# haberdashPI/SignalOperators.jl

Hardware: AMD Instinct MI355X
Metric: frames/sec sink() 44.1kHz 8ch Mix+Filt+Resample; achieved HBM GB/s (higher is better)
Workload: dtype f64

## Files before the change

include/sigops.h:

```cpp
#ifndef SIGOPS_H
#define SIGOPS_H

#include <stdint.h>

#ifdef __cplusplus
extern "C" {
#endif
#if defined(__GNUC__)
#pragma GCC visibility push(default)
#endif

#define SO_ABI_VERSION 1

typedef enum so_status {
    SO_OK = 0,
    SO_ERR_INVALID = -1,
    SO_ERR_LENGTH = -2,
    SO_ERR_UNSUPPORTED = -3,
    SO_ERR_RUNTIME = -4,
    SO_ERR_CHANNELS = -5,
    SO_ERR_NODEVICE = -6
} so_status_t;

typedef enum so_dtype {
// ... 39 lines not shown
    SO_RAMP_IDENTITY = 1,
    SO_RAMP_EXPR = 2
} so_rampfn_t;

typedef enum so_mapfn {
    SO_MAP_ADD = 0,
    SO_MAP_MUL = 1,
    SO_MAP_SUB = 2,
    SO_MAP_DIV = 3,
    SO_MAP_TUPLECAT = 4,
    SO_MAP_GETCHAN = 5,
    SO_MAP_AS1CHANNEL = 6,
    SO_MAP_ASNCHANNELS = 7,
    SO_MAP_TOELTYPE = 8,
    SO_MAP_REVERSECH = 9,
    SO_MAP_EXPR = 10
} so_mapfn_t;

typedef struct so_eop {
    int32_t code;
    int32_t arg;
} so_eop_t;

typedef enum so_eop_code {
    SO_EOP_ARG = 0,
    SO_EOP_CONST = 1,
    SO_EOP_UN = 2,
    SO_EOP_BIN = 3,
    SO_EOP_CMP = 4,
    SO_EOP_SELECT = 5,
    SO_EOP_ROUND32 = 6,
    SO_EOP_INTERP = 7
} so_eop_code_t;

typedef enum so_un {
    SO_UN_NEG = 0, SO_UN_ABS = 1, SO_UN_SQRT = 2, SO_UN_CBRT = 3, SO_UN_SQUARE = 4,
    SO_UN_RECIPROCAL = 5, SO_UN_EXP = 6, SO_UN_EXP2 = 7, SO_UN_EXPM1 = 8, SO_UN_LOG = 9,
    SO_UN_LOG2 = 10, SO_UN_LOG10 = 11, SO_UN_LOG1P = 12, SO_UN_SIN = 13, SO_UN_COS = 14,
    SO_UN_TAN = 15, SO_UN_ARCSIN = 16, SO_UN_ARCCOS = 17, SO_UN_ARCTAN = 18, SO_UN_SINH = 19,
    SO_UN_COSH = 20, SO_UN_TANH = 21, SO_UN_ARCSINH = 22, SO_UN_ARCCOSH = 23,
    SO_UN_ARCTANH = 24, SO_UN_FLOOR = 25, SO_UN_CEIL = 26, SO_UN_TRUNC = 27, SO_UN_RINT = 28,
    SO_UN_SIGN = 29,
    SO_UN_COUNT = 30
} so_un_t;

typedef enum so_bin {
    SO_BIN_ADD = 0, SO_BIN_SUB = 1, SO_BIN_MUL = 2, SO_BIN_DIV = 3, SO_BIN_POW = 4,
    SO_BIN_REMAINDER = 5, SO_BIN_FMOD = 6, SO_BIN_MINIMUM = 7, SO_BIN_MAXIMUM = 8,
    SO_BIN_FMIN = 9, SO_BIN_FMAX = 10, SO_BIN_ARCTAN2 = 11, SO_BIN_HYPOT = 12,
    SO_BIN_COPYSIGN = 13,
    SO_BIN_COUNT = 14
} so_bin_t;

typedef enum so_cmp {
    SO_CMP_LT = 0, SO_CMP_LE = 1, SO_CMP_GT = 2, SO_CMP_GE = 3, SO_CMP_EQ = 4, SO_CMP_NE = 5,
    SO_CMP_COUNT = 6
} so_cmp_t;

typedef enum so_padkind {
    SO_PAD_VALUE = 0,
    SO_PAD_VECTOR = 1,
    SO_PAD_ZERO = 2,
    SO_PAD_ONE = 3,
    SO_PAD_LASTFRAME = 4,
    SO_PAD_CYCLE = 5,
    SO_PAD_MIRROR = 6
} so_padkind_t;

typedef enum so_rskind {
    SO_RS_RATIONAL = 0,
    SO_RS_ARBITRARY = 1,
    SO_RS_FIR = 2
} so_rskind_t;

typedef struct so_node {
    int32_t kind;
    int32_t dtype;
    int32_t nch;
    int32_t n_children;
    const int32_t* children;
    int64_t nframes;
    double fs;
    int32_t i0, i1, i2, i3;
    int64_t l0, l1;
    double d0, d1, d2, d3;
    const void* p0;
    const void* p1;
    int64_t s0, s1;
} so_node_t;

typedef struct so_out_desc {
    int32_t dtype;
    int32_t nch;
    int64_t nframes;
    int64_t frame_stride;
    int64_t chan_stride;
    int32_t is_device;
    int32_t reserved;
} so_out_desc_t;

typedef struct so_stats {
    int32_t n_stages;
    int32_t n_launches;
    int64_t algorithmic_bytes;
    int64_t scratch_bytes;
    int64_t h2d_bytes;
    int64_t d2h_bytes;
    double last_exec_ms;
    double dominant_kernel_ms;
    int64_t dominant_kernel_bytes;
    char dominant_kernel[64];
} so_stats_t;

typedef struct so_plan so_plan_t;

int32_t so_abi_version(void);

const char* so_last_error(void);

int32_t so_device_count(void);

int32_t so_plan_create(const so_node_t* nodes, int32_t n_nodes, int32_t root,
                       const so_out_desc_t* out, int32_t device, so_plan_t** plan);

int64_t so_plan_nframes(const so_plan_t* plan);

int32_t so_plan_execute(so_plan_t* plan, void* out, void* hip_stream);

int32_t so_plan_check(so_plan_t* plan, void* hip_stream);

int32_t so_plan_set_array(so_plan_t* plan, int32_t node_index, const void* data);

int32_t so_plan_stats(const so_plan_t* plan, so_stats_t* stats);

typedef struct so_step_info {
    char name[64];
    int64_t algorithmic_bytes;
    double ms;
    int32_t launches;
    int32_t pad;
} so_step_info_t;
int32_t so_plan_step_info(const so_plan_t* plan, int32_t index, so_step_info_t* info);

typedef enum so_counter {
    SO_COUNTER_GRAPH_REPLAYS = 0,
    SO_COUNTER_GRAPH_CAPTURES = 1,
    SO_COUNTER_DIRECT_EXECUTES = 2,
    SO_COUNTER_FUSED_MFMAS_PER_BLOCK = 3,
    SO_COUNTER_WPROJ = 4,
    SO_COUNTER_RSOS_RANGE_PERIODS = 5,
    SO_COUNTER_RSOS_WARMUP_PERIODS = 6,
    SO_COUNTER_RSOS_PERIOD_INPUTS = 7,
    SO_COUNTER_WPROJ_FRAMES = 8,
    SO_COUNTER_WPROJ_FIRST = 9
} so_counter_t;
int64_t so_plan_counter(const so_plan_t* plan, int32_t which);

int32_t so_rtc_compile_check(const char* body, char* log, int32_t log_capacity);

int32_t so_rtc_wait_idle(void);
int32_t so_rtc_shutdown(void);

int32_t so_plan_set_profiling(so_plan_t* plan, int32_t enable);

void so_plan_destroy(so_plan_t* plan);

typedef struct so_comm so_comm_t;
typedef struct so_slab {
    int64_t rows, row_elems;
    int64_t dst_offset;
    int64_t dst_row_stride;
} so_slab_t;
int32_t so_comm_unique_id(void* id128);
int32_t so_comm_create(const void* id128, int32_t world, int32_t rank, int32_t device, so_comm_t** comm);
int32_t so_comm_allgather(so_comm_t* comm, const void* mine, int64_t src_row_stride, void* full,
                          const so_slab_t* slabs, int32_t dtype, void* stream);
int32_t so_comm_reduce_sum(so_comm_t* comm, void* buf, int64_t rows, int64_t row_elems, int64_t row_stride,
                           int32_t dtype, int32_t root, void* stream);
const char* so_comm_last_error(void);
void so_comm_destroy(so_comm_t* comm);

typedef enum so_filt_type {
    SO_FILT_LOWPASS = 0,
    SO_FILT_HIGHPASS = 1,
    SO_FILT_BANDPASS = 2,
    SO_FILT_BANDSTOP = 3
} so_filt_type_t;

typedef enum so_filt_method {
    SO_METHOD_BUTTERWORTH = 0,
    SO_METHOD_CHEBYSHEV1 = 1
} so_filt_method_t;

int32_t so_design_iir(int32_t type, double f1, double f2, double fs, int32_t method,
                      int32_t order, double ripple_db, double* sos, int32_t sos_capacity,
                      int32_t* nsections, double* gain);

int32_t so_design_iir_zpk(int32_t type, double f1, double f2, double fs, int32_t method, int32_t order,
                          double ripple_db, double* z, int32_t* nz, double* p, int32_t* np, int32_t capacity,
                          double* k);
int32_t so_zpk_to_sos(const double* z, int32_t nz, const double* p, int32_t np, double k, double* sos,
                      int32_t sos_capacity, int32_t* nsections, double* gain);

int32_t so_tf_to_sos(const double* b, int32_t nb, const double* a, int32_t na, double* sos, int32_t sos_capacity,
                     int32_t* nsections, double* gain, double* residual);
int32_t so_tf_zero_input(const double* b, int32_t nb, const double* a, int32_t na, const double* si, int32_t nsi,
                         double* out, int64_t capacity, int64_t* nframes);

int32_t so_design_resample_rational(int64_t num, int64_t den, double* h, int32_t capacity,
                                    int32_t* hlen);
int32_t so_design_resample_arbitrary(double rate, int32_t nphi, double* h, int32_t capacity,
                                     int32_t* hlen);

int32_t so_resample_positions(double fs_in, double fs_out, double rate, int32_t nphi, const double* h,
                              int32_t hlen, int64_t n_out, int64_t* j, int32_t* p, double* alpha,
                              int64_t* nfix, int64_t* nbaked);

int32_t so_rsos_wproj_matrix(const double* sos, int32_t nsec, double gain, const double* tab, const int32_t* jend,
                             int32_t ngroups, int32_t kw, int64_t m, int32_t wp, double* v, int32_t capacity,
                             int32_t* j0, int32_t* k);

#if defined(__GNUC__)
#pragma GCC visibility pop
#endif
#ifdef __cplusplus
}
#endif
#endif
```

signaloperators.jl_amd/_capi.py:

```python
import ctypes as C
import os

_HERE = os.path.dirname(os.path.abspath(__file__))
LIB_PATH = os.environ.get("SIGOPS_LIB") or os.path.join(_HERE, "csrc", "libsigops.so")

SO_F32, SO_F64, SO_I64 = 0, 1, 2
SO_LEN_INF, SO_LEN_MISSING, SO_LEN_UNCHECKED = -1, -2, -3
(NODE_ARRAY, NODE_CONST, NODE_FUNC, NODE_UNTIL, NODE_AFTER, NODE_PAD, NODE_APPEND, NODE_RAMP,
 NODE_MAP, NODE_FILT_SOS, NODE_RESAMPLE, NODE_NORMPOWER, NODE_SAMPLEAT, NODE_COMB, NODE_CUMSUM,
 NODE_MOVING, NODE_MOVSUM, NODE_RECUR) = range(18)
FN = {"sin": 0, "cos": 1, "identity": 2, "randn": 3}
SO_FN_RANDN = FN["randn"]
RAMPFN = {"sinramp": 0, "identity": 1, "expr": 2}
MAPFN = {"add": 0, "mul": 1, "sub": 2, "div": 3, "tuplecat": 4, "getchan": 5, "as1channel": 6,
         "asnchannels": 7, "toeltype": 8, "reversech": 9, "expr": 10}
EOP = {"arg": 0, "const": 1, "un": 2, "bin": 3, "cmp": 4, "select": 5, "round32": 6, "interp": 7}
INTERP_MAX_KNOTS = 1 << 20
UN = {name: i for i, name in enumerate((
    "neg", "abs", "sqrt", "cbrt", "square", "reciprocal", "exp", "exp2", "expm1", "log", "log2", "log10", "log1p",
    "sin", "cos", "tan", "arcsin", "arccos", "arctan", "sinh", "cosh", "tanh", "arcsinh", "arccosh", "arctanh",
    "floor", "ceil", "trunc", "rint", "sign"))}
BIN = {name: i for i, name in enumerate((
    "add", "sub", "mul", "div", "pow", "remainder", "fmod", "minimum", "maximum", "fmin", "fmax", "arctan2", "hypot",
    "copysign"))}
CMP = {"lt": 0, "le": 1, "gt": 2, "ge": 3, "eq": 4, "ne": 5}
PAD = {"value": 0, "vector": 1, "zero": 2, "one": 3, "lastframe": 4, "cycle": 5, "mirror": 6}
RS_RATIONAL, RS_ARBITRARY, RS_FIR = 0, 1, 2
FILT = {"lowpass": 0, "highpass": 1, "bandpass": 2, "bandstop": 3}
METHOD = {"butterworth": 0, "chebyshev1": 1}


class so_node_t(C.Structure):
    _fields_ = [("kind", C.c_int32), ("dtype", C.c_int32), ("nch", C.c_int32),
                ("n_children", C.c_int32), ("children", C.POINTER(C.c_int32)),
                ("nframes", C.c_int64), ("fs", C.c_double),
                ("i0", C.c_int32), ("i1", C.c_int32), ("i2", C.c_int32), ("i3", C.c_int32),
                ("l0", C.c_int64), ("l1", C.c_int64),
                ("d0", C.c_double), ("d1", C.c_double), ("d2", C.c_double), ("d3", C.c_double),
                ("p0", C.c_void_p), ("p1", C.c_void_p), ("s0", C.c_int64), ("s1", C.c_int64)]


class so_out_desc_t(C.Structure):
    _fields_ = [("dtype", C.c_int32), ("nch", C.c_int32), ("nframes", C.c_int64),
                ("frame_stride", C.c_int64), ("chan_stride", C.c_int64),
                ("is_device", C.c_int32), ("reserved", C.c_int32)]


class so_stats_t(C.Structure):
    _fields_ = [("n_stages", C.c_int32), ("n_launches", C.c_int32),
                ("algorithmic_bytes", C.c_int64), ("scratch_bytes", C.c_int64),
                ("h2d_bytes", C.c_int64), ("d2h_bytes", C.c_int64),
                ("last_exec_ms", C.c_double), ("dominant_kernel_ms", C.c_double),
                ("dominant_kernel_bytes", C.c_int64), ("dominant_kernel", C.c_char * 64)]


class so_slab_t(C.Structure):
    _fields_ = [("rows", C.c_int64), ("row_elems", C.c_int64), ("dst_offset", C.c_int64), ("dst_row_stride", C.c_int64)]


class so_step_info_t(C.Structure):
    _fields_ = [("name", C.c_char * 64), ("algorithmic_bytes", C.c_int64), ("ms", C.c_double),
                ("launches", C.c_int32), ("pad", C.c_int32)]


EXPORTS = ["so_abi_version", "so_last_error", "so_device_count", "so_plan_create",
           "so_plan_nframes", "so_plan_execute", "so_plan_check", "so_plan_set_array", "so_plan_stats",
           "so_plan_set_profiling", "so_plan_destroy", "so_design_iir",
           "so_design_resample_rational", "so_design_resample_arbitrary",
           "so_resample_positions", "so_plan_step_info", "so_design_iir_zpk", "so_zpk_to_sos", "so_tf_to_sos", "so_tf_zero_input", "so_plan_counter", "so_rsos_wproj_matrix",
           "so_rtc_compile_check", "so_rtc_wait_idle", "so_rtc_shutdown", "so_comm_unique_id", "so_comm_create", "so_comm_allgather", "so_comm_reduce_sum", "so_comm_last_error", "so_comm_destroy"]

_lib = None


class EngineMissing(RuntimeError):
    pass


def lib():
    global _lib
    if _lib is not None:
        return _lib
    if not os.path.exists(LIB_PATH):
        raise EngineMissing(
            f"{LIB_PATH} not built: run `python __graft_entry__.py build` "
            "(hipcc --offload-arch=gfx950). The HIP engine has no CPU fallback.")
    try:
        import importlib.util as _ilu

        if _ilu.find_spec("torch") is not None:
            import torch
    except Exception:
        pass
    L = C.CDLL(LIB_PATH)
    L.so_abi_version.restype = C.c_int32
    L.so_last_error.restype = C.c_char_p
    L.so_device_count.restype = C.c_int32
    L.so_plan_create.restype = C.c_int32
    L.so_plan_create.argtypes = [C.POINTER(so_node_t), C.c_int32, C.c_int32,
                                 C.POINTER(so_out_desc_t), C.c_int32, C.POINTER(C.c_void_p)]
    L.so_plan_nframes.restype = C.c_int64
    L.so_plan_nframes.argtypes = [C.c_void_p]
    L.so_plan_execute.restype = C.c_int32
    L.so_plan_execute.argtypes = [C.c_void_p, C.c_void_p, C.c_void_p]
    L.so_plan_check.restype = C.c_int32
    L.so_plan_check.argtypes = [C.c_void_p, C.c_void_p]
    L.so_plan_set_array.restype = C.c_int32
    L.so_plan_set_array.argtypes = [C.c_void_p, C.c_int32, C.c_void_p]
    L.so_plan_stats.restype = C.c_int32
    L.so_plan_stats.argtypes = [C.c_void_p, C.POINTER(so_stats_t)]
    L.so_plan_set_profiling.restype = C.c_int32
    L.so_plan_set_profiling.argtypes = [C.c_void_p, C.c_int32]
    L.so_plan_destroy.restype = None
    L.so_plan_destroy.argtypes = [C.c_void_p]
    L.so_design_iir.restype = C.c_int32
    L.so_design_iir.argtypes = [C.c_int32, C.c_double, C.c_double, C.c_double, C.c_int32,
                                C.c_int32, C.c_double, C.POINTER(C.c_double), C.c_int32,
                                C.POINTER(C.c_int32), C.POINTER(C.c_double)]
    L.so_design_resample_rational.restype = C.c_int32
    L.so_design_resample_rational.argtypes = [C.c_int64, C.c_int64, C.POINTER(C.c_double),
                                              C.c_int32, C.POINTER(C.c_int32)]
    L.so_design_resample_arbitrary.restype = C.c_int32
    L.so_design_resample_arbitrary.argtypes = [C.c_double, C.c_int32, C.POINTER(C.c_double),
                                               C.c_int32, C.POINTER(C.c_int32)]
    L.so_design_iir_zpk.restype = C.c_int32
    L.so_design_iir_zpk.argtypes = [C.c_int32, C.c_double, C.c_double, C.c_double, C.c_int32, C.c_int32, C.c_double,
                                    C.POINTER(C.c_double), C.POINTER(C.c_int32), C.POINTER(C.c_double),
                                    C.POINTER(C.c_int32), C.c_int32, C.POINTER(C.c_double)]
    L.so_zpk_to_sos.restype = C.c_int32
    L.so_zpk_to_sos.argtypes = [C.POINTER(C.c_double), C.c_int32, C.POINTER(C.c_double), C.c_int32, C.c_double,
                                C.POINTER(C.c_double), C.c_int32, C.POINTER(C.c_int32), C.POINTER(C.c_double)]
    L.so_tf_to_sos.restype = C.c_int32
    L.so_tf_to_sos.argtypes = [C.POINTER(C.c_double), C.c_int32, C.POINTER(C.c_double), C.c_int32, C.POINTER(C.c_double),
                               C.c_int32, C.POINTER(C.c_int32), C.POINTER(C.c_double), C.POINTER(C.c_double)]
    L.so_tf_zero_input.restype = C.c_int32
    L.so_tf_zero_input.argtypes = [C.POINTER(C.c_double), C.c_int32, C.POINTER(C.c_double), C.c_int32,
                                   C.POINTER(C.c_double), C.c_int32, C.POINTER(C.c_double), C.c_int64,
                                   C.POINTER(C.c_int64)]
    L.so_rtc_compile_check.restype = C.c_int32
    L.so_rtc_compile_check.argtypes = [C.c_char_p, C.c_char_p, C.c_int32]
    L.so_rtc_wait_idle.restype = C.c_int32
    L.so_rtc_wait_idle.argtypes = []
    L.so_rtc_shutdown.restype = C.c_int32
    L.so_rtc_shutdown.argtypes = []
    import atexit

    atexit.register(L.so_rtc_shutdown)
    L.so_comm_unique_id.restype = C.c_int32
    L.so_comm_unique_id.argtypes = [C.c_void_p]
    L.so_comm_create.restype = C.c_int32
    L.so_comm_create.argtypes = [C.c_void_p, C.c_int32, C.c_int32, C.c_int32, C.POINTER(C.c_void_p)]
    L.so_comm_allgather.restype = C.c_int32
    L.so_comm_allgather.argtypes = [C.c_void_p, C.c_void_p, C.c_int64, C.c_void_p, C.POINTER(so_slab_t), C.c_int32, C.c_void_p]
    L.so_comm_reduce_sum.restype = C.c_int32
    L.so_comm_reduce_sum.argtypes = [C.c_void_p, C.c_void_p, C.c_int64, C.c_int64, C.c_int64, C.c_int32, C.c_int32, C.c_void_p]
    L.so_comm_last_error.restype = C.c_char_p
    L.so_comm_destroy.restype = None
    L.so_comm_destroy.argtypes = [C.c_void_p]
    L.so_plan_counter.restype = C.c_int64
    L.so_plan_counter.argtypes = [C.c_void_p, C.c_int32]
    L.so_rsos_wproj_matrix.restype = C.c_int32
    L.so_rsos_wproj_matrix.argtypes = [C.POINTER(C.c_double), C.c_int32, C.c_double, C.POINTER(C.c_double), C.POINTER(C.c_int32),
                                       C.c_int32, C.c_int32, C.c_int64, C.c_int32, C.POINTER(C.c_double), C.c_int32,
                                       C.POINTER(C.c_int32), C.POINTER(C.c_int32)]
    L.so_plan_step_info.restype = C.c_int32
    L.so_plan_step_info.argtypes = [C.c_void_p, C.c_int32, C.POINTER(so_step_info_t)]
    L.so_resample_positions.restype = C.c_int32
    L.so_resample_positions.argtypes = [C.c_double, C.c_double, C.c_double, C.c_int32, C.POINTER(C.c_double),
                                        C.c_int32, C.c_int64, C.POINTER(C.c_int64), C.POINTER(C.c_int32),
                                        C.POINTER(C.c_double), C.POINTER(C.c_int64), C.POINTER(C.c_int64)]
    if L.so_abi_version() != 1:
        raise EngineMissing("libsigops ABI version mismatch")
    _lib = L
    return L


def last_error():
    return lib().so_last_error().decode("utf-8", "replace")
```

signaloperators.jl_amd/csrc/capi.cpp:

```cpp
#include <hip/hip_runtime_api.h>

#include <cstring>
#include <string>
#include <vector>

#include "../../include/sigops.h"
#include "plan.h"

namespace {
thread_local std::string g_err;
int set_err(int status, const std::string& msg) {
    g_err = msg;
    return status;
}
}

struct so_plan {
    so::Plan* p;
};

extern "C" {

int32_t so_abi_version(void) { return SO_ABI_VERSION; }

// ... 73 lines not shown
int32_t so_rtc_shutdown(void) {
    so::rtc_shutdown();
    return SO_OK;
}

int64_t so_plan_counter(const so_plan_t* plan, int32_t which) {
    if (!plan) return -1;
    return so::plan_counter(plan->p, which);
}

int32_t so_plan_step_info(const so_plan_t* plan, int32_t index, so_step_info_t* info) {
    if (!plan) return set_err(SO_ERR_INVALID, "so_plan_step_info: null plan");
    return so::plan_step_info(plan->p, index, info);
}

void so_plan_destroy(so_plan_t* plan) {
    if (!plan) return;
    so::plan_destroy(plan->p);
    delete plan;
}

int32_t so_design_iir(int32_t type, double f1, double f2, double fs, int32_t method,
                      int32_t order, double ripple_db, double* sos, int32_t sos_capacity,
                      int32_t* nsections, double* gain) {
    std::vector<double> s;
    double g = 1.0;
    std::string err;
    int st = so::design_iir(type, f1, f2, fs, method, order, ripple_db, s, g, err);
    if (st != SO_OK) return set_err(st, err);
    if (!sos || !nsections || !gain || (int)s.size() > sos_capacity)
        return set_err(SO_ERR_INVALID, "so_design_iir: output buffer too small");
    std::memcpy(sos, s.data(), s.size() * sizeof(double));
    *nsections = (int32_t)(s.size() / 6);
    *gain = g;
    return SO_OK;
}

int32_t so_design_iir_zpk(int32_t type, double f1, double f2, double fs, int32_t method, int32_t order,
                          double ripple_db, double* z, int32_t* nz, double* p, int32_t* np, int32_t capacity,
                          double* k) {
    std::vector<double> zz, pp;
    double kk = 1.0;
    std::string err;
    int st = so::design_iir_zpk(type, f1, f2, fs, method, order, ripple_db, zz, pp, kk, err);
    if (st != SO_OK) return set_err(st, err);
    if (!z || !p || !nz || !np || !k || (int)zz.size() > 2 * capacity || (int)pp.size() > 2 * capacity)
        return set_err(SO_ERR_INVALID, "so_design_iir_zpk: output buffer too small");
    std::memcpy(z, zz.data(), zz.size() * sizeof(double));
    std::memcpy(p, pp.data(), pp.size() * sizeof(double));
    *nz = (int32_t)(zz.size() / 2);
    *np = (int32_t)(pp.size() / 2);
    *k = kk;
    return SO_OK;
}

int32_t so_zpk_to_sos(const double* z, int32_t nz, const double* p, int32_t np, double k, double* sos,
                      int32_t sos_capacity, int32_t* nsections, double* gain) {
    std::vector<double> s;
    double g = 1.0;
    std::string err;
    if ((nz > 0 && !z) || (np > 0 && !p)) return set_err(SO_ERR_INVALID, "so_zpk_to_sos: null roots");
    int st = so::zpk_to_sos(z, nz, p, np, k, s, g, err);
    if (st != SO_OK) return set_err(st, err);
    if (!sos || !nsections || !gain || (int)s.size() > sos_capacity)
        return set_err(SO_ERR_INVALID, "so_zpk_to_sos: output buffer too small");
    std::memcpy(sos, s.data(), s.size() * sizeof(double));
    *nsections = (int32_t)(s.size() / 6);
    *gain = g;
    return SO_OK;
}

int32_t so_tf_to_sos(const double* b, int32_t nb, const double* a, int32_t na, double* sos, int32_t sos_capacity,
                     int32_t* nsections, double* gain, double* residual) {
    std::vector<double> s;
    double g = 1.0, r = 0.0;
    std::string err;
    int st = so::tf_to_sos(b, nb, a, na, s, g, r, err);
    if (st != SO_OK) return set_err(st, err);
    if (!sos || !nsections || !gain || (int)s.size() > sos_capacity)
        return set_err(SO_ERR_INVALID, "so_tf_to_sos: output buffer too small");
    std::memcpy(sos, s.data(), s.size() * sizeof(double));
    *nsections = (int32_t)(s.size() / 6);
    *gain = g;
    if (residual) *residual = r;
    return SO_OK;
}

int32_t so_tf_zero_input(const double* b, int32_t nb, const double* a, int32_t na, const double* si, int32_t nsi,
                         double* out, int64_t capacity, int64_t* nframes) {
    std::string err;
    int64_t used = 0;
    if (!out || !nframes || capacity < 0) return set_err(SO_ERR_INVALID, "so_tf_zero_input: null output");
    int st = so::tf_zero_input(b, nb, a, na, si, nsi, out, capacity, used, err);
    if (st != SO_OK) return set_err(st, err);
    *nframes = used;
    return SO_OK;
}

static int32_t copy_taps(const std::vector<double>& h, double* out, int32_t capacity, int32_t* hlen) {
    if (!hlen) return set_err(SO_ERR_INVALID, "null hlen");
    *hlen = (int32_t)h.size();
    if (!out) return SO_OK;
    if ((int)h.size() > capacity) return set_err(SO_ERR_INVALID, "tap buffer too small");
    std::memcpy(out, h.data(), h.size() * sizeof(double));
    return SO_OK;
}

int32_t so_design_resample_rational(int64_t num, int64_t den, double* h, int32_t capacity,
                                    int32_t* hlen) {
    std::vector<double> t;
    std::string err;
    int st = so::design_resample_rational(num, den, t, err);
    if (st != SO_OK) return set_err(st, err);
    return copy_taps(t, h, capacity, hlen);
}

int32_t so_design_resample_arbitrary(double rate, int32_t nphi, double* h, int32_t capacity,
                                     int32_t* hlen) {
    std::vector<double> t;
    std::string err;
    int st = so::design_resample_arbitrary(rate, nphi, t, err);
    if (st != SO_OK) return set_err(st, err);
    return copy_taps(t, h, capacity, hlen);
}

int32_t so_resample_positions(double fs_in, double fs_out, double rate, int32_t nphi, const double* h,
                              int32_t hlen, int64_t n_out, int64_t* j, int32_t* p, double* alpha,
                              int64_t* nfix, int64_t* nbaked) {
    if (!h || hlen < 1 || nphi < 1 || !(rate > 0) || n_out < 0 || !j || !p || !alpha)
        return set_err(SO_ERR_INVALID, "so_resample_positions: bad arguments");
    return so::resample_positions(fs_in, fs_out, rate, nphi, h, hlen, n_out, j, p, alpha, nfix, nbaked);
}

int32_t so_rsos_wproj_matrix(const double* sos, int32_t nsec, double gain, const double* tab, const int32_t* jend,
                             int32_t ngroups, int32_t kw, int64_t m, int32_t wp, double* v, int32_t capacity,
                             int32_t* j0, int32_t* k) {
    if (!sos || !tab || !jend || !v || !j0 || !k || nsec < 1 || nsec > 6 || ngroups < 1 || kw < 1 || m < 1 || wp < 1)
        return set_err(SO_ERR_INVALID, "so_rsos_wproj_matrix: bad arguments");
    if (ngroups > 256 || kw > 4096 || capacity < 0 || m > (1 << 20) || wp > (1 << 20) || (int64_t)wp * m + kw > (1 << 22))
        return set_err(SO_ERR_INVALID, "so_rsos_wproj_matrix: period, window or warm-up too long");
    for (int g = 0; g < ngroups; ++g)
        if (jend[g] < -(1 << 22) || jend[g] > (1 << 22)) return set_err(SO_ERR_INVALID, "so_rsos_wproj_matrix: window end out of range");
    std::vector<double> V;
    int jj = 0, K = 0;
    so::rsos_wproj_matrix_sos(sos, nsec, gain, tab, jend, ngroups, kw, m, wp, V, jj, K);
    *j0 = jj;
    *k = K;
    if (K > capacity) return set_err(SO_ERR_INVALID, "so_rsos_wproj_matrix: capacity too small");
    for (int d = 0; d < 12; ++d)
        for (int o = 0; o < K; ++o) v[(size_t)d * capacity + o] = V[(size_t)d * K + o];
    return SO_OK;
}

}
```

signaloperators.jl_amd/csrc/executor.cpp:

```cpp
#include "plan_impl.h"

namespace so {

static inline int carrier_vec_ok(const DCarrier& c, int64_t V) {
    if (!std::getenv("SIGOPS_STRICT_ALIGN")) return (uintptr_t)c.base % (c.dtype == SO_F64 ? 8 : 4) == 0;
    return ((uintptr_t)c.base % 16 == 0) && (c.cstride % V == 0);
}

static hipError_t h2d_small(void* dst, const void* src, size_t bytes) {
    constexpr size_t kPiece = 16 * 1024;
    if (bytes < 2 * kPiece || bytes > (1u << 20)) return hipMemcpy(dst, src, bytes, hipMemcpyHostToDevice);
    for (size_t off = 0; off < bytes; off += kPiece) {
        const hipError_t e = hipMemcpy((char*)dst + off, (const char*)src + off, std::min(kPiece, bytes - off), hipMemcpyHostToDevice);
        if (e != hipSuccess) return e;
    }
    return hipSuccess;
}

static void upload_tables(Plan* P) {
    std::vector<Buf>& bufs = P->bufs;
    auto up = [&](int buf, const auto& v, size_t at = 0) {
        HIPCHECK(h2d_small((char*)bufs[buf].d + at, v.data(), v.size() * sizeof(*v.data())));
    };
    auto alloc_up = [](auto*& d, const auto& v) {
// ... 723 lines not shown
    const int nl = launch_comb(a, st);
    if (nl < 0) fail(SO_ERR_UNSUPPORTED, "Comb: more than 65535 channels, or a delay AND a signal of 2^39 frames and more, are not lowered");
    return nl;
}

static int run_cumsum(Plan* P, const Step& s, void* outp, hipStream_t st) {
    const Stage& S = P->stages[s.idx];
    const Node& N = P->nodes[S.node];
    const int xdt = P->nodes[N.kids[0]].dtype;
    const View in = stage_in(P, S, N.nch, xdt), out = stage_out(P, s.idx, outp);
    CumsumArgs a{};
    a.x = in.d;
    a.xcs = in.pitch;
    a.xfs = S.x_fstride;
    a.x_f32 = xdt == SO_F32;
    a.y = (double*)out.d;
    a.ycs = out.pitch;
    a.n = S.need;
    a.nch = N.nch;
    a.tot_pitch = cumsum_totals(S.need);
    a.tot = S.aux_buf >= 0 ? (double*)P->bufs[S.aux_buf].d : nullptr;
    const int nl = launch_cumsum(a, st);
    if (nl < 0) fail(SO_ERR_UNSUPPORTED, "Cumsum: more than 65535 channels, or 2^31 chunks of 16384 frames and more, are not lowered");
    return nl;
}

static int run_recur(Plan* P, const Step& s, void* outp, hipStream_t st) {
    const Stage& S = P->stages[s.idx];
    const Node& N = P->nodes[S.node];
    const bool row = N.kids.size() == 2;
    const int bdt = P->nodes[N.kids[row ? 1 : 0]].dtype;
    const View in = stage_in(P, S, N.nch, bdt), out = stage_out(P, s.idx, outp);
    RecurArgs a{};
    a.b = in.d;
    a.bcs = in.pitch;
    a.bfs = S.x_fstride;
    a.b_f32 = bdt == SO_F32;
    if (!row) {
        a.ac = N.nd.d0;
    } else if (S.pos_array_node >= 0) {
        a.a = (const double*)array_base(P, S.pos_array_node) + S.pos_offset;
        a.acs = S.pos_pitch;
    } else {
        const Buf& b = P->bufs[S.pos_buf];
        a.a = (const double*)b.d;
        a.acs = S.pos_pitch == 0 ? 0 : b.pitch;
    }
    a.y = (double*)out.d;
    a.ycs = out.pitch;
    a.n = S.need;
    a.nch = N.nch;
    a.op = N.nd.i0;
    a.tot_pitch = cumsum_totals(S.need);
    a.tot = S.aux_buf >= 0 ? (double*)P->bufs[S.aux_buf].d : nullptr;
    const int nl = launch_recur(a, st);
    if (nl < 0) fail(SO_ERR_UNSUPPORTED, "Recur: more than 65535 channels, or 2^31 chunks of 16384 frames and more, are not lowered");
    return nl;
}

static int run_moving(Plan* P, const Step& s, void* outp, hipStream_t st) {
    const Stage& S = P->stages[s.idx];
    const Node& N = P->nodes[S.node];
    const View in = stage_in(P, S, N.nch, N.dtype), out = stage_out(P, s.idx, outp);
    MovingArgs a{};
    a.x = in.d;
    a.xcs = in.pitch;
    a.xfs = S.x_fstride;
    a.n_in = S.in_frames;
    a.y = out.d;
    a.ycs = out.pitch;
    a.n_out = S.need - S.base;
    a.off = S.base - S.in_base;
    a.back = N.nd.l0;
    a.ahead = N.nd.l1;
    a.tab = S.aux_buf >= 0 ? P->bufs[S.aux_buf].d : nullptr;
    a.nch = N.nch;
    a.f32 = N.dtype == SO_F32;
    a.is_min = N.nd.i0;
    const int nl = launch_moving(a, st);
    if (nl < 0) fail(SO_ERR_UNSUPPORTED, "Moving: more than 65535 channels, or 2^31 tiles of 2048 frames and more, are not lowered");
    return nl;
}

static int run_movsum(Plan* P, const Step& s, void* outp, hipStream_t st) {
    const Stage& S = P->stages[s.idx];
    const Node& N = P->nodes[S.node];
    const int xdt = P->nodes[N.kids[0]].dtype;
    const View in = stage_in(P, S, N.nch, xdt), out = stage_out(P, s.idx, outp);
    MovsumArgs a{};
    a.x = in.d;
    a.xcs = in.pitch;
    a.xfs = S.x_fstride;
    a.x_f32 = xdt == SO_F32;
    a.n_in = S.in_frames;
    a.y = (double*)out.d;
    a.ycs = out.pitch;
    a.n_out = S.need - S.base;
    a.off = S.base - S.in_base;
    a.abs0 = S.in_base;
    a.back = N.nd.l0;
    a.ahead = N.nd.l1;
    a.tab = S.aux_buf >= 0 ? (double*)P->bufs[S.aux_buf].d : nullptr;
    a.nch = N.nch;
    a.op = N.nd.i0;
    const int nl = launch_movsum(a, st);
    if (nl < 0) fail(SO_ERR_UNSUPPORTED, "Movsum: more than 65535 channels, or 2^31 tiles of 2048 frames or blocks of 1024 frames and more, are not lowered");
    return nl;
}

static int run_rsos_fused(Plan* P, const Stage& S, const SosGeom& g, const View& out, hipStream_t st) {
    const Node& N = P->nodes[S.node];
    const Stage& S3 = P->stages[S.rsos_src];
    RsSos rs = S.rs;
    rs.out_pitch = out.pitch;
    rs.out_f32 = g.out_dtype == SO_F32 || N.dtype == SO_F32;
    if (rs.f32m && rs.out_f32) rs.ring32 = 1;
    else rs.f32m = 0;
    rs.sring = rs.f32m && (rs.fuse == 1 || rs.fuse == 2) && !std::getenv("SIGOPS_RSOS_NO_SRING") ? 1 : 0;
    char* const yk = out.d - (size_t)S.rs.store_lo * (rs.out_f32 ? 4 : 8);
    rs.store_lo = S.rs.store_lo + g.store_lo;
    rs.mats = (const double*)P->bufs[S.rsos_mats_buf].d;
    rs.bad = nullptr;
    const bool fixup = S.rsos_jrel_buf >= 0 && !std::getenv("SIGOPS_RSOS_NO_FIXUP");
    int rearm = 0;
    if (S.bad_buf >= 0 && rs.nranges >= 1 && !std::getenv("SIGOPS_SOS_NOPOISON")) {
        int32_t* const words = (int32_t*)P->bufs[S.bad_buf].d;
        const size_t nch = (size_t)N.nch;
        if (fixup && !P->graph_plan && rs.nch == N.nch && P->bufs[S.bad_buf].bytes >= 2 * nch * 4) {
            if (!S.bad_armed) {
                arm_bad(words, 2 * nch, st);
                S.bad_set = 0;
            }
            rs.bad = words + (S.bad_set ? nch : 0);
            rearm = S.bad_set ? -(int)nch : (int)nch;
        } else {
            S.bad_armed = false;
            rs.bad = words;
            arm_bad(rs.bad, nch, st);
        }
    }
    rs.err = kernel_error_word(P);
    static long long* d_rtrace = nullptr;
    static int rtrace_seen = 0;
    const char* const rtrace_skip = std::getenv("SIGOPS_RSOS_TRACE_SKIP");
    const bool rtracing = std::getenv("SIGOPS_RSOS_TRACE") != nullptr && rtrace_seen++ >= (rtrace_skip ? std::atoi(rtrace_skip) : 0);
    const size_t rtrace_n = (size_t)(16 * kRsosTraceIters + 16) * 8;
    if (rtracing) {
        if (!d_rtrace) HIPCHECK(hipMalloc(&d_rtrace, rtrace_n * 8));
        HIPCHECK(hipMemsetAsync(d_rtrace, 0, rtrace_n * 8, st));
        rs.trace = d_rtrace;
    }
    const double* rtab = (const double*)P->bufs[S.rsos_tab_buf >= 0 ? S.rsos_tab_buf : S3.tab_buf].d;
    const int* rjend = (const int*)P->bufs[S.rsos_jend_buf >= 0 ? S.rsos_jend_buf : S3.jend_buf].d;
    if (launch_rsos(rtab, rjend, rs, yk, global_tables(P, S3), S.rsos_grid, st) != 0)
        fail(SO_ERR_RUNTIME, "internal: no fused resampler + IIR instantiation for this geometry");
    if (rtracing) dump_rsos_trace(d_rtrace, rtrace_n, rs, st);
    int nl = 1;
    if (rs.bad && fixup) {
        RsFixup fx{};
        set_rsos_fixup(fx, P, S, RsosItem{rs, rtab, rjend, yk, global_tables(P, S3)});
        fx.rearm = rearm;
        nl += launch_rsos_fixup(fx, st);
        if (rearm != 0) {
            S.bad_set ^= 1;
            S.bad_armed = true;
        }
    } else if (rs.bad) {
        SosGeom pg = g;
        pg.n = rs.n_out;
        pg.chunk = rs.pr * rs.L;
        pg.nchunks = rs.nranges;
        pg.store_lo = rs.store_lo;
        pg.bad = rs.bad;
        nl += launch_sos_poison(yk, pg, st);
    }
    return nl;
}

static int run_sos(Plan* P, const Step& s, void* outp, hipStream_t st) {
    const Stage& S = P->stages[s.idx];
    const Node& N = P->nodes[S.node];
    const size_t esz = dsize(N.dtype);
    const View in = stage_in(P, S, N.nch, N.dtype), out = stage_out(P, s.idx, outp);
    SosGeom g = S.sg;
    g.in_pitch = in.pitch;
    g.out_pitch = out.pitch;
    g.store_lo = s.idx == P->alias_stage ? P->alias_skip : 0;
    if (s.idx == P->alias_stage && P->alias_narrow) g.out_dtype = SO_F32;
    g.align_rows = S.pre_stage < 0 && !std::getenv("SIGOPS_SOS_NOALIGN");
    g.bad = nullptr;
    if (S.rsos_src >= 0) return run_rsos_fused(P, S, g, out, st);
    if (S.bad_buf >= 0 && S.pre_stage < 0 && !S.onepass && !S.xscan && !g.exact && !std::getenv("SIGOPS_SOS_NOPOISON")) {
        g.bad = (int32_t*)P->bufs[S.bad_buf].d;
        arm_bad(g.bad, (size_t)N.nch, st);
    }
    int nl = 0;
    for (size_t gi = 0; gi < S.groups.size() && S.onepass; ++gi) {
        const void* x = gi == 0 ? (const void*)in.d : (const void*)out.d;
        SosOne o = S.so1;
        o.in_pitch = gi == 0 ? in.pitch : out.pitch;
        o.out_pitch = out.pitch;
        const int64_t al = 16 / (int64_t)esz;
        o.vec_in = ((uintptr_t)x % 16 == 0) && (o.in_pitch % al == 0);
        o.vec_out = ((uintptr_t)out.d % 16 == 0) && (o.out_pitch % al == 0);
        const Buf& sb = P->bufs[S.one_sync_buf];
        const Buf& vb = P->bufs[S.one_vpub_buf];
        if (sb.bytes % 4 == 0 && vb.bytes % 4 == 0) {
            HIPCHECK((hipError_t)launch_fill_u32(sb.d, sb.bytes / 4, 0u, st));
            HIPCHECK((hipError_t)launch_fill_u32(vb.d, vb.bytes / 4, 0xffffffffu, st));
        } else {
            HIPCHECK(hipMemsetAsync(sb.d, 0, sb.bytes, st));
            HIPCHECK(hipMemsetAsync(vb.d, 0xff, vb.bytes, st));
        }
        launch_sos_onepass(x, out.d, o, S.groups[gi], (const double*)P->bufs[S.one_tabs_buf].d + S.one_tabs_off[gi],
                           (int*)sb.d, (double*)vb.d, N.dtype, st);
        nl += 1;
    }
    if (S.pre_stage >= 0) {
        const Stage& S3 = P->stages[S.pre_stage];
        nl += launch_sos_prestate(in.d, out.d, (const double*)P->bufs[S3.vper_buf].d, S3.rp.nperiods,
                                  (const double*)P->bufs[S.qmat_buf].d, S3.rp.pt, (double*)P->bufs[S.v_buf].d,
                                  (double*)P->bufs[S.s0_buf].d, (const double*)P->bufs[S.mpow_buf].d, g, S.groups[0], st);
    }
    bool exact_done = false;
    if (g.exact && !S.onepass && S.pre_stage < 0 && S.groups.size() <= 2) {
        exact_done = launch_sos_exact(in.d, out.d, g, S.groups[0], S.groups.size() > 1 ? S.groups[1] : SosCoefs{}, st) == 0;
        if (exact_done) nl += 1;
    }
    for (size_t gi = 0; gi < S.groups.size() && !S.onepass && S.pre_stage < 0 && !exact_done; ++gi) {
        const void* x = gi == 0 ? (const void*)in.d : (const void*)out.d;
        SosGeom gg = g;
        if (gi > 0) gg.in_pitch = out.pitch;
        if (gi == 0 && S.src_op) set_sine_source(gg, S);
        if (S.xscan) {
            double* vb = (double*)P->bufs[S.v_buf].d;
            double* sb = (double*)P->bufs[S.s0_buf].d;
            nl += launch_sos_phase(x, out.d, vb, nullptr, gg, S.groups[gi], 1, st);
            nl += launch_sos_xscan(vb, sb, (const double*)((char*)P->bufs[S.xs_mats_buf].d + gi * 2 * 16 * 16 * 8),
                                   (double*)P->bufs[S.sblk_buf].d, gg, S.groups[gi].nsec, st);
            nl += launch_sos_phase(x, out.d, nullptr, sb, gg, S.groups[gi], 3, st);
            continue;
        }
        nl += launch_sos(x, out.d, S.v_buf >= 0 ? (double*)P->bufs[S.v_buf].d : nullptr,
                         S.s0_buf >= 0 ? (double*)P->bufs[S.s0_buf].d : nullptr,
                         S.mpow_buf >= 0 ? (const double*)((char*)P->bufs[S.mpow_buf].d + gi * S.mpow_stride() * 8) : nullptr,
                         gg, S.groups[gi], st);
        nl += launch_sos_poison(out.d, gg, st);
        if (gg.bad && gi + 1 < S.groups.size()) arm_bad(gg.bad, (size_t)N.nch, st);
    }
    return nl;
}

static void run_resample_periodic(Plan* P, const Step& s, const View& out, hipStream_t st) {
    const Stage& S = P->stages[s.idx];
    const Node& N = P->nodes[S.node];
    RsPeriodic rp = S.rp;
    rp.in_pitch = 0;
    rp.out_pitch = out.pitch;
    rp.out_f32 = s.idx == P->alias_stage && P->alias_narrow;
    if (rp.nstate > 0) {
        rp.wtab = (const double*)P->bufs[S.wtab_buf].d;
        rp.vper = (double*)P->bufs[S.vper_buf].d;
    }
    const int64_t al = 16 / (int64_t)dsize(N.dtype);
    rp.vec_ok = ((uintptr_t)out.d % 16 == 0) && (out.pitch % al == 0) && (rp.L % al == 0);
    static long long* d_trace = nullptr;
    const bool tracing = std::getenv("SIGOPS_RS_TRACE") != nullptr;
    const size_t trace_n = (size_t)16 * kRsTraceIters * kRsTraceStamps;
    if (tracing) {
        if (!d_trace) HIPCHECK(hipMalloc(&d_trace, trace_n * 8));
        HIPCHECK(hipMemsetAsync(d_trace, 0, trace_n * 8, st));
        rp.trace = d_trace;
    }
    const bool nf_fix = S.rs_nf_buf >= 0 && S.rs_jrel_buf >= 0 && rp.ga == 0 && rp.arr2 == 0 && rp.nstate == 0 && S.ctl_buf >= 0 &&
                        S.car_buf >= 0 && !S.carriers.empty() && rp.rows <= 32 && rp.kw <= 160;
    rp.nf = nf_fix ? (uint32_t*)P->bufs[S.rs_nf_buf].d : nullptr;
    const double* tab = (const double*)P->bufs[S.tab_buf].d;
    const int* jend = (const int*)P->bufs[S.jend_buf].d;
    if (launch_resample_periodic(out.d, tab, jend, rp, N.dtype, global_tables(P, S), st) != 0)
        fail(SO_ERR_RUNTIME, "internal: no periodic resampler instantiation for this geometry");
    if (nf_fix) {
        RsPerFixup fx{};
        fx.g = rp;
        fx.tab = tab;
        fx.jend = jend;
        fx.jrel = (const int*)P->bufs[S.rs_jrel_buf].d;
        fx.taps = S.rg.taps;
        fx.out_f32 = (N.dtype == SO_F32 || rp.out_f32) ? 1 : 0;
        fx.gsrc = global_tables(P, S);
        fx.y = out.d;
        (void)launch_rs_fixup(fx, st);
    }
    if (tracing) dump_rs_trace(d_trace, trace_n, rp, st);
}

static int run_resample(Plan* P, const Step& s, void* outp, hipStream_t st) {
    const Stage& S = P->stages[s.idx];
    const Node& N = P->nodes[S.node];
    const View in = S.periodic ? View{nullptr, 0} : stage_in(P, S, N.nch, N.dtype), out = stage_out(P, s.idx, outp);
    const double* pfbt = S.tiled ? (const double*)P->bufs[S.pfbt_buf].d : nullptr;
    const double* dpfbt = S.tiled ? (const double*)P->bufs[S.dpfbt_buf].d : nullptr;
    if (S.periodic)
        run_resample_periodic(P, s, out, st);
    else if (S.rows) {
        RsRows rr = S.rr;
        rr.in_pitch = in.pitch;
        rr.out_pitch = out.pitch;
// ... 172 lines not shown
                if (ms > best) {
                    best = ms;
                    P->stats.dominant_kernel_ms = ms;
                    P->stats.dominant_kernel_bytes = P->steps[si].bytes;
                    std::snprintf(P->stats.dominant_kernel, sizeof P->stats.dominant_kernel, "%s", P->steps[si].name.c_str());
                }
            }
            P->stats.last_exec_ms = total;
        }
    } catch (const PlanError& e) {
        disarm_bad(P);
        err = e.msg;
        return e.status;
    }
    return SO_OK;
}

int plan_execute(Plan* P, void* outp, void* stream, std::string& err) {
    DeviceGuard guard(P->device);
    if (kernel_gave_up(P, err)) {
        disarm_bad(P);
        return SO_ERR_RUNTIME;
    }
    const bool eligible = P->steps.size() >= 4 && P->out.is_device && P->host_leaves.empty() && !P->profiling &&
                          !std::getenv("SIGOPS_NO_GRAPH") && !std::getenv("SIGOPS_RS_TRACE");
    P->graph_plan = eligible;
    if (!eligible) {
        P->n_direct++;
        return plan_execute_direct(P, outp, stream, err);
    }
    hipStream_t st = (hipStream_t)stream;
    const bool leaves_match = P->out_alias_buf < 0 || P->bufs[P->out_alias_buf].d == outp;
    if (P->graph_exec && P->graph_out == outp && P->graph_epoch == P->array_epoch && leaves_match) {
        if (hipSetDevice(P->device) == hipSuccess && hipGraphLaunch(P->graph_exec, st) == hipSuccess) {
            P->n_replays++;
            return SO_OK;
        }
        (void)hipGetLastError();
        (void)hipGraphExecDestroy(P->graph_exec);
        P->graph_exec = nullptr;
        P->graph_failed = true;
    }
    if (P->graph_failed || P->last_out != outp || P->last_epoch != P->array_epoch) {
        P->last_out = outp;
        P->last_epoch = P->array_epoch;
        P->n_direct++;
        return plan_execute_direct(P, outp, stream, err);
    }
    if (P->graph_exec && P->graph_out == outp && P->graph_epoch == P->array_epoch) {
        P->n_direct++;
        return plan_execute_direct(P, outp, stream, err);
    }
    if (P->graph_exec) {
        (void)hipGraphExecDestroy(P->graph_exec);
        P->graph_exec = nullptr;
    }
    hipGraph_t graph = nullptr;
    if (!P->capture_stream && hipStreamCreateWithFlags(&P->capture_stream, hipStreamNonBlocking) != hipSuccess)
        P->capture_stream = nullptr;
    if (!P->capture_stream || hipSetDevice(P->device) != hipSuccess ||
        hipStreamBeginCapture(P->capture_stream, hipStreamCaptureModeRelaxed) != hipSuccess) {
        (void)hipGetLastError();
        P->graph_failed = true;
        return plan_execute_direct(P, outp, stream, err);
    }
    const int rc = plan_execute_direct(P, outp, (void*)P->capture_stream, err);
    const hipError_t ec = hipStreamEndCapture(P->capture_stream, &graph);
    if (std::getenv("SIGOPS_DEBUG_PLAN"))
        std::fprintf(stderr, "[sigops] graph capture: rc=%d end=%d (%s) graph=%p err=%s\n", rc, (int)ec, hipGetErrorString(ec), (void*)graph, err.c_str());
    if (rc != SO_OK || ec != hipSuccess || !graph ||
        hipGraphInstantiate(&P->graph_exec, graph, nullptr, nullptr, 0) != hipSuccess) {
        (void)hipGetLastError();
        if (graph) (void)hipGraphDestroy(graph);
        P->graph_exec = nullptr;
        P->graph_failed = true;
        return rc != SO_OK ? rc : plan_execute_direct(P, outp, stream, err);
    }
    (void)hipGraphDestroy(graph);
    P->graph_out = outp;
    P->graph_epoch = P->array_epoch;
    P->n_captures++;
    if (hipGraphLaunch(P->graph_exec, st) != hipSuccess) {
        (void)hipGetLastError();
        P->graph_failed = true;
        return plan_execute_direct(P, outp, stream, err);
    }
    return SO_OK;
}

int plan_set_array(Plan* P, int32_t node_index, const void* data, std::string& err) {
    if (node_index < 0 || node_index >= (int)P->nodes.size() || P->nodes[node_index].nd.kind != SO_NODE_ARRAY) {
        err = "so_plan_set_array: not an ARRAY node";
        return SO_ERR_INVALID;
    }
    DeviceGuard guard(P->device);
    P->array_ptr[node_index] = data;
    P->array_epoch++;
    if (P->nodes[node_index].nd.i0) {
        bool changed = false;
        for (size_t i = 0; i < P->leaves.size(); ++i)
            if (P->leaf_array_node[i] == node_index) {
                P->leaves[i].base = data;
                changed = true;
            }
        if (changed && P->d_leaves)
            if (hipMemcpy(P->d_leaves, P->leaves.data(), P->leaves.size() * sizeof(DLeaf), hipMemcpyHostToDevice) != hipSuccess) {
                err = "so_plan_set_array: leaf upload failed";
                return SO_ERR_RUNTIME;
            }
        for (auto& S : P->stages) {
            bool touched = false;
            for (auto& c : S.carriers) {
                if (c.array_node == node_index) {
                    c.base = data;
                    const int64_t V = 16 / (int64_t)dsize(c.dtype);
                    c.vec_ok = carrier_vec_ok(c, V);
                    touched = true;
                }
                if (car_has_arr2(c) && c.array_node2 == node_index) {
                    c.base2 = data;
                    c.vec_ok2 = (uintptr_t)c.base2 % (c.dtype2 == SO_F64 ? 8 : 4) == 0;
                    touched = true;
                }
            }
            if (touched) {
                const RsCtl ctl = P->make_ctl(S);
                if (hipMemcpy(P->bufs[S.car_buf].d, S.carriers.data(), S.carriers.size() * sizeof(DCarrier), hipMemcpyHostToDevice) != hipSuccess ||
                    hipMemcpy(P->bufs[S.ctl_buf].d, &ctl, sizeof(RsCtl), hipMemcpyHostToDevice) != hipSuccess) {
                    err = "so_plan_set_array: carrier upload failed";
                    return SO_ERR_RUNTIME;
                }
            }
        }
    }
    return SO_OK;
}

int64_t plan_nframes(const Plan* P) {
    const Node& R = P->nodes[P->root];
    return isinf_(R.len) ? SO_LEN_INF : R.len.n;
}
void plan_stats(const Plan* P, so_stats_t* st) { *st = P->stats; }
void plan_set_profiling(Plan* P, int mode) {
    P->profiling = mode < 0 || mode > 2 ? 1 : mode;
    P->prof_execs = 0;
}
int64_t plan_counter(const Plan* P, int which) {
    switch (which) {
    case SO_COUNTER_GRAPH_REPLAYS: return P->n_replays;
    case SO_COUNTER_GRAPH_CAPTURES: return P->n_captures;
    case SO_COUNTER_DIRECT_EXECUTES: return P->n_direct;
    case SO_COUNTER_FUSED_MFMAS_PER_BLOCK: {
        for (const Stage& S : P->stages)
            if (S.kind == ST_SOS && S.rsos_src >= 0 && S.need > 0) return S.rs.ks + 14;
        return 0;
    }
    case SO_COUNTER_WPROJ: {
        for (const Stage& S : P->stages)
            if (S.kind == ST_SOS && S.rsos_src >= 0 && S.need > 0) return S.rs.wproj;
        return 0;
    }
    case SO_COUNTER_RSOS_RANGE_PERIODS:
    case SO_COUNTER_RSOS_WARMUP_PERIODS:
    case SO_COUNTER_RSOS_PERIOD_INPUTS:
    case SO_COUNTER_WPROJ_FRAMES:
    case SO_COUNTER_WPROJ_FIRST:
        for (const Stage& S : P->stages)
            if (S.kind == ST_SOS && S.rsos_src >= 0 && S.need > 0)
                return which == SO_COUNTER_RSOS_RANGE_PERIODS ? S.rs.pr : which == SO_COUNTER_RSOS_WARMUP_PERIODS ? S.rs.wp
                     : which == SO_COUNTER_RSOS_PERIOD_INPUTS ? S.rs.M : which == SO_COUNTER_WPROJ_FRAMES ? S.rs.wk : S.rs.wj0;
        return 0;
    default: return -1;
    }
}
int plan_step_info(const Plan* P, int index, so_step_info_t* info) {
    if (info && index >= 0 && index < (int)P->steps.size()) {
        const Step& s = P->steps[index];
        std::memset(info, 0, sizeof *info);
        std::snprintf(info->name, sizeof info->name, "%s", s.name.c_str());
        info->algorithmic_bytes = s.bytes;
        info->ms = s.ms;
        if (P->profiling == 2 && P->prof_execs > 0) {
            const size_t evset = 2 * P->steps.size();
            const int64_t n = std::min<int64_t>(P->prof_execs, (int64_t)prof_cap(P));
            double sum = 0;
            int64_t got = 0;
            for (int64_t e = 0; e < n; ++e) {
                float ms = 0;
                if (hipEventElapsedTime(&ms, P->events[evset * e + 2 * index], P->events[evset * e + 2 * index + 1]) == hipSuccess) {
                    sum += ms;
                    ++got;
                } else (void)hipGetLastError();
            }
            info->ms = got ? sum / (double)got : 0.0;
        }
        info->launches = s.launches;
    }
    return (int)P->steps.size();
}
int plan_check(Plan* P, void* stream, std::string& err) {
    DeviceGuard guard(P->device);
    try {
        if (P->nlanes > 1 || P->graph_exec) HIPCHECK(hipDeviceSynchronize());
        else HIPCHECK(hipStreamSynchronize((hipStream_t)stream));
    } catch (const PlanError& e) {
        err = e.msg;
        return e.status;
    }
    if (kernel_gave_up(P, err)) return SO_ERR_RUNTIME;
    return SO_OK;
}

void plan_destroy(Plan* P) {
    if (!P) return;
    {
        DeviceGuard guard(P->device);
        P->release();
    }
    delete P;
}


}
```

signaloperators.jl_amd/csrc/k_rsos.hip:

```cpp
#include "kcommon.h"
#include "kstage.h"

#ifndef SO_RSOS_ONLY_KS
#define SO_RSOS_ONLY_KS -1
#endif
#ifndef SO_RSOS_ONLY_F32
#define SO_RSOS_ONLY_F32 0
#endif
#ifndef SO_RSOS_ONLY_NW
#define SO_RSOS_ONLY_NW 0
#endif

namespace so {

typedef double v4d __attribute__((ext_vector_type(4)));
typedef float v4f __attribute__((ext_vector_type(4)));

#define SO_LDS __attribute__((address_space(3)))
__device__ __forceinline__ int flag_ld(uint32_t a) { return *(const volatile SO_LDS int*)(uintptr_t)a; }
__device__ __forceinline__ void flag_st(uint32_t a, int v) { *(volatile SO_LDS int*)(uintptr_t)a = v; }
#define SO_SPIN_PAUSE(spins, sleep, limit)                         \
    do {                                                           \
        if (++(spins) > (limit)) rsos_wait_failed(sh);             \
        if ((sleep) == 1) __builtin_amdgcn_s_sleep(1);             \
        else __builtin_amdgcn_s_sleep(2);                          \
    } while (0)
__device__ __forceinline__ int wave_min(int v, int n) {
    int m = __builtin_amdgcn_readlane(v, 0);
#pragma unroll
    for (int i = 1; i < 12; ++i)
        if (i < n) m = min(m, __builtin_amdgcn_readlane(v, i));
    return m;
}
__device__ __forceinline__ void wait_vmcnt_le60(int n) {
#define SO_W(k) case k: asm volatile("s_waitcnt vmcnt(" #k ")" ::: "memory"); break;
    if (n < 8) {
        switch (n < 0 ? 0 : n) { SO_W(0) SO_W(1) SO_W(2) SO_W(3) SO_W(4) SO_W(5) SO_W(6) SO_W(7) }
    } else {
        switch (n > 60 ? 15 : n >> 2) {
            case 2: asm volatile("s_waitcnt vmcnt(8)" ::: "memory"); break;
            case 3: asm volatile("s_waitcnt vmcnt(12)" ::: "memory"); break;
            case 4: asm volatile("s_waitcnt vmcnt(16)" ::: "memory"); break;
            case 5: asm volatile("s_waitcnt vmcnt(20)" ::: "memory"); break;
            case 6: asm volatile("s_waitcnt vmcnt(24)" ::: "memory"); break;
            case 7: asm volatile("s_waitcnt vmcnt(28)" ::: "memory"); break;
            case 8: asm volatile("s_waitcnt vmcnt(32)" ::: "memory"); break;
            case 9: asm volatile("s_waitcnt vmcnt(36)" ::: "memory"); break;
            case 10: asm volatile("s_waitcnt vmcnt(40)" ::: "memory"); break;
            case 11: asm volatile("s_waitcnt vmcnt(44)" ::: "memory"); break;
            case 12: asm volatile("s_waitcnt vmcnt(48)" ::: "memory"); break;
            case 13: asm volatile("s_waitcnt vmcnt(52)" ::: "memory"); break;
            case 14: asm volatile("s_waitcnt vmcnt(56)" ::: "memory"); break;
            default: asm volatile("s_waitcnt vmcnt(60)" ::: "memory"); break;
        }
    }
#undef SO_W
}

__device__ __attribute__((noinline)) double2 rsos_sine_at(int64_t i1, double omega, double phi, double fs, int has_omega) {
    const double t = __ddiv_rn((double)i1, fs);
    const double ph = has_omega ? __dadd_rn(__dmul_rn(t, omega), phi) : __dadd_rn(t, phi);
    double sb, cb;
    sincospi_c(2.0 * ph, sb, cb);
    return double2{sb, cb};
}

template <int RU>
__device__ __attribute__((noinline)) void rsos_stage_slow(int64_t n_in, int rpitch, const DCarrier* gcar, int ncar, const DOp* gops,
                                                          const DLeaf* gleaves, int64_t n0, int lanes, int ch0, double* buf) {
    const int lane = threadIdx.x & 63;
    if (lane < lanes) stage_generic_impl<double, RU, true>(n_in, rpitch, gcar, ncar, gops, gleaves, n0 + 2 * lane, lane, 0, ch0, buf);
}
template <int RU>
__device__ __attribute__((noinline)) void rsos_stage_slow32(int64_t n_in, int rpitch, const DCarrier* gcar, int ncar, const DOp* gops,
                                                            const DLeaf* gleaves, int64_t n0, int lanes, int ch0, float* buf) {
    const int lane = threadIdx.x & 63;
    if (lane < lanes) stage_generic_impl<float, RU>(n_in, 2 * rpitch, gcar, ncar, gops, gleaves, n0 + 4 * lane, lane, 0, ch0, buf);
}

template <int RU, int OP>
__device__ __forceinline__ void rsos_rmw(uint32_t la, uint32_t row_bytes, v2d gn) {
    if constexpr (RU > 4) {
        rsos_rmw<4, OP>(la, row_bytes, gn);
        rsos_rmw<RU - 4, OP>(la + 4 * row_bytes, row_bytes, gn);
        return;
    } else {
        v2d raw[RU];
#pragma unroll
        for (int c = 0; c < RU; ++c) raw[c] = lds_ld16(la + (uint32_t)c * row_bytes);
        lds_wait(raw);
#pragma unroll
        for (int c = 0; c < RU; ++c) raw[c] = OP == 0 ? raw[c] * gn : OP == 1 ? raw[c] + gn : OP == 2 ? raw[c] - gn : gn - raw[c];
        lds_pin(raw);
#pragma unroll
        for (int c = 0; c < RU; ++c) lds_st16(la + (uint32_t)c * row_bytes, raw[c]);
    }
}

template <int RU>
__device__ __forceinline__ void rsos_add(uint32_t la, uint32_t row_bytes, v2d gn) {
    const double g0 = gn[0], g1 = gn[1];
#pragma unroll
    for (int c = 0; c < RU; ++c) {
        const uint32_t a = la + (uint32_t)c * row_bytes;
        asm volatile("ds_add_f64 %0, %1\n\tds_add_f64 %0, %2 offset:8" ::"v"(a), "v"(g0), "v"(g1) : "memory");
    }
}

template <int RB, int C, int RU>
__device__ __forceinline__ void rsos_add_imm(uint32_t la, double g0, double g1) {
    if constexpr (C < RU) {
        asm volatile("ds_add_f64 %0, %1 offset:%3\n\tds_add_f64 %0, %2 offset:%4" ::"v"(la), "v"(g0), "v"(g1), "n"(C * RB), "n"(C * RB + 8) : "memory");
        rsos_add_imm<RB, C + 1, RU>(la, g0, g1);
    }
}

template <int RB, int R, int N>
__device__ __forceinline__ void rsos_add_rows(uint32_t la0, uint32_t la8, double g0, double g1) {
    if constexpr (N > 0) {
        asm volatile("ds_add_f64 %0, %1 offset:%3\n\tds_add_f64 %0, %2 offset:%4" ::"v"(R < 8 ? la0 : la8), "v"(g0), "v"(g1), "n"((R & 7) * RB), "n"((R & 7) * RB + 8) : "memory");
        rsos_add_rows<RB, R + 1, N - 1>(la0, la8, g0, g1);
    }
}
template <int RB, int RU, int NL, int J, int MUC>
__device__ __forceinline__ void rsos_add_units(uint32_t la0, uint32_t la8, const double2 (&bs)[MUC], double2 d0, double2 d1, bool sine, double gc, bool neg) {
    if constexpr (J < MUC) {
        double g0 = gc, g1 = gc;
        if (sine) {
            g0 = fma(bs[J].x, d0.y, bs[J].y * d0.x);
            g1 = fma(bs[J].x, d1.y, bs[J].y * d1.x);
        }
        if (neg) {
            g0 = -g0;
            g1 = -g1;
        }
        rsos_add_rows<RB, J * NL * RU, RU>(la0, la8, g0, g1);
        rsos_add_units<RB, RU, NL, J + 1, MUC>(la0, la8, bs, d0, d1, sine, gc, neg);
    }
}

template <int RU, int OP>
__device__ __forceinline__ void rsos_step32(uint32_t la, uint32_t row_bytes, float g0, float g1) {
    if constexpr (RU > 4) {
        rsos_step32<4, OP>(la, row_bytes, g0, g1);
        rsos_step32<RU - 4, OP>(la + 4 * row_bytes, row_bytes, g0, g1);
    } else {
        float2 raw[RU];
#pragma unroll
        for (int c = 0; c < RU; ++c) asm volatile("ds_read_b64 %0, %1" : "=v"(raw[c]) : "v"(la + (uint32_t)c * row_bytes) : "memory");
        if constexpr (RU == 4) asm volatile("s_waitcnt lgkmcnt(0)" : "+v"(raw[0]), "+v"(raw[1]), "+v"(raw[2]), "+v"(raw[3])::"memory");
        else if constexpr (RU == 2) asm volatile("s_waitcnt lgkmcnt(0)" : "+v"(raw[0]), "+v"(raw[1])::"memory");
        else asm volatile("s_waitcnt lgkmcnt(0)" : "+v"(raw[0])::"memory");
#pragma unroll
        for (int c = 0; c < RU; ++c) {
            raw[c].x = OP == 0 ? raw[c].x * g0 : OP == 1 ? raw[c].x + g0 : g0 - raw[c].x;
            raw[c].y = OP == 0 ? raw[c].y * g1 : OP == 1 ? raw[c].y + g1 : g1 - raw[c].y;
        }
#pragma unroll
        for (int c = 0; c < RU; ++c) asm volatile("ds_write_b64 %0, %1" ::"v"(la + (uint32_t)c * row_bytes), "v"(raw[c]) : "memory");
    }
}

template <int RB, int RU, int OP>
__device__ __forceinline__ void rsos_step32_imm(uint32_t la, float g0, float g1) {
    float2 raw[RU];
#define SO_RD(C) if constexpr (C < RU) asm volatile("ds_read_b64 %0, %1 offset:%2" : "=v"(raw[C < RU ? C : 0]) : "v"(la), "n"((C < RU ? C : 0) * RB) : "memory");
    SO_RD(0) SO_RD(1) SO_RD(2) SO_RD(3) SO_RD(4) SO_RD(5) SO_RD(6) SO_RD(7)
#undef SO_RD
    if constexpr (RU == 8) asm volatile("s_waitcnt lgkmcnt(0)" : "+v"(raw[0]), "+v"(raw[1]), "+v"(raw[2]), "+v"(raw[3]), "+v"(raw[4]), "+v"(raw[5]), "+v"(raw[6]), "+v"(raw[7])::"memory");
// ... 842 lines not shown
    v4d acc = v4d{0.0, 0.0, 0.0, 0.0};
    auto mm = [&](const double (&a)[16], const v2d (&b)[8]) __attribute__((always_inline)) {
#pragma unroll
        for (int i = 0; i < 8; ++i) {
            acc = __builtin_amdgcn_mfma_f64_16x16x4f64(a[2 * i], b[i][0], acc, 0, 0, 0);
            acc = __builtin_amdgcn_mfma_f64_16x16x4f64(a[2 * i + 1], b[i][1], acc, 0, 0, 0);
        }
    };
    auto load = [&](int c, double (&a)[16], v2d (&b)[8]) __attribute__((always_inline)) {
        const double SO_GLB* const vp = V + (size_t)c * 128;
        const double SO_GLB* const rp = row + (size_t)c * 8;
#pragma unroll
        for (int i = 0; i < 8; ++i) {
            a[2 * i] = vp[i * 128];
            a[2 * i + 1] = vp[i * 128 + 64];
            b[i] = *(const v2d_a8 SO_GLB*)(rp + 8 * i);
        }
    };
    double aA[16], aB[16];
    v2d bA[8], bB[8];
    const int c1f = min(c1, K >> 3);
    const int nfull = c1f > c0 ? (c1f - c0) >> 3 : 0;
    if (nfull > 0) {
        load(c0, aA, bA);
        if constexpr (SO_RSOS_TRACE) {
            asm volatile("s_waitcnt vmcnt(0)" ::: "memory");
            rsos_stamp_pro(trace, 1);
        }
        for (int n = 0; n < nfull; n += 2) {
            const int c = c0 + 8 * n;
            if (n + 1 < nfull) load(c + 8, aB, bB);
            mm(aA, bA);
            if (n + 2 < nfull) load(c + 16, aA, bA);
            if (n + 1 < nfull) mm(aB, bB);
        }
    }
    rsos_stamp_pro(trace, 2);
    {
        const int c = c0 + 8 * nfull;
#pragma unroll
        for (int i = 0; i < 8; ++i) {
            const int cc = c + i;
            aA[2 * i] = aA[2 * i + 1] = 0.0;
            bA[i] = v2d{0.0, 0.0};
            if (cc < c1) {
                aA[2 * i] = V[(size_t)(2 * cc) * 64];
                aA[2 * i + 1] = V[(size_t)(2 * cc + 1) * 64];
                const int f = 8 * cc + 2 * gq;
                if (f + 1 < K) bA[i] = *(const v2d_a8 SO_GLB*)(row + 8 * cc);
                else if (f < K) bA[i][0] = row[8 * cc];
            }
        }
        if constexpr (SO_RSOS_TRACE) {
            asm volatile("s_waitcnt vmcnt(0)" ::: "memory");
            rsos_stamp_pro(trace, 3);
        }
        mm(aA, bA);
    }
#pragma unroll
    for (int v = 0; v < 3; ++v) l.ss[(1 + yi) * 192 + v * 64 + lane] = acc[v];
    flag_st(fl_base + 4 * (kRsosFlagWp + yi), 1);
    rsos_stamp_pro(trace, 4);
}

template <int NY>
__device__ __attribute__((noinline)) void rsos_wproj_chain(RsosShared* sh_, double* dyn, int64_t G_) {
    constexpr int NX = 2 * NY + 1;
    const int lane = threadIdx.x & 63;
    SO_LDS RsosShared* const sh = (SO_LDS RsosShared*)rsos_lds_ptr(sh_);
    const int64_t G = rfl64(G_);
    const SO_LDS RsSos& g = sh->g;
    const RsosLds l = rsos_carve(dyn, uni(g.cyc) > 0 ? 0 : uni(g.ngroups) * uni(g.ks) * 64, uni(g.rpitch), NX, rsos_nss(NY));
    const uint32_t fl_base = (uint32_t)(uintptr_t)sh->flags;
    const int ct = uni(g.ct), fuse = uni(g.fuse);
    const int gq = lane >> 4, n16 = lane & 15;
    double s[3] = {0.0, 0.0, 0.0};
    long long* trace = nullptr;
    if constexpr (SO_RSOS_TRACE) trace = (long long*)rfl64((int64_t)(uintptr_t)g.trace);
    rsos_stamp_pro(trace, 0);
    if (fuse >= 0) {
        const SO_LDS DCarrier& C0 = sh->ctl.car[0];
        const DLeaf leaf0 = leaf_uniform(sh_->ctl.leaves[min(kCtlLeaves - 1, max(0, uni(C0.slot_leaf[0])))]);
        const int64_t ncg = uni(g.nch) / ct;
        const int64_t r = (G / ncg) * uni(g.rgs) + n16 / ct;
        const int64_t f0 = (r * rfl64(g.pr) - uni(g.wp)) * rfl64(g.M) + uni(g.wj0);
        const double2 sc = rsos_sine_at(f0 + leaf0.df + 1, leaf0.v0, leaf0.v1, leaf0.v2, leaf0.flag);
        const double SO_GLB* const W = (const double SO_GLB*)rfl64((int64_t)(uintptr_t)g.mats) + 14 * 64 + (size_t)((uni(g.wk) + 7) >> 3) * 128;
#pragma unroll
        for (int v = 0; v < 3; ++v) {
            const double t = fma(sc.y, W[gq + 4 * v], sc.x * W[16 + gq + 4 * v]);
            s[v] = fuse == 2 ? -t : t;
        }
    }
    int spins = 0;
    for (;;) {
        const int f = lane < NY ? flag_ld(fl_base + 4 * (kRsosFlagWp + lane)) : 1;
        if (wave_min(f, NY) >= 1) break;
        SO_SPIN_PAUSE(spins, 1, 1 << 22);
    }
    rsos_stamp_pro(trace, 1);
#pragma unroll
    for (int yi = 0; yi < NY; ++yi)
#pragma unroll
        for (int v = 0; v < 3; ++v) s[v] += l.ss[(1 + yi) * 192 + v * 64 + lane];
#pragma unroll
    for (int v = 0; v < 3; ++v) l.ss[v * 64 + lane] = s[v];
    rsos_stamp_pro(trace, 2);
}

template <int NY>
__device__ __attribute__((noinline)) void rsos_helper(RsosShared* sh_, double* dyn) {
    constexpr int NX = 2 * NY + 1;
    const int lane = threadIdx.x & 63;
    SO_LDS RsosShared* const sh = (SO_LDS RsosShared*)rsos_lds_ptr(sh_);
    const SO_LDS RsSos& g = sh->g;
    const RsosLds l = rsos_carve(dyn, 0, uni(g.rpitch), NX, rsos_nss(NY));
    const int NB = (uni(sh->wpe) + (int)rfl64(g.pr)) * uni(g.ngroups);
    const double SO_GLB* mats = (const double SO_GLB*)rfl64((int64_t)(uintptr_t)g.mats);
    const uint32_t fl_base = (uint32_t)(uintptr_t)sh->flags;
    const int debug = uni(g.debug);
    const bool f32m = uni(g.f32m) != 0 && uni(g.out_f32) != 0;
    double Dk[4];
#pragma unroll
    for (int v = 0; v < 4; ++v) Dk[v] = f32m ? mats[(lane >> 4) * 64 + v * 16 + (lane & 15)] : mats[v * 64 + lane];
    __builtin_amdgcn_s_setprio(1);
    constexpr int res[3] = {kRsosHres0, kRsosHres1, kRsosHres2};
    int hslot[3] = {kRsosHres0 % NX, kRsosHres1 % NX, kRsosHres2 % NX}, hring = 0;
    for (int b0 = 0; b0 < NB; b0 += NY) {
#pragma unroll
        for (int j = 0; j < 3; ++j) {
            const int bh = b0 + res[j];
            if (bh < NB) {
                int spins = 0;
                while (uni(flag_ld(fl_base + 4 * (kRsosFlagXh + j))) < bh + 1 && !(debug & 16)) SO_SPIN_PAUSE(spins, 2, 1 << 22);
                double xr[4];
#pragma unroll
                for (int v = 0; v < 3; ++v) xr[v] = l.xs[hslot[j] * 192 + v * 64 + lane];
                xr[3] = l.xh[(j * kRsosHslots + hring) * 64 + lane];
                v4d dh = v4d{0.0, 0.0, 0.0, 0.0};
#pragma unroll
                for (int v = 0; v < 4; ++v) dh = __builtin_amdgcn_mfma_f64_16x16x4f64(Dk[v], xr[v], dh, 0, 0, 0);
#pragma unroll
                for (int v = 0; v < 3; ++v) l.xs[hslot[j] * 192 + v * 64 + lane] = dh[v];
                flag_st(fl_base + 4 * (kRsosFlagXseq + hslot[j]), bh + 1);
            }
            hslot[j] += NY;
            if (hslot[j] >= NX) hslot[j] -= NX;
        }
        hring = hring + 1 == kRsosHslots ? 0 : hring + 1;
    }
    __builtin_amdgcn_s_setprio(0);
}

template <int KS, int NY, int NL, typename TO, int CYC, bool F32M = false, bool HW = false>
__device__ __attribute__((noinline)) void rsos_ywave(RsosShared* sh_, double* dyn, int64_t G_, int yi_) {
    static_assert(!F32M || (sizeof(TO) == 4 && CYC > 0), "the Float32 MFMA form: Float32 results, taps in registers");
    constexpr int NX = 2 * NY + 1;
    const int lane = threadIdx.x & 63;
    const int wave = uni(threadIdx.x >> 6);
    SO_LDS RsosShared* const sh = (SO_LDS RsosShared*)rsos_lds_ptr(sh_);
    const int64_t G = rfl64(G_);
    const int yi = uni(yi_);
    const SO_LDS RsSos& g = sh->g;
    const int ngroups = uni(g.ngroups), rpitch = uni(g.rpitch), RING = uni(g.ring);
    const RsosLds l = rsos_carve(dyn, CYC > 0 ? 0 : ngroups * KS * 64, rpitch, NX, rsos_nss(NY));
    const int ct = uni(g.ct), wp = uni(sh->wpe), debug = uni(g.debug);
    const int M = (int)rfl64(g.M);
    const int NB = (wp + (int)rfl64(g.pr)) * ngroups;
    constexpr int kw = 4 * KS;
    const int ulo_kw = uni(g.ulo) + (kw - 1);
    const int64_t n_out = rfl64(g.n_out), out_pitch = rfl64(g.out_pitch);
    const double SO_GLB* mats = (const double SO_GLB*)rfl64((int64_t)(uintptr_t)g.mats);
    long long* trace = (long long*)rfl64((int64_t)(uintptr_t)g.trace);
    TO SO_GLB* const y = (TO SO_GLB*)rfl64((int64_t)(uintptr_t)sh->y);
    const uint32_t fl_base = (uint32_t)(uintptr_t)sh->flags;
    const SO_LDS DCarrier& C0 = sh->ctl.car[0];
    const int64_t cs0 = rfl64(C0.cstride), df0 = rfl64(C0.df);
    const bool src32 = uni(g.src32) != 0;
    const bool x32 = sizeof(TO) == 4 && uni(g.x32) != 0;
    [[maybe_unused]] const bool ring32 = sizeof(TO) == 4 && uni(g.ring32) != 0;
    [[maybe_unused]] const bool sring = F32M && uni(g.sring) != 0;
    [[maybe_unused]] const int srow = ((lane & 15) / (ct < 8 ? ct : 8)) * (ct < 8 ? ct : 8);
    const bool single = uni((int)(C0.base != nullptr && C0.vec_ok && C0.dtype == (src32 ? SO_F32 : SO_F64))) && !(df0 & 1) && uni(g.fuse) >= -1 &&
                        (!src32 || uni(g.chunk) == 128) && (!uni(g.arr2) || rsos_two_ok(C0, uni(g.chunk)));
    const RsosGroup grp = rsos_group(sh, G, single, (int64_t)(rfl64((int64_t)(uintptr_t)C0.base) >> (src32 ? 2 : 3)), cs0, df0);
    const int gq = lane >> 4, n16 = lane & 15;
    double Dk[4], Tk[4], Ck[3];
    const int nkc = (uni(g.debug) & 131072) ? 3 : (2 * uni(g.nsec) + 3) / 4;
#pragma unroll
    for (int v = 0; v < 4; ++v) Dk[v] = F32M ? mats[(lane >> 4) * 64 + v * 16 + (lane & 15)] : mats[v * 64 + lane];
#pragma unroll
    for (int v = 0; v < 4; ++v) Tk[v] = F32M ? mats[(7 + (lane >> 4)) * 64 + v * 16 + (lane & 15)] : mats[(7 + v) * 64 + lane];
#pragma unroll
    for (int v = 0; v < 3; ++v) Ck[v] = mats[(11 + v) * 64 + lane];
    int cl;
    int nb0;
    {
        const int ri = n16 / ct;
        cl = ((grp.e0m + ri * grp.prMm) & 15) + gq;
        const int64_t ob = grp.ob0 + ri * grp.prL;
        nb0 = ob < 0 ? (int)((-ob) / 16) : 0;
    }
    const SO_LDS char* const ringc = (const SO_LDS char*)l.ring + (uint32_t)n16 * (uint32_t)rpitch * 8u;
    uint32_t yo0;
    int64_t ystep[4];
    const int64_t ybase_e = (int64_t)(grp.cg * ct) * out_pitch + grp.ob0;
#ifndef SO_Y_EARLY
#define SO_Y_EARLY 0
#endif
#ifndef SO_Y_SADDR
#define SO_Y_SADDR 1
#endif
#ifndef SO_ST_NT
#define SO_ST_NT " nt"
#endif
    const bool yfits = SO_Y_SADDR && uni((int)((((int64_t)(ct - 1) * out_pitch + (int64_t)(16 / ct) * grp.prL + 16) * (int64_t)sizeof(TO)) < ((int64_t)1 << 32)));
    int nbs_all;
    {
        int m = 0x7fffffff;
        int64_t off0 = 0;
#pragma unroll
        for (int v = 0; v < 4; ++v) {
            const int row = gq + 4 * v;
            const int ri = row / ct, cv = row % ct;
            const int64_t ob = grp.ob0 + ri * grp.prL;
            const int64_t off = ((int64_t)cv * out_pitch + (int64_t)ri * grp.prL + n16) * (int64_t)sizeof(TO);
            if (v == 0) off0 = off;
            ystep[v] = rfl64(off - off0);
            const int64_t tl = n_out - ob - n16;
            const int64_t nb = tl <= 0 ? 0 : (tl + 15) / 16;
            m = min(m, (int)(nb > 0x3fffffff ? 0x3fffffff : nb));
        }
        yo0 = (uint32_t)off0;
#pragma unroll
        for (int off = 32; off > 0; off >>= 1) m = min(m, __shfl_xor(m, off, 64));
        nbs_all = uni(m);
    }
    const int64_t slo = rfl64(g.store_lo);
    int nbl_max = 0;
    if (slo > grp.ob0) {
        const int64_t nb = (slo - grp.ob0 + 15) / 16;
        nbl_max = (int)(nb > 0x3fffffff ? 0x3fffffff : nb);
    }
    int nb0_any;
    {
        int m = nb0;
#pragma unroll
        for (int off = 32; off > 0; off >>= 1) m = max(m, __shfl_xor(m, off, 64));
        nb0_any = uni(m);
    }
    constexpr bool HELPABLE = HW && NY == 10 && CYC == 1;
    const bool help_on = HELPABLE && uni(g.help) != 0;
    const int hj = !help_on ? -1 : yi == kRsosHres0 ? 0 : yi == kRsosHres1 ? 1 : yi == kRsosHres2 ? 2 : -1;
    int hr = 0;
    int pi = 0, gi = yi;
    while (gi >= ngroups) {
        gi -= ngroups;
        ++pi;
    }
    int slot = yi % NX;
    int avail = 0;
    int wbm = -1;
    if (yi >= NB) flag_st(fl_base + 4 * (kRsosFlagYrd + yi), 0x7fffffff);
    uint32_t f_sseq = fl_base + 4 * kRsosFlagSseq, f_yrd = fl_base + 4 * (kRsosFlagYrd + yi);
    asm volatile("" : "+v"(f_sseq), "+v"(f_yrd));
    constexpr int NS = rsos_nss(NY);
    int sslot = yi % NS;
    int pb_ = -1, ppi_ = 0, pslot_ = 0;
    uint64_t ycur = (uint64_t)rfl64((int64_t)(uintptr_t)(y + (ybase_e + (int64_t)16 * yi))), ypend = 0;
    [[maybe_unused]] int cnt_in = 0, cnt_in_b = 0, cnt_st = 0, cnt_st_b = 0;
    [[maybe_unused]] const long long cyc0 = SO_RSOS_COUNT ? clock64() : 0;
    v4d payA = v4d{0.0, 0.0, 0.0, 0.0}, payB = v4d{0.0, 0.0, 0.0, 0.0};
    auto back_wait = [&](int sq, double (&sv)[3]) __attribute__((always_inline)) {
        int spins = 0;
        sq = uni(sq);
        if (sq < pb_ && !(debug & 8)) {
            if constexpr (SO_RSOS_COUNT) ++cnt_st_b;
            do {
                SO_SPIN_PAUSE(spins, 1, (debug & 32768) ? 4096 : (1 << 22));
                if constexpr (SO_RSOS_COUNT) ++cnt_st;
                sq = uni(flag_ld(f_sseq));
            } while (sq < pb_);
#pragma unroll
            for (int v = 0; v < 3; ++v) sv[v] = l.ss[pslot_ * 192 + v * 64 + lane];
        }
    };
    auto back_mfma = [&](const double (&sv)[3], v4d ay) __attribute__((always_inline)) {
        ay = __builtin_amdgcn_mfma_f64_16x16x4f64(sv[0], Ck[0], ay, 0, 0, 0);
        if (nkc > 1) ay = __builtin_amdgcn_mfma_f64_16x16x4f64(sv[1], Ck[1], ay, 0, 0, 0);
        if (nkc > 2) ay = __builtin_amdgcn_mfma_f64_16x16x4f64(sv[2], Ck[2], ay, 0, 0, 0);
        return ay;
    };
    auto back_store = [&](v4d ay, bool fresh) __attribute__((always_inline)) {
        if (debug & 1) return;
        const int64_t t0 = (int64_t)16 * pb_;
        const uint64_t yb = (uint64_t)rfl64((int64_t)ypend);
        if (fresh && yfits && sizeof(TO) == 8) asm volatile("s_nop 15\n\ts_nop 1" : "+v"(ay[0]), "+v"(ay[1]), "+v"(ay[2]), "+v"(ay[3])::"memory");
        auto out_index = [&](int v) __attribute__((always_inline)) { return grp.ob0 + (int64_t)((gq + 4 * v) / ct) * grp.prL + t0 + n16; };
        auto put = [&](int v, TO val) __attribute__((always_inline)) {
            if (yfits) {
                const uint64_t ybv = yb + (uint64_t)ystep[v];
                if constexpr (sizeof(TO) == 8) asm volatile("global_store_dwordx2 %0, %1, %2" SO_ST_NT ::"v"(yo0), "v"(val), "s"(ybv) : "memory");
                else asm volatile("global_store_dword %0, %1, %2" ::"v"(yo0), "v"(val), "s"(ybv) : "memory");
            } else {
                int row = gq + 4 * v;
                asm volatile("" : "+v"(row));
                y[(int64_t)(grp.cg * ct + row % ct) * out_pitch + grp.ob0 + (int64_t)(row / ct) * grp.prL + n16 + t0] = val;
            }
        };
        if (pb_ >= nbl_max && pb_ < nbs_all) {
#pragma unroll
            for (int v = 0; v < 4; ++v) put(v, (TO)ay[v]);
        } else {
#pragma unroll
            for (int v = 0; v < 4; ++v) {
                const int64_t m = out_index(v);
                if (m >= slo && m < n_out) put(v, (TO)ay[v]);
            }
        }
    };
    auto back = [&](int sq, double (&sv)[3], v4d& pay_) __attribute__((always_inline)) {
        back_wait(sq, sv);
        if (ppi_ < wp) return;
        rsos_stamp(trace, wave, pb_ / NY, 4, 40);
        back_store(back_mfma(sv, pay_), true);
        rsos_stamp(trace, wave, pb_ / NY, 5, 40);
    };
    using TapT = std::conditional_t<F32M, float, double>;
    auto block = [&](int b, const TapT (&at)[KS], v4d& pin, v4d& pout, int je, int jn) __attribute__((always_inline)) {
        const int wb = pi * M + je - ulo_kw;
        const int need = wb + kw + 16;
        rsos_stamp(trace, wave, b / NY, 0, 40);
        rsos_stamp_pro(trace, 5);
        int spins = 0;
        if constexpr (SO_RSOS_COUNT) cnt_in_b += avail < need ? 1 : 0;
        while (avail < need && !(debug & 16)) {
            const int v = lane < NL ? flag_ld(fl_base + 4 * (kRsosFlagLdp + lane)) : 0x7fffffff;
            avail = wave_min(v, NL);
            if (avail < need) {
                SO_SPIN_PAUSE(spins, 2, 1 << 22);
                if constexpr (SO_RSOS_COUNT) ++cnt_in;
            }
        }
        rsos_stamp(trace, wave, b / NY, 1, 40);
        int sq = 0;
        double sv[3] = {0.0, 0.0, 0.0};
        if (pb_ >= 0) {
            sq = flag_ld(f_sseq);
#pragma unroll
            for (int v = 0; v < 3; ++v) sv[v] = l.ss[pslot_ * 192 + v * 64 + lane];
        }
        if (wbm < 0) wbm = wb % RING;
        const int pos = wbm + cl;
        double bx[KS];
        bool have_bx = false;
        [[maybe_unused]] float bf32[KS];
        if constexpr (F32M) {
            if (wbm + 20 + kw <= RING) {
                const SO_LDS float* p0 = (const SO_LDS float*)(ringc + (uint32_t)pos * 4u);
#pragma unroll
                for (int s = 0; s < KS; ++s) bf32[s] = p0[4 * s];
            } else {
#pragma unroll
                for (int s = 0; s < KS; ++s) {
                    const int p_ = pos + 4 * s;
                    bf32[s] = *(const SO_LDS float*)(ringc + (uint32_t)(p_ >= RING ? p_ - RING : p_) * 4u);
                }
            }
            if (sring) {
                float sn[KS];
                const SO_LDS char* const sbase = (const SO_LDS char*)l.ring + (uint32_t)srow * (uint32_t)rpitch * 8u + (uint32_t)rpitch * 4u;
                if (wbm + 20 + kw <= RING) {
                    const SO_LDS float* p0 = (const SO_LDS float*)(sbase + (uint32_t)pos * 4u);
#pragma unroll
                    for (int s = 0; s < KS; ++s) sn[s] = p0[4 * s];
                } else {
#pragma unroll
                    for (int s = 0; s < KS; ++s) {
                        const int p_ = pos + 4 * s;
                        sn[s] = *(const SO_LDS float*)(sbase + (uint32_t)(p_ >= RING ? p_ - RING : p_) * 4u);
                    }
                }
#pragma unroll
                for (int s = 0; s < KS; ++s) bf32[s] += sn[s];
            }
            have_bx = true;
        } else if constexpr (sizeof(TO) == 4) {
            if (ring32) {
                float bf[KS];
                if (wbm + 20 + kw <= RING) {
                    const SO_LDS float* p0 = (const SO_LDS float*)(ringc + (uint32_t)pos * 4u);
#pragma unroll
                    for (int s = 0; s < KS; ++s) bf[s] = p0[4 * s];
                } else {
#pragma unroll
                    for (int s = 0; s < KS; ++s) {
                        const int p_ = pos + 4 * s;
                        bf[s] = *(const SO_LDS float*)(ringc + (uint32_t)(p_ >= RING ? p_ - RING : p_) * 4u);
                    }
                }
#pragma unroll
                for (int s = 0; s < KS; ++s) bx[s] = (double)bf[s];
                have_bx = true;
            }
        }
        if (have_bx) {
        } else if (wbm + 20 + kw <= RING) {
            const SO_LDS double* p0 = (const SO_LDS double*)(ringc + (uint32_t)pos * 8u);
#pragma unroll
            for (int s = 0; s < KS; ++s) bx[s] = p0[4 * s];
        } else {
#pragma unroll
            for (int s = 0; s < KS; ++s) {
                const int p_ = pos + 4 * s;
                bx[s] = *(const SO_LDS double*)(ringc + (uint32_t)(p_ >= RING ? p_ - RING : p_) * 8u);
            }
        }
        v4d ax = v4d{0.0, 0.0, 0.0, 0.0};
        if constexpr (F32M) {
            v4f a0 = v4f{0.f, 0.f, 0.f, 0.f}, a1 = v4f{0.f, 0.f, 0.f, 0.f};
#pragma unroll
            for (int s = 0; s < KS; ++s) {
                if (s & 1) a1 = __builtin_amdgcn_mfma_f32_16x16x4f32(at[s], bf32[s], a1, 0, 0, 0);
                else a0 = __builtin_amdgcn_mfma_f32_16x16x4f32(at[s], bf32[s], a0, 0, 0, 0);
            }
            const v4f af = a0 + a1;
#pragma unroll
            for (int v = 0; v < 4; ++v) ax[v] = (double)af[v];
        } else {
#pragma unroll
            for (int s = 0; s < KS; ++s) ax = __builtin_amdgcn_mfma_f64_16x16x4f64(at[s], bx[s], ax, 0, 0, 0);
        }
        if constexpr (sizeof(TO) == 4 && !F32M) {
            if (x32) {
#pragma unroll
                for (int v = 0; v < 4; ++v) ax[v] = (double)(float)ax[v];
            }
        }
        bool early = false;
        v4d ay_early = pin;
        if (SO_Y_EARLY && pb_ >= 0 && ppi_ >= wp && (uni(sq) >= pb_ || (debug & 8))) {
            ay_early = back_mfma(sv, pin);
            early = true;
        }
        int pi2 = pi, gi2 = gi + NY;
        while (gi2 >= ngroups) {
            gi2 -= ngroups;
            ++pi2;
        }
        const int wb2 = b + NY < NB ? pi2 * M + jn - ulo_kw : 0x7fffffff;
        flag_st(f_yrd, wb2);
        if (b + NY < NB) {
            wbm += wb2 - wb;
            while (wbm >= RING) wbm -= RING;
        }
        if (b < nb0_any) {
            asm volatile("" ::: "memory");
            if (b < nb0) ax = v4d{0.0, 0.0, 0.0, 0.0};
            asm volatile("" : "+v"(ax));
        }
        rsos_stamp(trace, wave, b / NY, 2, 40);
        v4d dx = v4d{0.0, 0.0, 0.0, 0.0};
        if (!HELPABLE || hj < 0) {
#pragma unroll
            for (int v = 0; v < 4; ++v) dx = __builtin_amdgcn_mfma_f64_16x16x4f64(Dk[v], ax[v], dx, 0, 0, 0);
        }
        pout = __builtin_amdgcn_mfma_f64_16x16x4f64(ax[0], Tk[0], v4d{0.0, 0.0, 0.0, 0.0}, 0, 0, 0);
#pragma unroll
        for (int v = 1; v < 4; ++v) pout = __builtin_amdgcn_mfma_f64_16x16x4f64(ax[v], Tk[v], pout, 0, 0, 0);
        if (!HELPABLE || hj < 0) {
#pragma unroll
            for (int v = 0; v < 3; ++v) l.xs[slot * 192 + v * 64 + lane] = dx[v];
            flag_st(fl_base + 4 * (kRsosFlagXseq + slot), b + 1);
        } else {
#pragma unroll
            for (int v = 0; v < 3; ++v) l.xs[slot * 192 + v * 64 + lane] = ax[v];
            l.xh[(hj * kRsosHslots + hr) * 64 + lane] = ax[3];
            flag_st(fl_base + 4 * (kRsosFlagXh + hj), b + 1);
            hr = hr + 1 == kRsosHslots ? 0 : hr + 1;
        }
        if (early) back_store(ay_early, false);
        else if (pb_ >= 0) back(sq, sv, pin);
        rsos_stamp(trace, wave, b / NY, 3, 40);
        pb_ = b;
        ppi_ = pi;
        pslot_ = sslot;
        ypend = ycur;
        ycur += (uint64_t)(16 * NY) * sizeof(TO);
        sslot += NY % NS;
        if (sslot >= NS) sslot -= NS;
        pi = pi2;
        gi = gi2;
        slot += NY;
        if (slot >= NX) slot -= NX;
    };
    int cur = 0;
    auto last_back = [&]() __attribute__((always_inline)) {
        if (pb_ < 0) return;
        double sv[3];
        const int sq = flag_ld(f_sseq);
#pragma unroll
        for (int v = 0; v < 3; ++v) sv[v] = l.ss[pslot_ * 192 + v * 64 + lane];
        if (cur) back(sq, sv, payB);
        else back(sq, sv, payA);
    };
    if constexpr (CYC > 0) {
        const double SO_GLB* tab = (const double SO_GLB*)rfl64((int64_t)(uintptr_t)sh->tab);
        TapT treg[CYC][KS];
        int jec[CYC];
#pragma unroll
        for (int c = 0; c < CYC; ++c) {
            const int gc = (yi + c * NY) % ngroups;
            jec[c] = uni(sh->jend[gc]);
#pragma unroll
            for (int s = 0; s < KS; ++s) treg[c][s] = (TapT)tab[((size_t)gc * KS + s) * 64 + lane];
        }
        for (int b = yi; b < NB;) {
#pragma unroll
            for (int k = 0; k < 2 * CYC; ++k) {
                if (b < NB) {
                    if ((k & 1) == 0) block(b, treg[k % CYC], payA, payB, jec[k % CYC], jec[(k + 1) % CYC]);
                    else block(b, treg[k % CYC], payB, payA, jec[k % CYC], jec[(k + 1) % CYC]);
                    cur = (k & 1) ^ 1;
                }
                b += NY;
            }
        }
        last_back();
        if constexpr (SO_RSOS_COUNT) {
            if (lane == 0) {
                rsos_count_out(trace, wave, 0, 0, cnt_in);
                rsos_count_out(trace, wave, 0, 1, cnt_in_b);
                rsos_count_out(trace, wave, 0, 2, cnt_st);
                rsos_count_out(trace, wave, 0, 3, cnt_st_b);
                rsos_count_out(trace, wave, 0, 4, clock64() - cyc0);
            }
        }
    } else if constexpr (!F32M) {
        for (int b = yi; b < NB; b += NY) {
            double at[KS];
            const SO_LDS double* tp = l.taps + gi * KS * 64 + lane;
#pragma unroll
            for (int s = 0; s < KS; ++s) at[s] = tp[s * 64];
            int gn = gi + NY;
            while (gn >= ngroups) gn -= ngroups;
            const int je = uni(sh->jend[gi]), jn = uni(sh->jend[gn]);
            if (cur == 0) block(b, at, payA, payB, je, jn);
            else block(b, at, payB, payA, je, jn);
            cur ^= 1;
        }
        last_back();
    }
}


constexpr int rsos_nthreads(int nw) { return (nw == 17 ? 16 : nw) * 64; }
template <int KS, int NW, typename TO, int CYC>
__device__ __forceinline__ void rsos_body(const double* __restrict__ tab, const int* __restrict__ jend_g, const RsSos& g, TO* __restrict__ y,
                                          const RsGlobalTables& gsrc, int64_t G0, int64_t Gstep) {
    constexpr bool HW = NW == 17;
    constexpr int NT = rsos_nthreads(NW);
    constexpr int NY = NW >= 16 ? 10 : NW - 2, NL = NW == 16 ? 2 : 1, NX = 2 * NY + 1;
    extern __shared__ double lds_raw[];
    __shared__ RsosShared sh;
    const int wave = uni(threadIdx.x >> 6);
    rsos_stamp_pro(g.trace, 6);
    {
        if (threadIdx.x == 0) {
            sh.g = g;
            sh.gcar = gsrc.car;
            sh.gops = gsrc.ops;
            sh.gleaves = gsrc.leaves;
            sh.y = (void*)y;
            sh.tab = tab;
        }
    }
    if constexpr (CYC == 0)
        for (int i = threadIdx.x; i < g.ngroups * KS * 64; i += NT) lds_raw[i] = tab[i];
    for (int i = threadIdx.x; i < g.ngroups; i += NT) sh.jend[i] = jend_g[i];
    {
        const int* src = reinterpret_cast<const int*>(gsrc.ctl);
        int* dst = reinterpret_cast<int*>(&sh.ctl);
        for (int i = threadIdx.x; i < (int)(sizeof(RsCtl) / 4); i += NT) dst[i] = src[i];
    }
    const int64_t ncg = g.nch / g.ct;
    const int64_t ngrp = ncg * ((g.nranges + g.rgs - 1) / g.rgs);
    double* const ss = lds_raw + (CYC > 0 ? 0 : (size_t)g.ngroups * KS * 64) + (size_t)16 * g.rpitch + (size_t)NX * 192;
    const int ru = g.ct < 8 ? g.ct : 8;
    for (int64_t G = G0; G < ngrp; G += Gstep) {
        __syncthreads();
        if (threadIdx.x < kRsosFlags) sh.flags[threadIdx.x] = 0;
        if (threadIdx.x < 192) ss[threadIdx.x] = 0.0;
        if (threadIdx.x == 0) {
            const bool pj = NW != 16 && NW != 17 && rsos_wproj_group(sh, G);
            sh.proj = pj ? 1 : 0;
            sh.wpe = pj ? 0 : g.wp;
            if (pj) sh.flags[kRsosFlagSseq] = -1;
        }
        __syncthreads();
        const bool proj = sh.proj != 0;
        rsos_stamp_pro(g.trace, 7);
        if (wave == 0) {
            if (!(g.debug & 64)) {
                if (proj) rsos_wproj_chain<NY>(&sh, lds_raw, G);
                const int nk = (g.debug & 131072) ? 3 : (2 * g.nsec + 3) / 4;
                if (nk <= 1) rsos_chain<NY, 1>(&sh, lds_raw, G);
                else if (nk == 2) rsos_chain<NY, 2>(&sh, lds_raw, G);
                else rsos_chain<NY, 3>(&sh, lds_raw, G);
            }
        } else if (NW == 16 && (wave == 13 || wave == 14)) {
            if (!g.gsplit || (g.debug & 256) || g.src32) continue;
            const int q = wave - 13;
            if (g.arr2) {
                if constexpr (NL == 2) {
                    if (ru == 8) rsos_loader<NY, NL, 8, false, 0, 2, true>(&sh, lds_raw, G, q);
                    else if (ru == 4) rsos_loader<NY, NL, 4, false, 0, 2, true>(&sh, lds_raw, G, q);
                    else if (ru == 2) rsos_loader<NY, NL, 2, false, 0, 2, true>(&sh, lds_raw, G, q);
                }
            } else if (ru == 2) {
                if (g.rpitch == 770) rsos_loader<NY, NL, 2, false, 770 * 8, 2>(&sh, lds_raw, G, q);
                else if (g.rpitch == 642) rsos_loader<NY, NL, 2, false, 642 * 8, 2>(&sh, lds_raw, G, q);
                else rsos_loader<NY, NL, 2, false, 0, 2>(&sh, lds_raw, G, q);
            } else if (ru == 4) {
                if (g.rpitch == 770) rsos_loader<NY, NL, 4, false, 770 * 8, 2>(&sh, lds_raw, G, q);
                else if (g.rpitch == 642) rsos_loader<NY, NL, 4, false, 642 * 8, 2>(&sh, lds_raw, G, q);
                else rsos_loader<NY, NL, 4, false, 0, 2>(&sh, lds_raw, G, q);
            }
        } else if (wave == 4 || (NW == 16 && wave == 8)) {
            const int q = wave == 4 ? 0 : 1;
            if (g.debug & 256) continue;
            if (NW == 16 && g.gsplit && !g.src32 && ru == 8 && g.arr2) {
                rsos_loader<NY, NL, 8, false, 0, 1>(&sh, lds_raw, G, q);
                continue;
            }
            if (NW == 16 && g.gsplit && !g.src32 && (ru == 2 || ru == 4)) {
                if (ru == 2) {
                    if (g.rpitch == 770) rsos_loader<NY, NL, 2, false, 770 * 8, 1>(&sh, lds_raw, G, q);
                    else if (g.rpitch == 642) rsos_loader<NY, NL, 2, false, 642 * 8, 1>(&sh, lds_raw, G, q);
                    else rsos_loader<NY, NL, 2, false, 0, 1>(&sh, lds_raw, G, q);
                } else {
                    if (g.rpitch == 770) rsos_loader<NY, NL, 4, false, 770 * 8, 1>(&sh, lds_raw, G, q);
                    else if (g.rpitch == 642) rsos_loader<NY, NL, 4, false, 642 * 8, 1>(&sh, lds_raw, G, q);
                    else rsos_loader<NY, NL, 4, false, 0, 1>(&sh, lds_raw, G, q);
                }
                continue;
            }
            switch (ru) {
            case 8:
                if (g.src32 && g.rpitch == 770) rsos_loader<NY, NL, 8, true, 770 * 8>(&sh, lds_raw, G, q);
                else if (g.src32 && g.rpitch == 642) rsos_loader<NY, NL, 8, true, 642 * 8>(&sh, lds_raw, G, q);
                else if (g.src32) rsos_loader<NY, NL, 8, true>(&sh, lds_raw, G, q);
                else if (g.rpitch == 770) rsos_loader<NY, NL, 8, false, 770 * 8>(&sh, lds_raw, G, q);
                else if (g.rpitch == 642) rsos_loader<NY, NL, 8, false, 642 * 8>(&sh, lds_raw, G, q);
                else rsos_loader<NY, NL, 8, false>(&sh, lds_raw, G, q);
                break;
            case 4:
                if (g.src32) rsos_loader<NY, NL, 4, true>(&sh, lds_raw, G, q);
                else if (g.rpitch == 770) rsos_loader<NY, NL, 4, false, 770 * 8>(&sh, lds_raw, G, q);
                else if (g.rpitch == 642) rsos_loader<NY, NL, 4, false, 642 * 8>(&sh, lds_raw, G, q);
                else rsos_loader<NY, NL, 4, false>(&sh, lds_raw, G, q);
                break;
            case 2:
                if (g.src32) rsos_loader<NY, NL, 2, true>(&sh, lds_raw, G, q);
                else if (g.rpitch == 770) rsos_loader<NY, NL, 2, false, 770 * 8>(&sh, lds_raw, G, q);
                else if (g.rpitch == 642) rsos_loader<NY, NL, 2, false, 642 * 8>(&sh, lds_raw, G, q);
                else rsos_loader<NY, NL, 2, false>(&sh, lds_raw, G, q);
                break;
            default:
                if (g.src32) rsos_loader<NY, NL, 1, true>(&sh, lds_raw, G, q);
                else rsos_loader<NY, NL, 1, false>(&sh, lds_raw, G, q);
                break;
            }
        } else if (HW && wave == 12) {
            if (g.help && !(g.debug & 128)) rsos_helper<NY>(&sh, lds_raw);
        } else if (!(g.debug & 128))
            {
            if (NW >= 16 && wave > 12) continue;
            const int yi = NW == 16 ? (wave < 4 ? wave - 1 : wave < 8 ? wave - 2 : wave < 12 ? wave - 3 : 9) : wave - (wave > 4 ? 2 : 1);
            if (proj) rsos_wproj_y<NY>(&sh, lds_raw, G, yi);
            if constexpr (sizeof(TO) == 4 && CYC > 0) {
                if (g.f32m) {
                    rsos_ywave<KS, NY, NL, TO, CYC, true, HW>(&sh, lds_raw, G, yi);
                    continue;
                }
            }
            rsos_ywave<KS, NY, NL, TO, CYC, false, HW>(&sh, lds_raw, G, yi);
        }
    }
}

template <int KS, int NW, typename TO, int CYC>
__global__ __launch_bounds__(rsos_nthreads(NW)) void k_rsos(const double* __restrict__ tab, const int* __restrict__ jend_g, RsSos g,
                                                  TO* __restrict__ y, RsGlobalTables gsrc) {
    rsos_body<KS, NW, TO, CYC>(tab, jend_g, g, y, gsrc, (int64_t)blockIdx.x, (int64_t)gridDim.x);
}

template <int KS, int NW, typename TO, int CYC>
__global__ __launch_bounds__(rsos_nthreads(NW)) void k_rsos_batch(const RsosItem* __restrict__ items, int gpm) {
    const int it = (int)(blockIdx.x / (unsigned)gpm);
    const RsosItem I = items[it];
    rsos_body<KS, NW, TO, CYC>(I.tab, I.jend, I.g, (TO*)I.y, I.gsrc, (int64_t)(blockIdx.x % (unsigned)gpm), (int64_t)gpm);
}

constexpr size_t kRsosStaticLds = sizeof(RsosShared) + 64;

#if SO_RSOS_ONLY_KS != 0
template <int KS, int NW, typename TO, int CYC>
static void launch_rsos_k(const double* tab, const int* jend, const RsSos& g, void* y, const RsGlobalTables& gsrc, int grid, hipStream_t st) {
    const size_t lds = rsos_lds_bytes(g.ngroups, KS, g.rpitch, NW, CYC);
    static bool seen[64];
    if (first_use_on_device(seen))
        (void)hipFuncSetAttribute((const void*)k_rsos<KS, NW, TO, CYC>, hipFuncAttributeMaxDynamicSharedMemorySize, (int)rsos_lds_budget());
    hipLaunchKernelGGL((k_rsos<KS, NW, TO, CYC>), dim3((unsigned)grid), dim3(rsos_nthreads(NW)), lds, st, tab, jend, g, (TO*)y, gsrc);
}

template <int KS, int NW, typename TO>
static void launch_rsos_batch_k(const RsosItem* items, int nitems, int gpm, const RsSos& g0, hipStream_t st) {
    const size_t lds = rsos_lds_bytes(g0.ngroups, KS, g0.rpitch, NW, 1);
    static bool seen[64];
    if (first_use_on_device(seen))
        (void)hipFuncSetAttribute((const void*)k_rsos_batch<KS, NW, TO, 1>, hipFuncAttributeMaxDynamicSharedMemorySize, (int)rsos_lds_budget());
    hipLaunchKernelGGL((k_rsos_batch<KS, NW, TO, 1>), dim3((unsigned)(nitems * gpm)), dim3(rsos_nthreads(NW)), lds, st, items, gpm);
}

template <int KS, typename TO>
static int launch_rsos_t(const double* tab, const int* jend, const RsSos& g, void* y, const RsGlobalTables& gsrc, int grid, hipStream_t st) {
    if constexpr (SO_RSOS_ONLY_NW == 0 || SO_RSOS_ONLY_NW == 12) if (g.nwaves == 12) {
        switch (g.cyc) {
        case 0: launch_rsos_k<KS, 12, TO, 0>(tab, jend, g, y, gsrc, grid, st); return 0;
        case 1: launch_rsos_k<KS, 12, TO, 1>(tab, jend, g, y, gsrc, grid, st); return 0;
        case 2:
            if constexpr (KS <= 16) {
                launch_rsos_k<KS, 12, TO, 2>(tab, jend, g, y, gsrc, grid, st);
                return 0;
            }
            return -1;
        default: return -1;
        }
    }
    if constexpr (SO_RSOS_ONLY_NW == 0 || SO_RSOS_ONLY_NW == 16) if (g.nwaves == 16) {
        if (g.cyc != 1) return -1;
        launch_rsos_k<KS, 16, TO, 1>(tab, jend, g, y, gsrc, grid, st);
        return 0;
    }
    if constexpr (SO_RSOS_ONLY_NW == 0 || SO_RSOS_ONLY_NW == 17) if (g.nwaves == 17) {
        if (g.cyc != 1) return -1;
        launch_rsos_k<KS, 17, TO, 1>(tab, jend, g, y, gsrc, grid, st);
        return 0;
    }
    if constexpr (SO_RSOS_ONLY_NW == 0 || SO_RSOS_ONLY_NW == 8) if (g.nwaves == 8) {
        switch (g.cyc) {
        case 0: launch_rsos_k<KS, 8, TO, 0>(tab, jend, g, y, gsrc, grid, st); return 0;
        case 1: launch_rsos_k<KS, 8, TO, 1>(tab, jend, g, y, gsrc, grid, st); return 0;
        case 2: launch_rsos_k<KS, 8, TO, 2>(tab, jend, g, y, gsrc, grid, st); return 0;
        case 3:
            if constexpr (KS <= 20) {
                launch_rsos_k<KS, 8, TO, 3>(tab, jend, g, y, gsrc, grid, st);
                return 0;
            }
            return -1;
        case 5:
            if constexpr (KS <= 16) {
                launch_rsos_k<KS, 8, TO, 5>(tab, jend, g, y, gsrc, grid, st);
                return 0;
            }
            return -1;
        default: return -1;
        }
    }
    return -1;
}
#endif

#define SO_RSOS_ARGS const double *tab, const int *jend, const RsSos &g, void *y, const RsGlobalTables &gsrc, int grid, hipStream_t st
#if SO_RSOS_ONLY_KS > 0
#define SO_RSOS_CAT2(a, b) a##b
#define SO_RSOS_CAT(a, b) SO_RSOS_CAT2(a, b)
#if SO_RSOS_ONLY_F32
#define SO_RSOS_TAG f
#define SO_RSOS_TO float
#else
#define SO_RSOS_TAG d
#define SO_RSOS_TO double
#endif
int SO_RSOS_CAT(SO_RSOS_CAT(SO_RSOS_CAT(launch_rsos_ks, SO_RSOS_ONLY_KS), SO_RSOS_TAG), SO_RSOS_ONLY_NW)(SO_RSOS_ARGS) {
    return launch_rsos_t<SO_RSOS_ONLY_KS, SO_RSOS_TO>(tab, jend, g, y, gsrc, grid, st);
}
#if SO_RSOS_ONLY_KS == 4 && (SO_RSOS_ONLY_NW == 12 || SO_RSOS_ONLY_NW == 16)
int SO_RSOS_CAT(SO_RSOS_CAT(launch_rsos_batch4, SO_RSOS_TAG), SO_RSOS_ONLY_NW)(const RsosItem* items, int nitems, int gpm, const RsSos& g0, hipStream_t st) {
    launch_rsos_batch_k<4, SO_RSOS_ONLY_NW, SO_RSOS_TO>(items, nitems, gpm, g0, st);
    return 0;
}
#endif
#else
size_t rsos_lds_bytes(int ngroups, int ks, int rpitch, int nwaves, int cyc) {
    const int ny = nwaves >= 16 ? 10 : nwaves - 2, nx = 2 * ny + 1;
    return ((cyc > 0 ? 0 : (size_t)ngroups * ks * 64) + (size_t)16 * rpitch + (size_t)nx * 192 + (size_t)rsos_nss(ny) * 192 + 16 * 16 * 2 +
            (nwaves == 17 ? 3 * kRsosHslots * 64 : 0)) * 8;
}
size_t rsos_lds_budget() { return 160 * 1024 - kRsosStaticLds; }

#if SO_RSOS_ONLY_KS == 0
#define SO_RS(KS_) \
    int launch_rsos_ks##KS_##d12(SO_RSOS_ARGS); int launch_rsos_ks##KS_##d16(SO_RSOS_ARGS); int launch_rsos_ks##KS_##d8(SO_RSOS_ARGS); \
    int launch_rsos_ks##KS_##f12(SO_RSOS_ARGS); int launch_rsos_ks##KS_##f16(SO_RSOS_ARGS); int launch_rsos_ks##KS_##f8(SO_RSOS_ARGS); \
    int launch_rsos_ks##KS_##d17(SO_RSOS_ARGS); int launch_rsos_ks##KS_##f17(SO_RSOS_ARGS);
SO_RS(4) SO_RS(12) SO_RS(13) SO_RS(14) SO_RS(16) SO_RS(20)
#undef SO_RS
#endif
#if SO_RSOS_ONLY_KS == 0
int launch_rsos_batch4d12(const RsosItem*, int, int, const RsSos&, hipStream_t);
int launch_rsos_batch4f12(const RsosItem*, int, int, const RsSos&, hipStream_t);
int launch_rsos_batch4d16(const RsosItem*, int, int, const RsSos&, hipStream_t);
int launch_rsos_batch4f16(const RsosItem*, int, int, const RsSos&, hipStream_t);
#endif
int launch_rsos_batch(const RsosItem* items, int nitems, int gpm, const RsSos& g0, hipStream_t st) {
    if (nitems <= 0 || gpm <= 0) return 0;
    if (g0.ks != 4 || g0.cyc != 1 || (g0.nwaves != 12 && g0.nwaves != 16)) return -1;
#if SO_RSOS_ONLY_KS == 0
    if (g0.nwaves == 12) return g0.out_f32 ? launch_rsos_batch4f12(items, nitems, gpm, g0, st) : launch_rsos_batch4d12(items, nitems, gpm, g0, st);
    return g0.out_f32 ? launch_rsos_batch4f16(items, nitems, gpm, g0, st) : launch_rsos_batch4d16(items, nitems, gpm, g0, st);
#else
    if (g0.nwaves == 12) {
        if (g0.out_f32) launch_rsos_batch_k<4, 12, float>(items, nitems, gpm, g0, st);
        else launch_rsos_batch_k<4, 12, double>(items, nitems, gpm, g0, st);
    } else {
        if (g0.out_f32) launch_rsos_batch_k<4, 16, float>(items, nitems, gpm, g0, st);
        else launch_rsos_batch_k<4, 16, double>(items, nitems, gpm, g0, st);
    }
    return 0;
#endif
}

int launch_rsos(SO_RSOS_ARGS) {
    if (g.n_out <= 0) return 0;
    if (g.ngroups > kRsosMaxGroups) return -1;
#if SO_RSOS_ONLY_KS == 0
#define SO_RS(KS_) \
    if (g.ks == KS_) {                                                                                                             \
        if (g.nwaves == 12) return g.out_f32 ? launch_rsos_ks##KS_##f12(tab, jend, g, y, gsrc, grid, st) : launch_rsos_ks##KS_##d12(tab, jend, g, y, gsrc, grid, st); \
        if (g.nwaves == 16) return g.out_f32 ? launch_rsos_ks##KS_##f16(tab, jend, g, y, gsrc, grid, st) : launch_rsos_ks##KS_##d16(tab, jend, g, y, gsrc, grid, st); \
        if (g.nwaves == 8) return g.out_f32 ? launch_rsos_ks##KS_##f8(tab, jend, g, y, gsrc, grid, st) : launch_rsos_ks##KS_##d8(tab, jend, g, y, gsrc, grid, st);    \
        if (g.nwaves == 17) return g.out_f32 ? launch_rsos_ks##KS_##f17(tab, jend, g, y, gsrc, grid, st) : launch_rsos_ks##KS_##d17(tab, jend, g, y, gsrc, grid, st); \
        return -1;                                                                                                                 \
    }
#else
#define SO_RS(KS_) \
// ... 10 lines not shown
```

signaloperators.jl_amd/csrc/plan.h:

```cpp
#pragma once
#include <cstdint>
#include <string>
#include <vector>

#include "../../include/sigops.h"

namespace so {

int design_iir(int type, double f1, double f2, double fs, int method, int order, double ripple,
               std::vector<double>& sos, double& gain, std::string& err);
int design_iir_zpk(int type, double f1, double f2, double fs, int method, int order, double ripple,
                   std::vector<double>& z, std::vector<double>& p, double& k, std::string& err);
int zpk_to_sos(const double* z, int nz, const double* p, int np, double k, std::vector<double>& sos, double& gain,
               std::string& err);
int tf_to_sos(const double* b, int nb, const double* a, int na, std::vector<double>& sos, double& gain, double& resid,
              std::string& err);
int tf_zero_input(const double* b, int nb, const double* a, int na, const double* si0, int nsi, double* out, int64_t cap,
                  int64_t& used, std::string& err);
int design_resample_rational(int64_t num, int64_t den, std::vector<double>& h, std::string& err);
int design_resample_arbitrary(double rate, int nphi, std::vector<double>& h, std::string& err);

void rsos_wproj_matrix_sos(const double* sos, int nsec, double gain, const double* tab, const int* jend, int ngroups, int kw, int64_t M, int wp,
                           std::vector<double>& V, int& j0, int& K);
int resample_positions(double fs_in, double fs_out, double rate, int nphi, const double* h, int hlen,
                       int64_t n_out, int64_t* j, int32_t* p, double* alpha, int64_t* nfix, int64_t* nbaked);

int rtc_compile_check(const std::string& body, std::string& err);
void rtc_wait_idle();
void rtc_shutdown();

struct Plan;
Plan* plan_create(const so_node_t* nodes, int32_t n_nodes, int32_t root, const so_out_desc_t* out,
                  int32_t device, int& status, std::string& err);
int plan_execute(Plan* p, void* out, void* stream, std::string& err);
int plan_check(Plan* p, void* stream, std::string& err);
int plan_set_array(Plan* p, int32_t node_index, const void* data, std::string& err);
int64_t plan_nframes(const Plan* p);
void plan_stats(const Plan* p, so_stats_t* st);
void plan_set_profiling(Plan* p, int mode);
int64_t plan_counter(const Plan* p, int which);
int plan_step_info(const Plan* p, int index, so_step_info_t* info);
void plan_destroy(Plan* p);

}
```

signaloperators.jl_amd/csrc/sigops_internal.h:

```cpp
#pragma once
#include <cstdint>

namespace so {

enum OpCode : int32_t {
    OP_CONST = 0,
    OP_LOAD = 1,
    OP_SCALAR = 2,
    OP_FUNC = 3,
    OP_RAMP = 4,
    OP_ADD = 5,
    OP_SUB = 6,
    OP_MUL = 7,
    OP_DIV = 8,
    OP_NEG = 9,
    OP_ROUND32 = 10,
    OP_STOREF = 11,
    OP_LOADF = 12
};

enum LeafMode : int32_t { LM_PLAIN = 0, LM_CYCLE = 1, LM_MIRROR = 2 };

struct DOp {
    int32_t code;
// ... 141 lines not shown
struct RsGeom {
    int64_t n_in, n_out;
    int64_t m0;
    int64_t j0;
    int64_t L, M;
    double delta, c0;
    int64_t c0i;
    int32_t arbitrary;
    int32_t exact;
    int32_t nphi, taps, nch;
    int32_t in_dtype, out_dtype;
    int64_t in_pitch, out_pitch;
};

struct RsTiled {
    RsGeom g;
    int32_t ct;
    int32_t tile_out;
    int32_t tile_in;
    int32_t pitch;
    int64_t ntiles;
    int32_t pair;
    int32_t pad_;
};

struct RsArb {
    RsGeom g;
    int32_t ct;
    int32_t nc;
    int32_t ringf;
    int32_t zrows;
    int32_t nranges;
    int32_t dma_ok, vec_out, depth, debug;
    int32_t no, pad_;
    int64_t bpr;
    int64_t nbatches;
    uint32_t* err;
};

struct RsFix {
    int64_t m;
    int64_t j;
    int32_t p;
    int32_t pad;
    double alpha;
};
struct RsFixArgs {
    const RsFix* fix;
    int64_t nfix;
    const double* pfb;
    const double* dpfb;
    int64_t n_in;
    int32_t taps, nch;
    int32_t stage_dtype;
    int32_t out_dtype;
    const DCarrier* car;
    const DOp* ops;
    const DLeaf* leaves;
    int32_t ncar, in_dtype;
    const void* x;
    int64_t in_pitch;
    void* y;
    int64_t out_pitch;
};

struct RsPeriodic {
    int64_t n_in, n_out;
    int64_t L, M;
    int64_t nperiods;
    int32_t pt, ct;
    int32_t rows;
    int32_t f32m;
    int32_t ngroups;
    int32_t kw;
    int32_t tile_len;
    int32_t lds_pitch;
    int32_t jlo;
    int32_t nch;
    int32_t vec_ok;
    int32_t nwaves;
    int32_t ptshift;
    int32_t ncompute;
    int32_t grid;
    int32_t pad;
    int32_t nslots;
    int32_t fslots;
    int32_t fpitch;
    int32_t nload;
    int32_t ftwo;
    int32_t out_f32;
    int32_t ga;
    int32_t arr2;
    int32_t nstate, ksw;
    const double* wtab;
    double* vper;
    int64_t in_pitch, out_pitch;
    long long* trace;
    uint32_t* nf;
};
constexpr int kRsTraceIters = 48, kRsTraceStamps = 8;
constexpr uint32_t kRsNfCap = 2047;

struct RsPerFixup {
    RsPeriodic g;
    const double* tab;
    const int* jend;
    const int* jrel;
    int32_t taps, out_f32;
    RsGlobalTables gsrc;
    void* y;
};
constexpr int kRsTwoBases = 128;
constexpr int kRsTwoDoubles = 128 + 2 * 2 * kRsTwoBases;

struct RsSos {
    int64_t n_in, n_out;
    int64_t L, M;
    int64_t pr;
    int32_t wp;
    int32_t nranges;
    int32_t ngroups;
    int32_t ks;
    int32_t ulo;
    int32_t ct, rgs;
    int32_t nch;
    int32_t nwaves;
    int32_t ring;
    int32_t rpitch;
    int32_t chunk;
    int32_t depth;
    int32_t nsec;
    int32_t fuse;
    int32_t fuse_sine;
    int32_t out_f32;
    int32_t src32;
    int32_t ring32;
    int32_t x32;
    int32_t f32m;
    int32_t sring;
    int32_t gsplit;
    int32_t help;
    int32_t debug;
    int32_t cyc;
    int32_t arr2;
    int32_t wproj;
    int32_t wk;
    int32_t wj0;
    int64_t out_pitch;
    int64_t store_lo;
    const double* mats;
    int32_t* bad;
    long long* trace;
    uint32_t* err;
};
constexpr int kRsosTraceIters = 96;

struct RsosItem {
    RsSos g;
    const double* tab;
    const int* jend;
    void* y;
    RsGlobalTables gsrc;
};

struct RsFixup {
    RsSos g;
    const double* tab;
    const int* jend;
    const int* jrel;
    int32_t taps;
    int32_t rearm;
    SosCoefs cf;
    RsGlobalTables gsrc;
    void* y;
};

struct RsRows {
    int64_t n_in, n_out;
    int64_t L, M;
    int64_t nperiods;
    int32_t taps;
    int32_t ct, pb;
    int32_t jlo;
    int32_t tile_len;
    int32_t pitch;
    int32_t nch;
    int32_t debug;
    int32_t kw, ngroups, pbshift;
    int32_t threads;
    int64_t in_pitch, out_pitch;
};

}
```

signaloperators.jl_amd/csrc/stages.cpp:

```cpp
#include "plan_impl.h"

namespace so {

static int env_int(const char* name, int dflt) {
    const char* ev = std::getenv(name);
    return ev ? std::atoi(ev) : dflt;
}

constexpr size_t kRsLdsAvail = 160 * 1024 - sizeof(RsCtl) - 64;

static int channels_per_group(int nch, int max) {
    if (max >= 16 && nch % 16 == 0) return 16;
    for (int c : {8, 4, 2})
        if (nch % c == 0) return c;
    return 1;
}


struct Tap {
    double hv, dv;
};
static Tap tap(const double* h, int hlen, int nphi, int p, int64_t age) {
    const int64_t hi = p + (int64_t)nphi * age;
    return {hi < hlen ? h[hi] : 0.0, hi + 1 < hlen ? h[hi + 1] - h[hi] : 0.0};
// ... 1506 lines not shown
    const size_t leaves_before = leaves.size();
    for (size_t i = 0; i < cs.size(); ++i) {
        DCarrier& c = cs[i];
        std::vector<DOp>& fcode = fcodes[i];
        int dmax = 2;
        c.nslots = (int)monos_all[i].size();
        for (size_t k = 0; k < monos_all[i].size(); ++k) {
            int ei = monos_all[i][k], r32 = 0;
            for (;;) {
                const Expr& ex = exprs[ei];
                if (ex.op == E_RETYPE) ei = ex.a;
                else if (ex.op == E_ROUND32) { r32 = 0x100; ei = ex.a; }
                else if (ex.op == E_ADD && is_const(ex.a, 0.0)) ei = ex.b;
                else if ((ex.op == E_ADD || ex.op == E_SUB) && is_const(ex.b, 0.0)) ei = ex.a;
                else break;
            }
            const int eop = exprs[ei].op;
            const int kind = eop == E_CONST ? OP_CONST : eop == E_SCALAR ? OP_SCALAR : eop == E_FUNC ? OP_FUNC : eop == E_RAMP ? OP_RAMP : -1;
            if (kind < 0) {
                leaves.resize(leaves_before);
                leaf_array_node.resize(leaves_before);
                { if (std::getenv("SIGOPS_DEBUG_PLAN")) std::fprintf(stderr, "[sigops] carrier fusion rejected (#%d)\n", 5); return false; }
            }
            c.slot_leaf[k] = add_leaf(exprs[ei]);
            c.slot_kind[k] = kind | r32;
            leafset.insert(c.slot_leaf[k]);
            std::map<int, int> none;
            gen(monos_all[i][k], fcode, none, fcode, false);
            fcode.push_back(DOp{OP_STOREF, (int)k});
            dmax = std::max(dmax, depth(monos_all[i][k]));
        }
        c.depth = dmax;
        nops_total += fcode.size();
        for (auto& o : fcode)
            if (o.code <= OP_RAMP) leafset.insert(o.arg);
        if (dmax > 2 || nops_total > (size_t)kCtlOps || leafset.size() > (size_t)kCtlLeaves) {
            leaves.resize(leaves_before);
            leaf_array_node.resize(leaves_before);
            { if (std::getenv("SIGOPS_DEBUG_PLAN")) std::fprintf(stderr, "[sigops] carrier fusion rejected (#%d)\n", 6); return false; }
        }
    }
    for (size_t i = 0; i < cs.size(); ++i) {
        cs[i].frame_pc = (int)ops.size();
        cs[i].frame_len = (int)fcodes[i].size();
        ops.insert(ops.end(), fcodes[i].begin(), fcodes[i].end());
    }
    if (ga) {
        auto same_leaf = [&](int a, int b) {
            const DLeaf &x = leaves[a], &y = leaves[b];
            return x.base == y.base && x.fstride == y.fstride && x.cstride == y.cstride && x.df == y.df && x.dc == y.dc &&
                   x.modn == y.modn && x.v0 == y.v0 && x.v1 == y.v1 && x.v2 == y.v2 && x.sf == y.sf && x.sc == y.sc &&
                   x.dtype == y.dtype && x.mode == y.mode && x.flag == y.flag && x.buf == y.buf;
        };
        for (size_t i = 1; i < cs.size(); ++i)
            if (cs[i].slot_kind[0] != cs[0].slot_kind[0] || !same_leaf(cs[i].slot_leaf[0], cs[0].slot_leaf[0])) ga = false;
        if (!ga) {
            leaves.resize(leaves_before);
            leaf_array_node.resize(leaves_before);
            ops.resize(ops.size() - nops_total);
            if (std::getenv("SIGOPS_DEBUG_PLAN")) std::fprintf(stderr, "[sigops] carrier fusion rejected (#%d)\n", 7);
            return false;
        }
        for (size_t i = 0; i < cs.size(); ++i) {
            cs[i].pad_ = (i == 0 ? 1 : 2) + (ga_add ? 2 : 0);
            cs[i].nsteps = 0;
            cs[i].dtype = SO_F32;
        }
    }
    out = cs;
    return true;
}

RsCtl Plan::make_ctl(const Stage& S) const {
    RsCtl ctl{};
    std::map<int, int> leafmap;
    for (const DCarrier& c0 : S.carriers) {
        if (ctl.ncar >= kCtlCar) throw PlanError{SO_ERR_RUNTIME, "internal: carrier control block overflow"};
        DCarrier c = c0;
        c.frame_pc = ctl.nops;
        for (int k = 0; k < c0.frame_len; ++k) {
            DOp o = ops[c0.frame_pc + k];
            if (o.code <= OP_RAMP) {
                auto it = leafmap.find(o.arg);
                if (it == leafmap.end()) {
                    if (ctl.nleaves >= kCtlLeaves) throw PlanError{SO_ERR_RUNTIME, "internal: leaf control block overflow"};
                    ctl.leaves[ctl.nleaves] = leaves[o.arg];
                    if (o.code == OP_SCALAR) ctl.leaves[ctl.nleaves].flag = 0;
                    it = leafmap.emplace(o.arg, ctl.nleaves++).first;
                }
                o.arg = it->second;
            }
            if (ctl.nops >= kCtlOps) throw PlanError{SO_ERR_RUNTIME, "internal: op control block overflow"};
            ctl.ops[ctl.nops++] = o;
        }
        for (int k = 0; k < c0.nslots; ++k) {
            auto it = leafmap.find(c0.slot_leaf[k]);
            if (it == leafmap.end()) {
                if (ctl.nleaves >= kCtlLeaves) throw PlanError{SO_ERR_RUNTIME, "internal: leaf control block overflow"};
                ctl.leaves[ctl.nleaves] = leaves[c0.slot_leaf[k]];
                if ((c0.slot_kind[k] & 0xff) == OP_SCALAR) ctl.leaves[ctl.nleaves].flag = 0;
                it = leafmap.emplace(c0.slot_leaf[k], ctl.nleaves++).first;
            }
            c.slot_leaf[k] = it->second;
        }
        ctl.car[ctl.ncar++] = c;
    }
    return ctl;
}


void Plan::batch_sos_stages() {
    if (std::getenv("SIGOPS_SOS_NOBATCH")) return;
    std::map<std::pair<int, int>, std::vector<int>> kinds;
    std::vector<int> order;
    for (size_t i = 0; i < stages.size(); ++i)
        if (stages[i].need > 0) order.push_back((int)i);
    std::sort(order.begin(), order.end(), [&](int a, int b) { return stages[a].node < stages[b].node; });
    for (int sid : order) {
        const Stage& S = stages[sid];
        if (S.kind != ST_SOS || S.onepass || S.sg.exact || S.xscan || S.under_norm || S.pre_stage >= 0 || S.groups.size() != 1 ||
            S.in_array_node < 0 || S.pw_step >= 0 || S.sg.nchunks < 1 || S.rsos_src >= 0)
            continue;
        kinds[{S.groups[0].nsec, nodes[S.node].dtype}].push_back(sid);
    }
    for (auto& kv : kinds) {
        if (kv.second.size() < 2) continue;
        SosBatch B;
        B.members = kv.second;
        B.nsec = kv.first.first;
        B.dtype = kv.first.second;
        int64_t chans = 0;
        for (int sid : B.members) chans += stages[sid].sg.nch;
        if (!std::getenv("SIGOPS_SOS_BATCH_KEEPCHUNKS"))
            for (int sid : B.members) {
                Stage& S = stages[sid];
                sos_chunking(sid, S.sg.n, S.sg.nch, nodes[S.node].dtype, S.groups, false, std::max<int64_t>(1, kSosSequences / chans));
            }
        B.desc_buf = raw_buf((B.members.size() + 1) * sizeof(SosDesc));
        {
            int off = 0;
            for (int sid : B.members) {
                B.bad_off.push_back(off);
                off += stages[sid].sg.nch;
            }
            B.bad_buf = raw_buf((size_t)std::max(off, 1) * 4);
        }
        for (int sid : B.members) stages[sid].batch = (int)batches.size();
        if (std::getenv("SIGOPS_DEBUG_PLAN"))
            std::fprintf(stderr, "[sigops] %zu IIR stages of %d sections share their launches\n", B.members.size(), B.nsec);
        batches.push_back(std::move(B));
    }
}

static void rsos_block_columns(const SosCoefs& cf, std::vector<double>& Tm, std::vector<double>& Cm, std::vector<double>& Dm, std::vector<double>& Am) {
    const int ns = cf.nsec, D = 2 * ns, B = 16;
    Tm.assign(B * B, 0.0);
    Cm.assign(B * 12, 0.0);
    Dm.assign(12 * B, 0.0);
    Am.assign(12 * 12, 0.0);
    for (int col = 0; col < B + D; ++col) {
        std::vector<double> st(D, 0.0);
        if (col >= B) st[col - B] = 1.0;
        for (int t = 0; t < B; ++t) {
            double v = col == t ? 1.0 : 0.0;
            for (int f = 0; f < ns; ++f) {
                const double xi = v;
                v = st[2 * f] + cf.b0[f] * xi;
                st[2 * f] = st[2 * f + 1] + cf.b1[f] * xi - cf.a1[f] * v;
                st[2 * f + 1] = cf.b2[f] * xi - cf.a2[f] * v;
            }
            v *= cf.gain;
            if (col < B) Tm[t * B + col] = v;
            else Cm[t * 12 + (col - B)] = v;
        }
        for (int d = 0; d < D; ++d) {
            if (col < B) Dm[d * B + col] = st[d];
            else Am[d * 12 + (col - B)] = st[d];
        }
    }
}

static void rsos_block_matrices(const SosCoefs& cf, std::vector<double>& mats) {
    const int B = 16;
    std::vector<double> Tm, Cm, Dm, Am;
    rsos_block_columns(cf, Tm, Cm, Dm, Am);
    mats.assign((size_t)14 * 64, 0.0);
    for (int lane = 0; lane < 64; ++lane) {
        const int i = lane & 15, kq = lane >> 4;
        for (int v = 0; v < 4; ++v) {
            const int k = 4 * v + kq;
            mats[(size_t)(0 + v) * 64 + lane] = i < 12 ? Dm[i * B + k] : 0.0;
            mats[(size_t)(7 + v) * 64 + lane] = Tm[i * B + k];
            if (v < 3) {
                mats[(size_t)(4 + v) * 64 + lane] = i < 12 ? Am[i * 12 + k] : 0.0;
                mats[(size_t)(11 + v) * 64 + lane] = Cm[i * 12 + k];
            }
        }
    }
}

static void rsos_wproj_matrix(const SosCoefs& cf, const double* tab, const int* jend, int ngroups, int kw, int64_t M, int wp, std::vector<double>& V,
                       int& j0, int& K) {
    std::vector<double> Tm, Cm, Dm, Am;
    rsos_block_columns(cf, Tm, Cm, Dm, Am);
    int64_t lo = INT64_MAX, hi = INT64_MIN;
    for (int p = 0; p < wp; p += std::max(1, wp - 1))
        for (int gi = 0; gi < ngroups; ++gi) {
            const int64_t o = (int64_t)p * M + jend[gi] - (kw - 1);
            lo = std::min(lo, o);
            hi = std::max(hi, o + kw - 1);
        }
    j0 = (int)lo;
    K = (int)(hi - lo + 1);
    std::vector<long double> acc((size_t)12 * K, 0.0L), P(12 * 16), Q(12 * 16);
    for (int i = 0; i < 12 * 16; ++i) P[i] = Dm[i];
    for (int64_t b = (int64_t)wp * ngroups - 1; b >= 0; --b) {
        const int gi = (int)(b % ngroups);
        const int64_t o0 = (b / ngroups) * M + jend[gi] - (kw - 1) - lo;
        for (int kk = 0; kk < kw; ++kk) {
            const double* tp = tab + ((size_t)gi * kw + kk) * 16;
            for (int d = 0; d < 12; ++d) {
                long double a = 0.0L;
                for (int t = 0; t < 16; ++t) a += P[d * 16 + t] * (long double)tp[t];
                acc[(size_t)d * K + o0 + kk] += a;
            }
        }
        if (b == 0) break;
        for (int d = 0; d < 12; ++d)
            for (int t = 0; t < 16; ++t) {
                long double a = 0.0L;
                for (int e = 0; e < 12; ++e) a += (long double)Am[d * 12 + e] * P[e * 16 + t];
                Q[d * 16 + t] = a;
            }
        P.swap(Q);
    }
    V.resize(acc.size());
    for (size_t i = 0; i < acc.size(); ++i) V[i] = (double)acc[i];
}

void rsos_wproj_matrix_sos(const double* sos, int nsec, double gain, const double* tab, const int* jend, int ngroups, int kw, int64_t M, int wp,
                           std::vector<double>& V, int& j0, int& K) {
    SosCoefs cf{};
    cf.nsec = nsec;
    cf.gain = gain;
    for (int f = 0; f < nsec; ++f) {
        cf.b0[f] = sos[6 * f + 0];
        cf.b1[f] = sos[6 * f + 1];
        cf.b2[f] = sos[6 * f + 2];
        cf.a1[f] = sos[6 * f + 4];
        cf.a2[f] = sos[6 * f + 5];
    }
    rsos_wproj_matrix(cf, tab, jend, ngroups, kw, M, wp, V, j0, K);
}


static int64_t warmup_periods(const SosCoefs& cf, int64_t L, double tol) {
    const int D = 2 * cf.nsec;
    int64_t wp = 1;
    const Mat P = matpow(sos_state_matrix(cf), L, D);
    Mat cur = P;
    while (!(maxabs(cur) < tol) && wp < 1000000 && std::isfinite(maxabs(cur))) {
        cur = matmul(cur, P, D);
        ++wp;
    }
    return maxabs(cur) < tol ? wp : 0;
}

struct RsosRanges {
    int ct = 1, rgs = 16;
    int64_t ncg = 0, nranges = 0, pr = 0, ngrp = 0;
};
static bool rsos_ranges(int nch, int64_t nperiods, int64_t min_pr, int gpm, int cus, int64_t align_M, RsosRanges& R) {
    R.ct = channels_per_group(nch, 16);
    R.rgs = 16 / R.ct;
    R.ncg = nch / R.ct;
    if (gpm > 0 && R.ncg > gpm) return false;
    const int64_t rgroups = gpm > 0 ? gpm / R.ncg : std::max<int64_t>(1, cus / R.ncg);
    int64_t nranges = rgroups * R.rgs;
    if (nperiods / nranges < min_pr) nranges = std::max<int64_t>(R.rgs, nperiods / min_pr / R.rgs * R.rgs);
    if (const char* ev = std::getenv("SIGOPS_RSOS_RANGES"))
        if (gpm == 0) nranges = std::max<int64_t>(1, std::atoll(ev));
    R.pr = (nperiods + nranges - 1) / nranges;
    if (align_M > 0 && R.ct < 8 && !std::getenv("SIGOPS_RSOS_NOALIGNPR")) {
        const int64_t mlt = 16 / std::__gcd<int64_t>(align_M % 16 == 0 ? 16 : align_M % 16, 16);
        if (R.pr % mlt != 0 && R.pr >= 8 * mlt) R.pr = (R.pr + mlt - 1) / mlt * mlt;
    }
    R.nranges = (nperiods + R.pr - 1) / R.pr;
    R.ngrp = R.ncg * ((R.nranges + R.rgs - 1) / R.rgs);
    return true;
}

static int rsos_ring_frames(const RsSos& g) {
    int ring = 4096;
    while (ring >= 128 && rsos_lds_bytes(g.ngroups, g.ks, ring + 2, g.nwaves, g.cyc) > rsos_lds_budget()) ring -= 128;
    if (const char* ev = std::getenv("SIGOPS_RSOS_RING")) ring = std::min(ring, std::max(128, std::atoi(ev) / 128 * 128));
    return ring;
}

void Plan::rsos_fuse_step(const DCarrier& c0, bool two_arrays, RsSos& g) const {
    g.fuse = -1;
    if (two_arrays) {
        g.fuse = c0.op[0] == OP_MUL ? 0 : c0.op[0] == OP_ADD ? 1 : ((c0.arg[0] & 0x100) ? 3 : 2);
        g.fuse_sine = 0;
        g.arr2 = 1;
    } else if (c0.nsteps == 1 && (c0.arg[0] & 0x2ff) == 0 && c0.nslots >= 1 &&
               (c0.op[0] == OP_MUL || c0.op[0] == OP_ADD || c0.op[0] == OP_SUB)) {
        g.fuse = c0.op[0] == OP_MUL ? 0 : c0.op[0] == OP_ADD ? 1 : ((c0.arg[0] & 0x100) ? 3 : 2);
        const DLeaf& L0 = leaves[c0.slot_leaf[0]];
        const int kind = c0.slot_kind[0];
        if (kind == OP_FUNC && L0.mode == SO_FN_SIN && L0.sf == 1) g.fuse_sine = 1;
        else if (kind == OP_CONST || kind == OP_SCALAR) g.fuse_sine = 0;
        else g.fuse = -2;
    } else if (c0.nsteps > 0)
        g.fuse = -2;
}

struct RsosFusion : RsosRanges {
    Plan& P;
    std::vector<Node>& nodes;
    std::vector<Stage>& stages;
    std::vector<DLeaf>& leaves;
    const size_t i2;
    const int i3;
    Stage &S2, &S3;
    const RsPeriodic& rp;
    const bool pure32;
    struct AltGuard {
        Stage& S;
        std::vector<DCarrier> car;
        int pw;
        bool armed;
        ~AltGuard() {
            if (armed) {
                S.carriers = car;
                S.pw_step = pw;
            }
        }
    } alt;
    bool two_arrays = false, plain_src = false, was_ga = false, own_tab = false, blocks_ok = false;
    int64_t Lp, Mp;
    int ngp, kwp, jlop, ks = 0;
    std::vector<double> own_taps;
    std::vector<int> own_jend;
    std::vector<int64_t> own_jr;
    int nch = 0, cus = 0;
    int64_t need = 0, L = 0, store_lo = 0, wp = 0;
    RsSos g{};
    RsosFusion(Plan& P_, size_t i2_, int i3_)
        : P(P_), nodes(P_.nodes), stages(P_.stages), leaves(P_.leaves), i2(i2_), i3(i3_), S2(P_.stages[i2_]), S3(P_.stages[i3_]), rp(S3.rp),
          pure32(nodes[S2.node].dtype == SO_F32), alt{S3, S3.carriers, S3.pw_step, false}, Lp(rp.L), Mp(rp.M), ngp(rp.ngroups), kwp(rp.kw), jlop(rp.jlo) {}

    bool source_form() {
        if (!rp.arr2 && !S3.alt_carriers.empty() && S3.pw_step >= 0 && S3.in_buf >= 0 && !std::getenv("SIGOPS_RSOS_NO_ARR2")) {
            S3.carriers = S3.alt_carriers;
            S3.pw_step = -1;
            alt.armed = true;
        }
        if (rp.arr2 || alt.armed) {
            const bool ok = !pure32 && nodes[S2.node].dtype == SO_F64 && S3.carriers.size() == 1 && S3.carriers[0].nsteps == 1 &&
                            (S3.carriers[0].arg[0] & kCarArr2) && !(S3.carriers[0].arg[0] & 0x200) && S3.carriers[0].dtype == SO_F64 &&
                            S3.carriers[0].dtype2 == SO_F64 && nodes[S2.node].nch % 2 == 0 &&
                            (S3.carriers[0].op[0] == OP_ADD || S3.carriers[0].op[0] == OP_SUB || S3.carriers[0].op[0] == OP_MUL) &&
                            !std::getenv("SIGOPS_RSOS_NO_ARR2");
            if (!ok) return false;
            two_arrays = true;
        }
        if (pure32) {
            bool plain = nodes[nodes[S3.node].kids[0]].dtype == SO_F32 && rp.ga == 0;
            for (auto& c : S3.carriers)
                if (c.nsteps != 0 || c.pad_ != 0 || c.dtype != SO_F32) plain = false;
            if (!plain) return false;
        }
        plain_src = S3.carriers.empty() && (S3.in_buf >= 0 || S3.in_array_node >= 0);
        return !S3.carriers.empty() || plain_src;
    }

    bool own_table() {
        blocks_ok = S3.periodic && Lp > 0 && Lp % 16 == 0 && (int64_t)ngp * 16 == Lp && ngp <= 256;
        if (!S3.rg.arbitrary && (!blocks_ok || ngp > 10) && !std::getenv("SIGOPS_RSOS_NOOWNTAB")) {
            const RsGeom& rg = S3.rg;
            const so_node_t& nd3 = nodes[S3.node].nd;
            const double* h = (const double*)nd3.p0;
            const int hlen = nd3.i2;
            const int64_t tmin = 16 / std::__gcd<int64_t>(rg.L, 16);
            for (int64_t m : {1, 2, 3, 5}) {
                const int64_t Ls = rg.L * tmin * m, Ms = rg.M * tmin * m;
                const int ng = (int)(Ls / 16);
                if (Ls > 4096 || (ng != 1 && ng != 2 && ng != 3 && ng != 5 && ng != 6 && ng != 10)) continue;
                PeriodPos pos = period_positions(rg, Ls, nullptr);
                const std::vector<int64_t>& jr = pos.j;
                GroupWindows win = group_windows(jr, Ls);
                std::vector<int>& jend = win.jend;
                const int64_t maxspan = win.maxspan;
                const int ksneed = (int)((rg.taps + maxspan + 3) / 4);
                int ksc = 0;
                for (int k : {12, 14, 16, 20})
                    if (!ksc && k >= ksneed) ksc = k;
                if (std::getenv("SIGOPS_DEBUG_PLAN"))
                    std::fprintf(stderr, "[sigops] k_rsos own taps: L %lld M %lld x %lld -> %d blocks, taps %d span %lld: %d k-steps (%d)\n",
                                 (long long)rg.L, (long long)rg.M, (long long)(tmin * m), ng, rg.taps, (long long)maxspan, ksneed, ksc);
                if (!ksc) break;
                const int kw = 4 * ksc;
                const int jlo = aligned_window_start(jend[0], kw);
                std::vector<double> tab = fill_tap_blocks(jr, Ls, jend, kw, rg.taps, [&](int64_t r, int64_t age) { return tap(h, hlen, rg.nphi, pos.p[(size_t)r], age).hv; });
                Lp = Ls;
                Mp = Ms;
                ngp = ng;
                kwp = kw;
                jlop = jlo;
                own_taps.swap(tab);
                own_jend.swap(jend);
                own_jr.swap(pos.j);
                own_tab = true;
                break;
            }
        }
        if (!own_tab && (!blocks_ok || !S3.periodic)) return false;
        return S3.base % Lp == 0 && Mp < (1 << 20);
    }

    bool trim_table() {
        if (!own_tab && !std::getenv("SIGOPS_RSOS_NOTRIM") && !S3.tab_host.empty() && (size_t)ngp * kwp * 16 == S3.tab_host.size()) {
            int lead = kwp;
            for (int gi = 0; gi < ngp && lead > 0; ++gi)
                for (int kk = 0; kk < lead; ++kk) {
                    bool z = true;
                    for (int rr = 0; rr < 16 && z; ++rr) z = S3.tab_host[((size_t)gi * kwp + kk) * 16 + rr] == 0.0;
                    if (!z) {
                        lead = kk;
                        break;
                    }
                }
            int ksc = 0;
            for (int k : {12, 13, 14, 16, 20})
                if (!ksc && 4 * k >= kwp - lead) ksc = k;
            if (ksc && 4 * ksc < kwp) {
                const int drop = kwp - 4 * ksc, kw = 4 * ksc;
                own_taps.assign((size_t)ngp * kw * 16, 0.0);
                for (int gi = 0; gi < ngp; ++gi)
                    for (int kk = 0; kk < kw; ++kk)
                        for (int rr = 0; rr < 16; ++rr)
                            own_taps[((size_t)gi * kw + kk) * 16 + rr] = S3.tab_host[((size_t)gi * kwp + kk + drop) * 16 + rr];
                own_jend = S3.jend_host;
                kwp = kw;
                own_tab = true;
                if (std::getenv("SIGOPS_DEBUG_PLAN"))
                    std::fprintf(stderr, "[sigops] k_rsos: %d leading zero slots in every group's window: %d k-steps instead of %d\n", lead, ksc,
                                 (kw + drop) / 4);
            }
        }
        ks = kwp / 4;
        return ks == 12 || ks == 13 || ks == 14 || ks == 16 || ks == 20;
    }

    bool sole_reader() {
        bool ok = true;
        was_ga = rp.ga != 0;
        for (auto& c : S3.carriers)
            if ((c.pad_ != 0) != was_ga) ok = false;
        if (was_ga && std::getenv("SIGOPS_RSOS_NO32")) ok = false;
        for (auto& L : leaves)
            if (L.buf == S2.in_buf) ok = false;
        for (size_t j = 0; j < stages.size(); ++j) {
            if (j != i2 && stages[j].in_buf == S2.in_buf) ok = false;
            if (j != i2)
                for (auto& c : stages[j].carriers)
                    if (c.buf == S2.in_buf) ok = false;
        }
        return ok;
    }

    bool warmup_and_ranges() {
        const SosCoefs& cf = S2.groups[0];
        nch = nodes[S2.node].nch;
        need = S2.need - S3.base, L = Lp;
        store_lo = S2.base - S3.base;
        const int64_t nperiods = (need + L - 1) / L;
        const double wtol = std::ldexp(1.0, -std::abs(env_int("SIGOPS_RSOS_WTOL", S2.under_norm ? 70 : 56)));
        wp = warmup_periods(cf, L, wtol);
        if (!wp) return false;
        cus = env_int("SIGOPS_RSOS_GRID", 256);
        rsos_ranges(nch, nperiods, std::max<int64_t>(1, wp), 0, cus, Mp, *this);
        return (pr + wp) * ngp < (1 << 30) && (pr + wp) * Mp < ((int64_t)1 << 30);
    }

    bool worth_it() const {
        if (const char* ev = std::getenv("SIGOPS_RSOS_MINGROUPS")) {
            if (ngrp < std::atoll(ev)) return false;
        } else {
            const double unit_cost = ct >= 8 ? 1.0 : ct == 4 ? 1.1 : ct == 2 ? 1.15 : 3.2;
            bool wpj = !std::getenv("SIGOPS_RSOS_NOWPROJ") && !std::getenv("SIGOPS_RSOS_NWAVES") && nodes[S2.node].dtype == SO_F64 && !two_arrays && !was_ga &&
                       ct >= 8 && wp * Mp + kwp <= 16384;
            if (wpj && plain_src) wpj = S3.in_array_node >= 0 && nodes[nodes[S3.node].kids[0]].dtype != SO_F32;
            else if (wpj) {
                const DCarrier& c0 = S3.carriers[0];
                const bool sine = c0.nsteps == 1 && (c0.arg[0] & 0x2ff) == 0 && c0.nslots >= 1 && (c0.op[0] == OP_ADD || (c0.op[0] == OP_SUB && !(c0.arg[0] & 0x100))) &&
                                  c0.slot_kind[0] == OP_FUNC && leaves[c0.slot_leaf[0]].mode == SO_FN_SIN && leaves[c0.slot_leaf[0]].sf == 1;
                wpj = c0.dtype == SO_F64 && c0.array_node >= 0 && (c0.nsteps == 0 || sine);
            }
            const double t_pro = wpj ? 0.013 * (double)(wp * Mp + kwp) : 0.0;
            const double t_fused = (double)((ngrp + cus - 1) / cus) * ((double)((pr + (wpj ? 0 : wp)) * ngp) * 0.30 * unit_cost * (ks + 14) / 28.0 + t_pro) + 15.0;
            const double t_two = 8.0e-6 * (double)need * nch + 95.0;
            if (std::getenv("SIGOPS_DEBUG_PLAN"))
                std::fprintf(stderr, "[sigops] k_rsos estimate: fused %.0f us (%lld groups, %lld + %lld periods), two kernels %.0f us\n", t_fused,
                             (long long)ngrp, (long long)pr, (long long)wp, t_two);
            if (t_fused > t_two) return false;
        }
        return true;
    }

    bool waves() {
        const SosCoefs& cf = S2.groups[0];
        g.n_in = S3.rg.n_in;
        g.n_out = need;
        g.store_lo = store_lo;
        g.L = L;
        g.M = Mp;
        g.pr = pr;
        g.wp = (int32_t)wp;
        g.nranges = (int32_t)nranges;
        g.ngroups = ngp;
        g.ks = ks;
        g.ulo = jlop;
        g.ct = ct;
        g.rgs = rgs;
        g.nch = nch;
        g.chunk = env_int("SIGOPS_RSOS_CHUNK", 128) == 64 ? 64 : 128;
        g.depth = std::max(1, std::min(4, env_int("SIGOPS_RSOS_DEPTH", 4)));
        g.nsec = cf.nsec;
        g.debug = env_int("SIGOPS_RSOS_DEBUG", 0);
        {
            auto cyc_of = [&](int nw) { return g.ngroups / std::__gcd(nw >= 16 ? 10 : nw - 2, g.ngroups); };
            auto fits = [&](int nw) {
                const int c = cyc_of(nw);
                return nw == 12 ? ((c == 1 || c == 2) && c * ks <= 32) : ((c == 1 || c == 2 || c == 3 || c == 5) && c * ks <= 80);
            };
            int nw = fits(12) ? 12 : fits(8) ? 8 : 12;
            const bool stepped = was_ga || (!plain_src && !S3.carriers.empty() && S3.carriers[0].nsteps > 0);
            if ((ct == 2 || (ct == 4 && !was_ga && nodes[S2.node].dtype == SO_F64 && !std::getenv("SIGOPS_RSOS_NOGSPLIT"))) && stepped && nw == 12 &&
                cyc_of(16) == 1 && ks <= 16)
                nw = 16;
            if (const char* ev = std::getenv("SIGOPS_RSOS_NWAVES")) nw = std::atoi(ev) == 8 ? 8 : (std::atoi(ev) == 16 || std::atoi(ev) == 17) && cyc_of(16) == 1 && ks <= 16 ? std::atoi(ev) : 12;
            if (two_arrays) {
                if (!(cyc_of(16) == 1 && ks <= 16)) return false;
                nw = 16;
            }
            g.nwaves = nw;
            g.cyc = (nw >= 16 || fits(nw)) && !std::getenv("SIGOPS_RSOS_LDSTAPS") ? cyc_of(nw) : 0;
            const bool inst = nw == 12 ? (g.cyc == 0 || g.cyc == 1 || (g.cyc == 2 && ks <= 16))
                            : nw >= 16 ? g.cyc == 1
                                       : (g.cyc == 0 || g.cyc == 1 || g.cyc == 2 || (g.cyc == 3 && ks <= 20) || (g.cyc == 5 && ks <= 16));
            return inst;
        }
    }

    bool ring() {
        {
            const int ny = g.nwaves >= 16 ? 10 : g.nwaves - 2;
            const int64_t span = (int64_t)(2 * ny - 1) * ((16 * Mp + L - 1) / L + 1) + kwp + 16 + 2 * g.chunk;
            const int ring = rsos_ring_frames(g);
            if (std::getenv("SIGOPS_DEBUG_PLAN"))
                std::fprintf(stderr, "[sigops] k_rsos: ring %d frames (needs %lld), LDS %zu of %zu\n", ring, (long long)span,
                             rsos_lds_bytes(g.ngroups, ks, ring + 2, g.nwaves, g.cyc), rsos_lds_budget());
            if (ring < 128 || ring < span) return false;
            g.ring = ring;
            g.rpitch = ring + 2;
        }
        return true;
    }

    void rewrite_carriers() {
        if (plain_src) {
            S3.carriers.push_back(default_carrier(S3, S3.in_frames, nodes[nodes[S3.node].kids[0]].dtype == SO_F32 ? SO_F32 : SO_F64, nch));
            S3.car_buf = P.raw_buf(sizeof(DCarrier));
            S3.ctl_buf = P.raw_buf(sizeof(RsCtl));
        }
        if (was_ga) {
            for (size_t i = 0; i < S3.carriers.size(); ++i) {
                DCarrier& c = S3.carriers[i];
                c.pad_ = 0;
                c.nsteps = 1;
                if (i > 0) c.dtype = SO_F64;
            }
            S3.rp.ga = 0;
            g.src32 = 1;
        } else
            g.src32 = S3.carriers[0].dtype == SO_F32 && S3.carriers[0].nsteps == 0 ? 1 : 0;
        g.x32 = pure32 ? 1 : 0;
        P.rsos_fuse_step(S3.carriers[0], two_arrays, g);
        g.gsplit = g.nwaves == 16 && !g.src32 && g.fuse >= 0 && (g.arr2 || ((ct == 2 || ct == 4) && !std::getenv("SIGOPS_RSOS_NOGSPLIT"))) ? 1 : 0;
        g.ring32 = g.src32 && g.fuse == -1 && pure32 && !std::getenv("SIGOPS_RSOS_NO_RING32") ? 1 : 0;
        g.help = g.nwaves == 17 ? 1 : 0;
        g.f32m = g.src32 && g.fuse >= -1 && g.cyc > 0 && !std::getenv("SIGOPS_RSOS_NO_F32MFMA") && !std::getenv("SIGOPS_RSOS_NO_RING32") ? 1 : 0;
    }

    void commit() {
        const SosCoefs& cf = S2.groups[0];
        S2.rs = g;
        S2.rsos_src = i3;
        S2.carriers.clear();
        {
            const std::vector<int64_t>& jr = own_jr.empty() ? S3.per_j : own_jr;
            const std::vector<int>& je = own_tab ? own_jend : S3.jend_host;
            S2.rsos_jrel_host.clear();
            if ((int64_t)jr.size() >= Lp && (int64_t)je.size() >= ngp) {
                S2.rsos_jrel_host.resize((size_t)Lp);
                for (int64_t r = 0; r < Lp; ++r) S2.rsos_jrel_host[(size_t)r] = (int)(jr[(size_t)r] - je[(size_t)(r / 16)]);
                S2.rsos_jrel_buf = P.raw_buf(S2.rsos_jrel_host.size() * 4);
                S2.rsos_taps = S3.rg.taps;
            }
        }
        if (own_tab) {
            S2.rsos_tab_host.swap(own_taps);
            S2.rsos_jend_host.swap(own_jend);
            S2.rsos_tab_buf = P.raw_buf(S2.rsos_tab_host.size() * 8);
            S2.rsos_jend_buf = P.raw_buf(S2.rsos_jend_host.size() * 4);
        }
        S2.rsos_grid = (int)std::min<int64_t>(ngrp, cus);
        rsos_block_matrices(cf, S2.rsos_mats_host);
    }

    void wproj_tables() {
        const SosCoefs& cf = S2.groups[0];
        {
            const std::vector<double>& tb = own_tab ? S2.rsos_tab_host : S3.tab_host;
            const std::vector<int>& je = own_tab ? S2.rsos_jend_host : S3.jend_host;
            const DCarrier& c0 = S3.carriers[0];
            const bool form = g.fuse == -1 || ((g.fuse == 1 || g.fuse == 2) && g.fuse_sine);
            S2.rs.wproj = 0;
            if (!std::getenv("SIGOPS_RSOS_NOWPROJ") && nodes[S2.node].dtype == SO_F64 && !two_arrays && !g.src32 && !g.ring32 && !g.f32m &&
                !g.gsplit && !g.help && (g.nwaves == 12 || g.nwaves == 8) && ct >= 8 && form && c0.dtype == SO_F64 && c0.array_node >= 0 &&
                tb.size() == (size_t)ngp * kwp * 16 && (int)je.size() >= ngp && wp * Mp + kwp <= 16384) {
                std::vector<double> V;
                int j0 = 0, K = 0;
                rsos_wproj_matrix(cf, tb.data(), je.data(), ngp, kwp, Mp, (int)wp, V, j0, K);
                const int K8 = (K + 7) / 8 * 8;
                std::vector<double>& mt = S2.rsos_mats_host;
                mt.resize((size_t)14 * 64 + (size_t)K8 / 4 * 64 + 32, 0.0);
                for (int ksx = 0; ksx < K8 / 4; ++ksx)
                    for (int lane = 0; lane < 64; ++lane) {
                        const int i = lane & 15, f = 8 * (ksx >> 1) + 2 * (lane >> 4) + (ksx & 1);
                        mt[(size_t)14 * 64 + (size_t)ksx * 64 + lane] = i < 12 && f < K ? V[(size_t)i * K + f] : 0.0;
                    }
                if (g.fuse >= 0) {
                    const DLeaf& L0 = leaves[c0.slot_leaf[0]];
                    const long double wc = L0.flag ? (long double)L0.v0 / (long double)L0.v2 : 1.0L / (long double)L0.v2;
                    long double vs[12] = {}, vc[12] = {};
                    for (int f = 0; f < K; ++f) {
                        long double ph = wc * f;
                        ph -= floorl(ph);
                        const long double sn = sinl(2.0L * 3.141592653589793238462643383279502884L * ph);
                        const long double cs = cosl(2.0L * 3.141592653589793238462643383279502884L * ph);
                        for (int i = 0; i < 12; ++i) {
                            vs[i] += (long double)V[(size_t)i * K + f] * sn;
                            vc[i] += (long double)V[(size_t)i * K + f] * cs;
                        }
                    }
                    for (int i = 0; i < 12; ++i) {
                        mt[(size_t)14 * 64 + (size_t)K8 / 4 * 64 + i] = (double)vs[i];
                        mt[(size_t)14 * 64 + (size_t)K8 / 4 * 64 + 16 + i] = (double)vc[i];
                    }
                }
                S2.rs.wproj = 1;
                S2.rs.wk = K;
                S2.rs.wj0 = j0;
                if (std::getenv("SIGOPS_DEBUG_PLAN"))
                    std::fprintf(stderr, "[sigops] k_rsos: warm-up as one product: %d frames from %d (%d k-steps instead of %lld blocks)\n", K, j0, K8 / 4,
                                 (long long)(wp * ngp));
            }
        }
    }

    void commit_launch() {
        S2.rsos_mats_buf = P.raw_buf(S2.rsos_mats_host.size() * 8);
        if (S2.bad_buf < 0) S2.bad_buf = P.raw_buf((size_t)nch * 8);
        S3.fused_away = true;
        if (alt.armed) {
            alt.armed = false;
            P.bufs[S3.in_buf].bytes = 0;
        }
        if (std::getenv("SIGOPS_DEBUG_PLAN"))
            std::fprintf(stderr,
                         "[sigops] resampler + IIR fused (k_rsos): %lld ranges of %lld periods (+%lld warm-up), %lld groups of %d ch x %d ranges, "
                         "ks=%d ring=%d chunk=%d waves=%d cyc=%d fuse=%d/%d\n",
                         (long long)nranges, (long long)pr, (long long)wp, (long long)ngrp, ct, rgs, ks, g.ring, g.chunk, g.nwaves, g.cyc,
                         g.fuse, g.fuse_sine);
    }
};

void Plan::fuse_resample_sos() {
    if (std::getenv("SIGOPS_NO_RSOS")) return;
    for (size_t i2 = 0; i2 < stages.size(); ++i2) {
        Stage& S2 = stages[i2];
        if (S2.kind != ST_SOS || S2.onepass || S2.need <= 0 || S2.groups.size() != 1 || S2.groups[0].nsec > 6 ||
            S2.in_buf < 0 || S2.in_array_node >= 0 || S2.in_offset != S2.base || S2.pw_step >= 0 || S2.sg.exact || (S2.xscan && !S2.under_norm) ||
            (S2.under_norm && (S2.norm_df != 0 || S2.base != 0 || std::getenv("SIGOPS_NORM_EXACT_FILT"))) || S2.src_op || S2.batch >= 0 || S2.pre_stage >= 0 ||
            (nodes[S2.node].dtype != SO_F64 && nodes[S2.node].dtype != SO_F32) || S2.in_frames != S2.need - S2.base)
            continue;
        const bool pure32 = nodes[S2.node].dtype == SO_F32;
        if (pure32 && std::getenv("SIGOPS_RSOS_NO32")) continue;
        if (S2.base > 0 && std::getenv("SIGOPS_RSOS_NOWINDOWS")) continue;
        int i3 = -1;
        for (size_t j = 0; j < stages.size(); ++j)
            if (stages[j].kind == ST_RESAMPLE && stages[j].out_buf == S2.in_buf) i3 = (int)j;
        if (i3 < 0 || i3 == alias_stage || stages[i3].win_off >= 0) continue;
        Stage& S3 = stages[i3];
        const RsPeriodic& rp = S3.rp;
        if (S3.base > S2.base) continue;
        if (rp.nstate || nodes[S3.node].dtype != nodes[S2.node].dtype || !S3.fix_host.empty() || S3.need < S2.need || (int)S3.carriers.size() > kCtlCar)
            continue;
        RsosFusion F(*this, i2, i3);
        if (!F.source_form() || !F.own_table() || !F.trim_table() || !F.sole_reader() || !F.warmup_and_ranges() || !F.worth_it() || !F.waves() ||
            !F.ring())
            continue;
        F.rewrite_carriers();
        F.commit();
        F.wproj_tables();
        F.commit_launch();
    }
}

struct PlainRsos {
    Plan& P;
    std::vector<Node>& nodes;
    std::vector<Stage>& stages;
    const int cus;
    bool fit(size_t i2, int gpm, RsSos& g, double& cost) const {
        Stage& S2 = stages[i2];
        const int dt = nodes[S2.node].dtype;
        if (dt != SO_F64 && dt != SO_F32) return false;
        const DCarrier& c0 = S2.carriers[0];
        const bool pure32 = dt == SO_F32;
        if (pure32 && (c0.nsteps != 0 || c0.dtype != SO_F32)) return false;
        if (!pure32 && c0.dtype != SO_F64) return false;
        const SosCoefs& cf = S2.groups[0];
        const int nch = nodes[S2.node].nch;
        const int64_t need = S2.need, L = 160;
        const int ngp = 10, ks = 4, kw = 16;
        const int64_t nperiods = (need + L - 1) / L;
        const int64_t wp = warmup_periods(cf, L, std::ldexp(1.0, -std::abs(env_int("SIGOPS_PLAIN_WTOL", 70))));
        if (!wp) return false;
        RsosRanges R;
        if (!rsos_ranges(nch, nperiods, std::max<int64_t>(1, 4 * wp), gpm, cus, 0, R)) return false;
        const int ct = R.ct, rgs = R.rgs;
        const int64_t pr = R.pr, nranges = R.nranges, ngrp = R.ngrp;
        if ((pr + wp) * ngp >= (1 << 30) || (pr + wp) * L >= ((int64_t)1 << 30)) return false;
        const bool stepped_few = (ct == 2 || ct == 4) && !pure32 && c0.nsteps == 1 && !std::getenv("SIGOPS_RSOS_NOGSPLIT");
        const int plain_nw = env_int("SIGOPS_PLAIN_NWAVES", stepped_few ? 16 : 12) == 16 ? 16 : 12;
        const double unit_cost = stepped_few && plain_nw == 16 ? (ct == 4 ? 1.16 : 1.22) : ct >= 8 ? 1.0 : ct == 4 ? 1.19 : ct == 2 ? 1.4 : 3.4;
        cost = (double)((pr + wp) * ngp) * 0.197 * unit_cost;
        if (gpm > 0) {
            cost *= (double)((ngrp + gpm - 1) / gpm);
        } else if (const char* ev = std::getenv("SIGOPS_RSOS_MINGROUPS")) {
            if (ngrp < std::atoll(ev)) return false;
        } else {
            const double t_fused = (double)((ngrp + cus - 1) / cus) * cost + 15.0;
            const double nsamp = (double)need * nch;
            const double t_three = (nsamp < 1e8 ? 4.4e-6 * nsamp + 25.0 : 3.4e-6 * nsamp + 110.0) * (pure32 ? 0.9 : 1.0) * (c0.nsteps > 0 ? 1.1 : 1.0) *
                                   (S2.under_norm ? 1.6 : 1.0);
            if (std::getenv("SIGOPS_DEBUG_PLAN"))
                std::fprintf(stderr, "[sigops] single-pass IIR estimate: %.0f us (%lld groups, %lld + %lld periods), three passes %.0f us\n", t_fused,
                             (long long)ngrp, (long long)pr, (long long)wp, t_three);
            if (t_fused > t_three) return false;
        }
        g = RsSos{};
        g.n_in = S2.in_frames;
        g.n_out = need;
        g.store_lo = 0;
        g.L = L;
        g.M = L;
        g.pr = pr;
        g.wp = (int32_t)wp;
        g.nranges = (int32_t)nranges;
        g.ngroups = ngp;
        g.ks = ks;
        g.ulo = 0;
        g.ct = ct;
        g.rgs = rgs;
        g.nch = nch;
        g.chunk = 128;
        g.depth = std::max(1, std::min(4, env_int("SIGOPS_RSOS_DEPTH", 4)));
        g.nsec = cf.nsec;
        g.debug = env_int("SIGOPS_RSOS_DEBUG", 0);
        g.nwaves = plain_nw;
        g.cyc = 1;
        {
            const int ny = 10;
            const int64_t span = (int64_t)(2 * ny - 1) * 17 + kw + 16 + 2 * g.chunk;
            const int ring = rsos_ring_frames(g);
            if (ring < 128 || ring < span) return false;
            g.ring = ring;
            g.rpitch = ring + 2;
        }
        g.help = 0;
        g.src32 = pure32 ? 1 : 0;
        g.x32 = pure32 ? 1 : 0;
        g.ring32 = pure32 && !std::getenv("SIGOPS_RSOS_NO_RING32") ? 1 : 0;
        g.gsplit = 0;
        P.rsos_fuse_step(c0, false, g);
        g.gsplit = g.nwaves == 16 && !g.src32 && g.fuse >= 0 && (ct == 2 || ct == 4) && !std::getenv("SIGOPS_RSOS_NOGSPLIT") ? 1 : 0;
        return true;
    }
    void commit(size_t i2, const RsSos& g) const {
        Stage& S2 = stages[i2];
        const int ngp = g.ngroups, kw = 16;
        const int64_t L = g.L;
        S2.rsos_tab_host.assign((size_t)ngp * kw * 16, 0.0);
        S2.rsos_jend_host.assign((size_t)ngp, 0);
        for (int gi = 0; gi < ngp; ++gi) {
            S2.rsos_jend_host[(size_t)gi] = 16 * gi + 15;
            for (int kk = 0; kk < kw; ++kk) S2.rsos_tab_host[((size_t)gi * kw + kk) * 16 + kk] = 1.0;
        }
        S2.rsos_tab_buf = P.raw_buf(S2.rsos_tab_host.size() * 8);
        S2.rsos_jend_buf = P.raw_buf(S2.rsos_jend_host.size() * 4);
        S2.rsos_jrel_host.resize((size_t)L);
        for (int64_t r = 0; r < L; ++r) S2.rsos_jrel_host[(size_t)r] = (int)(r % 16) - 15;
        S2.rsos_jrel_buf = P.raw_buf(S2.rsos_jrel_host.size() * 4);
        S2.rsos_taps = 1;
        S2.rs = g;
        S2.rsos_src = (int)i2;
        const int64_t ngrp = (int64_t)(g.nch / g.ct) * ((g.nranges + g.rgs - 1) / g.rgs);
        S2.rsos_grid = (int)std::min<int64_t>(ngrp, cus);
        rsos_block_matrices(S2.groups[0], S2.rsos_mats_host);
        S2.rsos_mats_buf = P.raw_buf(S2.rsos_mats_host.size() * 8);
        if (std::getenv("SIGOPS_DEBUG_PLAN"))
            std::fprintf(stderr, "[sigops] IIR in one pass (k_rsos, identity resampler%s): %lld ranges of %lld periods (+%d warm-up), %lld groups of %d ch x %d ranges, ring=%d fuse=%d/%d\n",
                         S2.rsb >= 0 ? ", batched" : "", (long long)g.nranges, (long long)g.pr, g.wp, (long long)ngrp, g.ct, g.rgs, g.ring, g.fuse, g.fuse_sine);
    }
};

void Plan::fuse_plain_sos() {
    if (std::getenv("SIGOPS_NO_RSOS") || std::getenv("SIGOPS_NO_PLAIN_RSOS")) return;
    const int cus = env_int("SIGOPS_RSOS_GRID", 256);
    const PlainRsos one{*this, nodes, stages, cus};
    int candidates = 0;
    for (auto& S : stages)
        if (S.kind == ST_SOS && S.rsos_src < 0 && S.carriers.size() == 1 && S.need > 0) ++candidates;
    std::vector<size_t> small;
    for (size_t i2 = 0; i2 < stages.size(); ++i2) {
        Stage& S2 = stages[i2];
        if (S2.kind != ST_SOS || S2.rsos_src >= 0 || S2.carriers.size() != 1 || S2.need <= 0 || S2.onepass || S2.sg.exact || (S2.xscan && !S2.under_norm) ||
            (S2.under_norm && S2.norm_df != 0) || S2.batch >= 0 || S2.pre_stage >= 0 || S2.base != 0 || S2.groups.size() != 1 || S2.groups[0].nsec > 6 || S2.pw_step >= 0)
            continue;
        if (candidates > 1 && (int64_t)S2.need * nodes[S2.node].nch < ((int64_t)1 << 26) && !std::getenv("SIGOPS_RSOS_MINGROUPS")) {
            small.push_back(i2);
            continue;
        }
        RsSos g{};
        double cost = 0.0;
        if (!one.fit(i2, 0, g, cost)) continue;
        one.commit(i2, g);
        if (S2.bad_buf < 0) S2.bad_buf = raw_buf((size_t)g.nch * 8);
    }
    const char* const want_s = std::getenv("SIGOPS_RSOS_BATCH");
    const int want = want_s && *want_s ? std::atoi(want_s) : -1;
    if (small.size() < 2 || want == 0) return;
    std::map<std::pair<int, int>, std::vector<size_t>> kinds;
    for (size_t i2 : small) {
        if ((int)i2 == alias_stage) continue;
        {
            const DCarrier& c0 = stages[i2].carriers[0];
            bool plain = c0.array_node >= 0 && c0.buf < 0;
            for (int k = 0; k < c0.nslots && plain; ++k)
                if (leaves[c0.slot_leaf[k]].buf >= 0) plain = false;
            if (!plain) continue;
        }
        RsSos g{};
        double cost = 0.0;
        if (!one.fit(i2, 1 << 20, g, cost)) continue;
        kinds[{nodes[stages[i2].node].dtype == SO_F32 ? 1 : 0, g.nwaves}].push_back(i2);
// ... 166 lines not shown
```

signaloperators.jl_amd/engine.py:

```python
import ctypes as C

import numpy as np

from . import _capi as K
from . import signals as S
from .lowering import lower, _DT

Array = np.ndarray


def process_sink_params(x):
    x = S._assignal(x)
    n = S.nframes(x)
    if n is None:
        S.error("Unknown number of frames in signal.")
    if S.isknowninf(n):
        S.error("Cannot store infinite signal.")
    return x


def _timeslice(x):
    if isinstance(x, S.ArraySig):
        return x.data
    d = _timeslice(x.signal)
    n = d.shape[0]
    L = x.resolvelen()
    if x.kind == "until":
        return d[: min(max(L, 0), n)]
    return d[min(max(L, 0), n):]


def _is_datacut(x):
    if isinstance(x, S.ArraySig):
        return True
    return isinstance(x, S.CutApply) and x.evaltrait == "data" and _is_datacut(x.signal)


def _root(x):
    if isinstance(x, S.ArraySig):
        if x.container is not None:
            return 2, x
        if S._is_torch(x.data):
            return 0, x
        return (1 if x.fs is None else 0), x
    best = None
    for c in getattr(x, "children", ()):
        r = _root(c)
        if best is None or r[0] > best[0]:
            best = r
    return best or (0, None)


def _refineroot(x):
    pr, leaf = _root(x)
    if pr == 2:
        return leaf.container
    if pr == 1:
        return Array
    return tuple


class Plan:

    def __init__(self, x, result_shape, result_dtype, strides, is_device, device=0, rng=None):
        self.lowered = lower(x, nframes_out=result_shape[0], rng=rng)
        self.desc = K.so_out_desc_t(dtype=_DT[np.dtype(result_dtype)], nch=result_shape[1],
                                    nframes=result_shape[0], frame_stride=strides[0],
                                    chan_stride=strides[1], is_device=1 if is_device else 0)
        self.handle = C.c_void_p()
        L = K.lib()
        st = L.so_plan_create(self.lowered.nodes, self.lowered.n, self.lowered.root,
                              C.byref(self.desc), device, C.byref(self.handle))
        if st != 0:
            raise S.ErrorException(K.last_error())

    def execute(self, out_ptr, stream=None):
        st = K.lib().so_plan_execute(self.handle, C.c_void_p(out_ptr), C.c_void_p(stream or 0))
        if st != 0:
            raise S.ErrorException(K.last_error())
        self._unchecked = (stream or 0) if self.desc.is_device else None

    def check(self, stream=None):
        self._unchecked = None
        st = K.lib().so_plan_check(self.handle, C.c_void_p(stream or 0))
        if st != 0:
            raise S.ErrorException(K.last_error())

    def set_array(self, k, data):
        idx, sig = self.lowered.array_nodes[k]
        if hasattr(data, "data_ptr"):
            ptr = data.data_ptr()
        else:
            ptr = data.ctypes.data
        self._keep_arrays = getattr(self, "_keep_arrays", {})
        self._keep_arrays[k] = data
        st = K.lib().so_plan_set_array(self.handle, idx, C.c_void_p(ptr))
        if st != 0:
            raise S.ErrorException(K.last_error())

    def set_profiling(self, on=True):
        K.lib().so_plan_set_profiling(self.handle, int(on))

    def stats(self):
        s = K.so_stats_t()
        K.lib().so_plan_stats(self.handle, C.byref(s))
        return {f[0]: (getattr(s, f[0]).decode() if f[0] == "dominant_kernel" else getattr(s, f[0]))
                for f in K.so_stats_t._fields_}

    def counters(self):
        L = K.lib()
        return {"graph_replays": L.so_plan_counter(self.handle, 0), "graph_captures": L.so_plan_counter(self.handle, 1),
                "direct_executes": L.so_plan_counter(self.handle, 2), "fused_mfmas_per_block": L.so_plan_counter(self.handle, 3),
                "wproj": L.so_plan_counter(self.handle, 4)}

    def rsos_geometry(self):
        L = K.lib()
        return {k: L.so_plan_counter(self.handle, i) for i, k in enumerate(("pr", "wp", "M", "wproj_frames", "wproj_first"), 5)}

    def steps(self):
        out = []
        info = K.so_step_info_t()
        n = K.lib().so_plan_step_info(self.handle, 0, C.byref(info))
        for i in range(n):
            K.lib().so_plan_step_info(self.handle, i, C.byref(info))
            out.append({"name": info.name.decode(), "algorithmic_bytes": info.algorithmic_bytes,
                        "ms": info.ms, "launches": info.launches})
        return out

    def close(self):
        if self.handle:
            err = None
            if getattr(self, "_unchecked", None) is not None:
                if K.lib().so_plan_check(self.handle, C.c_void_p(self._unchecked)) != 0:
                    err = K.last_error()
                self._unchecked = None
            K.lib().so_plan_destroy(self.handle)
            self.handle = C.c_void_p()
            if err is not None:
                raise S.ErrorException(err)

    def __del__(self):
        try:
            self.close()
        except Exception:
            pass


def _result_fields(result):
    if S._is_torch(result):
        shape = tuple(result.shape)
        st = result.stride()
        if len(shape) == 1:
            shape, st = (shape[0], 1), (st[0], 0)
        dt = {"torch.float32": S.F32, "torch.float64": S.F64}[str(result.dtype)]
        return shape, dt, st, result.is_cuda, result.data_ptr()
    shape = result.shape
    item = result.itemsize
    if result.ndim == 1:
        return (shape[0], 1), result.dtype, (result.strides[0] // item or 1, 0), False, result.ctypes.data
    return shape, result.dtype, (result.strides[0] // item or 1, result.strides[1] // item), False, \
        result.ctypes.data


def sink_into(result, x, *, device=0, rng=None, stream=None):
    x = S._assignal(x)
    shape, dt, strides, is_dev, ptr = _result_fields(result)
    n = S.nframes(x)
    if n is not None and not S.isknowninf(n) and n < shape[0]:
        S.error(f"Signal is too short to fill buffer of length {shape[0]}.")
    x = S.ToChannels(x, shape[1])
    plan = Plan(x, shape, dt, strides, is_dev, device=device, rng=rng)
    try:
        plan.execute(ptr, stream)
        if is_dev:
            plan.check(stream)
    finally:
        plan.close()
    return result


def sink(x, to=None, *, device=0, rng=None):
    if to is None and (isinstance(x, type) or x is tuple or (isinstance(x, str) and x == "torch")):
        to_ = x
        return S.Curried(lambda y: sink(y, to_, device=device, rng=rng))
    x = process_sink_params(x)
    if to is None:
        to = _refineroot(x)
    if _is_datacut(x) and to is Array:
        return _timeslice(x)
    n = S.nframes(x)
    dt = x.dtype
    if dt == S.I64:
        S.error("the HIP engine sinks Float32/Float64 signals only (SURVEY.md §8(b)); "
                "integer signals take the stock CPU sink")
    if to == "torch":
        import torch

        tdt = torch.float32 if dt == S.F32 else torch.float64
        res = torch.empty((x.nch, n), dtype=tdt, device=f"cuda:{device}").t()
        sink_into(res, x, device=device, rng=rng)
        return res, x.fs
    res = np.empty((n, x.nch), dtype=dt, order="F")
    sink_into(res, x, device=device, rng=rng)
    if isinstance(to, type) and hasattr(to, "initsink"):
        if x.fs is None:
            S.error("Unknown frame rate: array-type sinks carry a frame rate")
        return to.initsink(res, x.fs)
    return res if to is Array else (res, x.fs)


def stream(x, blocksize, to=None, *, device=0):
    from . import lowering as LW
    from .units import frames

    x = S._assignal(x)
    blocksize = int(blocksize)
    if blocksize <= 0:
        S.error("stream: blocksize must be positive")
    n = S.nframes(x)
    if n is None:
        S.error("Unknown number of frames in signal.")
    finite = not S.isknowninf(n)
    if to is None:
        to = _refineroot(x)
    cache = {"device": f"cuda:{device}"}
    pos = 0
    while not finite or pos < n:
        m = blocksize if not finite else min(blocksize, n - pos)
        blk = S.Until(S.After(x, pos * frames) if pos else x, m * frames)
        prev, LW._device_cache = LW._device_cache, cache
        try:
            res = sink(blk, to, device=device)
        finally:
            LW._device_cache = prev
        yield res
        pos += m


class BlockStream:

    def __init__(self, pipeline, fs, nch=1, dtype=np.float64, history=1 << 16, device=0):
        import torch

        from .units import inHz

        self.pipeline = pipeline
        self.fs = inHz(fs)
        self.nch = int(nch)
        self.dtype = np.dtype(dtype)
        self.tdt = torch.float32 if self.dtype == np.float32 else torch.float64
        self.history = int(history)
        self.device = device
        self.dev = f"cuda:{device}"
        self.cap = 0
        self.buf = None
        self.start = 0
        self.received = 0
        self.emitted = 0
        self.closed = False

    def _append(self, block):
        import torch

        if hasattr(block, "data_ptr"):
            b = block.to(self.dev, self.tdt)
        else:
            b = torch.from_numpy(np.ascontiguousarray(np.asarray(block, dtype=self.dtype))).to(self.dev)
        if b.dim() == 1:
            b = b[:, None]
        if b.shape[1] != self.nch:
# ... 178 lines not shown
```

Baseline: 30.21 billion.

## Fold IIR block transfer matrix into resampler taps in fused rsos kernel

Precomputes on the host a folded form of the fused resampler+IIR block. The 16x16 lower-triangular block matrix T is multiplied into the resampler tap table, and the state-update matrix is replaced by E = D·T⁻¹ with permuted time ordering. The kernel can then skip the four per-block MFMAs that apply T. It writes outputs with wider dwordx4 stores in the permuted layout, and a new template path is gated on f64, 8 or 12 waves, and a conditioning bound (amp ≤ 256). The trade-off is extra host-side setup, a larger operand buffer, and some risk of numerical error when T is poorly conditioned.

Measured after the change: 31.35 billion (median of 6 runs). 3.8% higher.

```diff
diff --git a/include/sigops.h b/include/sigops.h
--- a/include/sigops.h
+++ b/include/sigops.h
@@ -215,7 +215,8 @@
     SO_COUNTER_RSOS_WARMUP_PERIODS = 6,
     SO_COUNTER_RSOS_PERIOD_INPUTS = 7,
     SO_COUNTER_WPROJ_FRAMES = 8,
-    SO_COUNTER_WPROJ_FIRST = 9
+    SO_COUNTER_WPROJ_FIRST = 9,
+    SO_COUNTER_RSOS_FOLD = 10
 } so_counter_t;
 int64_t so_plan_counter(const so_plan_t* plan, int32_t which);
 
@@ -283,6 +284,9 @@
                              int32_t ngroups, int32_t kw, int64_t m, int32_t wp, double* v, int32_t capacity,
                              int32_t* j0, int32_t* k);
 
+int32_t so_rsos_fold_tables(const double* sos, int32_t nsec, double gain, const double* tab, int32_t ngroups, int32_t kw,
+                            double* e, double* ftab, double* amp, int32_t* fold);
+
 #if defined(__GNUC__)
 #pragma GCC visibility pop
 #endif
diff --git a/signaloperators.jl_amd/_capi.py b/signaloperators.jl_amd/_capi.py
--- a/signaloperators.jl_amd/_capi.py
+++ b/signaloperators.jl_amd/_capi.py
@@ -67,7 +67,7 @@
            "so_plan_nframes", "so_plan_execute", "so_plan_check", "so_plan_set_array", "so_plan_stats",
            "so_plan_set_profiling", "so_plan_destroy", "so_design_iir",
            "so_design_resample_rational", "so_design_resample_arbitrary",
-           "so_resample_positions", "so_plan_step_info", "so_design_iir_zpk", "so_zpk_to_sos", "so_tf_to_sos", "so_tf_zero_input", "so_plan_counter", "so_rsos_wproj_matrix",
+           "so_resample_positions", "so_plan_step_info", "so_design_iir_zpk", "so_zpk_to_sos", "so_tf_to_sos", "so_tf_zero_input", "so_plan_counter", "so_rsos_wproj_matrix", "so_rsos_fold_tables",
            "so_rtc_compile_check", "so_rtc_wait_idle", "so_rtc_shutdown", "so_comm_unique_id", "so_comm_create", "so_comm_allgather", "so_comm_reduce_sum", "so_comm_last_error", "so_comm_destroy"]
 
 _lib = None
@@ -163,6 +163,9 @@
     L.so_rsos_wproj_matrix.argtypes = [C.POINTER(C.c_double), C.c_int32, C.c_double, C.POINTER(C.c_double), C.POINTER(C.c_int32),
                                        C.c_int32, C.c_int32, C.c_int64, C.c_int32, C.POINTER(C.c_double), C.c_int32,
                                        C.POINTER(C.c_int32), C.POINTER(C.c_int32)]
+    L.so_rsos_fold_tables.restype = C.c_int32
+    L.so_rsos_fold_tables.argtypes = [C.POINTER(C.c_double), C.c_int32, C.c_double, C.POINTER(C.c_double), C.c_int32, C.c_int32,
+                                      C.POINTER(C.c_double), C.POINTER(C.c_double), C.POINTER(C.c_double), C.POINTER(C.c_int32)]
     L.so_plan_step_info.restype = C.c_int32
     L.so_plan_step_info.argtypes = [C.c_void_p, C.c_int32, C.POINTER(so_step_info_t)]
     L.so_resample_positions.restype = C.c_int32
diff --git a/signaloperators.jl_amd/csrc/capi.cpp b/signaloperators.jl_amd/csrc/capi.cpp
--- a/signaloperators.jl_amd/csrc/capi.cpp
+++ b/signaloperators.jl_amd/csrc/capi.cpp
@@ -249,4 +249,14 @@
     return SO_OK;
 }
 
-}
+int32_t so_rsos_fold_tables(const double* sos, int32_t nsec, double gain, const double* tab, int32_t ngroups, int32_t kw,
+                            double* e, double* ftab, double* amp, int32_t* fold) {
+    if (!sos || !tab || !e || !ftab || !amp || !fold || nsec < 1 || nsec > 6 || ngroups < 1 || ngroups > 256 || kw < 1 || kw > 4096)
+        return set_err(SO_ERR_INVALID, "so_rsos_fold_tables: bad arguments");
+    int f = 0;
+    so::rsos_fold_tables_sos(sos, nsec, gain, tab, ngroups, kw, e, ftab, amp, &f);
+    *fold = f;
+    return SO_OK;
+}
+
+}
diff --git a/signaloperators.jl_amd/csrc/executor.cpp b/signaloperators.jl_amd/csrc/executor.cpp
--- a/signaloperators.jl_amd/csrc/executor.cpp
+++ b/signaloperators.jl_amd/csrc/executor.cpp
@@ -899,7 +899,8 @@
     }
     const double* rtab = (const double*)P->bufs[S.rsos_tab_buf >= 0 ? S.rsos_tab_buf : S3.tab_buf].d;
     const int* rjend = (const int*)P->bufs[S.rsos_jend_buf >= 0 ? S.rsos_jend_buf : S3.jend_buf].d;
-    if (launch_rsos(rtab, rjend, rs, yk, global_tables(P, S3), S.rsos_grid, st) != 0)
+    if (rs.out_f32) rs.fold = 0;
+    if (launch_rsos(rs.fold ? rs.mats + rs.fold_off + 7 * 64 : rtab, rjend, rs, yk, global_tables(P, S3), S.rsos_grid, st) != 0)
         fail(SO_ERR_RUNTIME, "internal: no fused resampler + IIR instantiation for this geometry");
     if (rtracing) dump_rsos_trace(d_rtrace, rtrace_n, rs, st);
     int nl = 1;
@@ -1378,7 +1379,12 @@
     case SO_COUNTER_DIRECT_EXECUTES: return P->n_direct;
     case SO_COUNTER_FUSED_MFMAS_PER_BLOCK: {
         for (const Stage& S : P->stages)
-            if (S.kind == ST_SOS && S.rsos_src >= 0 && S.need > 0) return S.rs.ks + 14;
+            if (S.kind == ST_SOS && S.rsos_src >= 0 && S.need > 0) return S.rs.ks + (S.rs.fold ? 10 : 14);
+        return 0;
+    }
+    case SO_COUNTER_RSOS_FOLD: {
+        for (const Stage& S : P->stages)
+            if (S.kind == ST_SOS && S.rsos_src >= 0 && S.need > 0) return S.rs.fold;
         return 0;
     }
     case SO_COUNTER_WPROJ: {
diff --git a/signaloperators.jl_amd/csrc/k_rsos.hip b/signaloperators.jl_amd/csrc/k_rsos.hip
--- a/signaloperators.jl_amd/csrc/k_rsos.hip
+++ b/signaloperators.jl_amd/csrc/k_rsos.hip
@@ -15,6 +15,7 @@
 
 typedef double v4d __attribute__((ext_vector_type(4)));
 typedef float v4f __attribute__((ext_vector_type(4)));
+typedef double v2d __attribute__((ext_vector_type(2)));
 
 #define SO_LDS __attribute__((address_space(3)))
 __device__ __forceinline__ int flag_ld(uint32_t a) { return *(const volatile SO_LDS int*)(uintptr_t)a; }
@@ -1163,9 +1164,10 @@
     __builtin_amdgcn_s_setprio(0);
 }
 
-template <int KS, int NY, int NL, typename TO, int CYC, bool F32M = false, bool HW = false>
+template <int KS, int NY, int NL, typename TO, int CYC, bool F32M = false, bool HW = false, bool FOLD = false>
 __device__ __attribute__((noinline)) void rsos_ywave(RsosShared* sh_, double* dyn, int64_t G_, int yi_) {
     static_assert(!F32M || (sizeof(TO) == 4 && CYC > 0), "the Float32 MFMA form: Float32 results, taps in registers");
+    static_assert(!FOLD || (sizeof(TO) == 8 && !F32M && !HW), "the folded block: Float64 results, no helper wave");
     constexpr int NX = 2 * NY + 1;
     const int lane = threadIdx.x & 63;
     const int wave = uni(threadIdx.x >> 6);
@@ -1196,14 +1198,23 @@
                         (!src32 || uni(g.chunk) == 128) && (!uni(g.arr2) || rsos_two_ok(C0, uni(g.chunk)));
     const RsosGroup grp = rsos_group(sh, G, single, (int64_t)(rfl64((int64_t)(uintptr_t)C0.base) >> (src32 ? 2 : 3)), cs0, df0);
     const int gq = lane >> 4, n16 = lane & 15;
-    double Dk[4], Tk[4], Ck[3];
+    double Dk[4], Ck[3];
+    [[maybe_unused]] double Tk[4];
     const int nkc = (uni(g.debug) & 131072) ? 3 : (2 * uni(g.nsec) + 3) / 4;
-#pragma unroll
-    for (int v = 0; v < 4; ++v) Dk[v] = F32M ? mats[(lane >> 4) * 64 + v * 16 + (lane & 15)] : mats[v * 64 + lane];
-#pragma unroll
-    for (int v = 0; v < 4; ++v) Tk[v] = F32M ? mats[(7 + (lane >> 4)) * 64 + v * 16 + (lane & 15)] : mats[(7 + v) * 64 + lane];
-#pragma unroll
-    for (int v = 0; v < 3; ++v) Ck[v] = mats[(11 + v) * 64 + lane];
+    if constexpr (FOLD) {
+        const double SO_GLB* fm = mats + uni(g.fold_off);
+#pragma unroll
+        for (int v = 0; v < 4; ++v) Dk[v] = fm[v * 64 + lane];
+#pragma unroll
+        for (int v = 0; v < 3; ++v) Ck[v] = fm[(4 + v) * 64 + lane];
+    } else {
+#pragma unroll
+        for (int v = 0; v < 4; ++v) Dk[v] = F32M ? mats[(lane >> 4) * 64 + v * 16 + (lane & 15)] : mats[v * 64 + lane];
+#pragma unroll
+        for (int v = 0; v < 4; ++v) Tk[v] = F32M ? mats[(7 + (lane >> 4)) * 64 + v * 16 + (lane & 15)] : mats[(7 + v) * 64 + lane];
+#pragma unroll
+        for (int v = 0; v < 3; ++v) Ck[v] = mats[(11 + v) * 64 + lane];
+    }
     int cl;
     int nb0;
     {
@@ -1227,7 +1238,26 @@
 #endif
     const bool yfits = SO_Y_SADDR && uni((int)((((int64_t)(ct - 1) * out_pitch + (int64_t)(16 / ct) * grp.prL + 16) * (int64_t)sizeof(TO)) < ((int64_t)1 << 32)));
     int nbs_all;
-    {
+    [[maybe_unused]] bool st16 = false;
+    if constexpr (FOLD) {
+        const int ri = n16 / ct, cv = n16 % ct;
+        const int64_t ob = grp.ob0 + ri * grp.prL;
+        const int64_t off0 = ((int64_t)cv * out_pitch + (int64_t)ri * grp.prL + 2 * gq) * (int64_t)sizeof(TO);
+        yo0 = (uint32_t)off0;
+#pragma unroll
+        for (int v = 0; v < 4; ++v) ystep[v] = 0;
+        const int64_t tl = n_out - ob - 15;
+        const int64_t nb = tl <= 0 ? 0 : (tl + 15) / 16;
+        int m = (int)(nb > 0x3fffffff ? 0x3fffffff : nb);
+        int al = (int)((((uint64_t)(uintptr_t)y + (uint64_t)(ybase_e * (int64_t)sizeof(TO) + off0)) & 15) == 0);
+#pragma unroll
+        for (int off = 32; off > 0; off >>= 1) {
+            m = min(m, __shfl_xor(m, off, 64));
+            al = min(al, __shfl_xor(al, off, 64));
+        }
+        nbs_all = uni(m);
+        st16 = uni(al) != 0;
+    } else {
         int m = 0x7fffffff;
         int64_t off0 = 0;
 #pragma unroll
@@ -1297,6 +1327,12 @@
         }
     };
     auto back_mfma = [&](const double (&sv)[3], v4d ay) __attribute__((always_inline)) {
+        if constexpr (FOLD) {
+            ay = __builtin_amdgcn_mfma_f64_16x16x4f64(Ck[0], sv[0], ay, 0, 0, 0);
+            if (nkc > 1) ay = __builtin_amdgcn_mfma_f64_16x16x4f64(Ck[1], sv[1], ay, 0, 0, 0);
+            if (nkc > 2) ay = __builtin_amdgcn_mfma_f64_16x16x4f64(Ck[2], sv[2], ay, 0, 0, 0);
+            return ay;
+        }
         ay = __builtin_amdgcn_mfma_f64_16x16x4f64(sv[0], Ck[0], ay, 0, 0, 0);
         if (nkc > 1) ay = __builtin_amdgcn_mfma_f64_16x16x4f64(sv[1], Ck[1], ay, 0, 0, 0);
         if (nkc > 2) ay = __builtin_amdgcn_mfma_f64_16x16x4f64(sv[2], Ck[2], ay, 0, 0, 0);
@@ -1307,6 +1343,31 @@
         const int64_t t0 = (int64_t)16 * pb_;
         const uint64_t yb = (uint64_t)rfl64((int64_t)ypend);
         if (fresh && yfits && sizeof(TO) == 8) asm volatile("s_nop 15\n\ts_nop 1" : "+v"(ay[0]), "+v"(ay[1]), "+v"(ay[2]), "+v"(ay[3])::"memory");
+        if constexpr (FOLD) {
+            const int64_t o0 = grp.ob0 + (int64_t)(n16 / ct) * grp.prL + t0 + 2 * gq;
+            const bool all = pb_ >= nbl_max && pb_ < nbs_all;
+            if (all && yfits && st16) {
+                const v2d lo = v2d{ay[0], ay[1]}, hi = v2d{ay[2], ay[3]};
+                asm volatile("global_store_dwordx4 %0, %1, %3\n\tglobal_store_dwordx4 %0, %2, %3 offset:64\n\ts_nop 1" ::"v"(yo0),
+                             "v"(lo), "v"(hi), "s"(yb)
+                             : "memory");
+            } else if (yfits) {
+                if (all || (o0 >= slo && o0 < n_out)) asm volatile("global_store_dwordx2 %0, %1, %2" ::"v"(yo0), "v"(ay[0]), "s"(yb) : "memory");
+                if (all || (o0 + 1 >= slo && o0 + 1 < n_out)) asm volatile("global_store_dwordx2 %0, %1, %2 offset:8" ::"v"(yo0), "v"(ay[1]), "s"(yb) : "memory");
+                if (all || (o0 + 8 >= slo && o0 + 8 < n_out)) asm volatile("global_store_dwordx2 %0, %1, %2 offset:64" ::"v"(yo0), "v"(ay[2]), "s"(yb) : "memory");
+                if (all || (o0 + 9 >= slo && o0 + 9 < n_out)) asm volatile("global_store_dwordx2 %0, %1, %2 offset:72" ::"v"(yo0), "v"(ay[3]), "s"(yb) : "memory");
+            } else {
+                int row = n16;
+                asm volatile("" : "+v"(row));
+                TO SO_GLB* const p = y + ((int64_t)(grp.cg * ct + row % ct) * out_pitch + grp.ob0 + (int64_t)(row / ct) * grp.prL + t0 + 2 * gq);
+#pragma unroll
+                for (int v = 0; v < 4; ++v) {
+                    const int dt = (v & 1) + 8 * (v >> 1);
+                    if (all || (o0 + dt >= slo && o0 + dt < n_out)) p[dt] = (TO)ay[v];
+                }
+            }
+            return;
+        }
         auto out_index = [&](int v) __attribute__((always_inline)) { return grp.ob0 + (int64_t)((gq + 4 * v) / ct) * grp.prL + t0 + n16; };
         auto put = [&](int v, TO val) __attribute__((always_inline)) {
             if (yfits) {
@@ -1427,7 +1488,9 @@
                 bx[s] = *(const SO_LDS double*)(ringc + (uint32_t)(p_ >= RING ? p_ - RING : p_) * 8u);
             }
         }
-        v4d ax = v4d{0.0, 0.0, 0.0, 0.0};
+        v4d ax_ = v4d{0.0, 0.0, 0.0, 0.0};
+        v4d& ax = FOLD ? pout : ax_;
+        if constexpr (FOLD) ax = v4d{0.0, 0.0, 0.0, 0.0};
         if constexpr (F32M) {
             v4f a0 = v4f{0.f, 0.f, 0.f, 0.f}, a1 = v4f{0.f, 0.f, 0.f, 0.f};
 #pragma unroll
@@ -1476,9 +1539,11 @@
 #pragma unroll
             for (int v = 0; v < 4; ++v) dx = __builtin_amdgcn_mfma_f64_16x16x4f64(Dk[v], ax[v], dx, 0, 0, 0);
         }
-        pout = __builtin_amdgcn_mfma_f64_16x16x4f64(ax[0], Tk[0], v4d{0.0, 0.0, 0.0, 0.0}, 0, 0, 0);
-#pragma unroll
-        for (int v = 1; v < 4; ++v) pout = __builtin_amdgcn_mfma_f64_16x16x4f64(ax[v], Tk[v], pout, 0, 0, 0);
+        if constexpr (!FOLD) {
+            pout = __builtin_amdgcn_mfma_f64_16x16x4f64(ax[0], Tk[0], v4d{0.0, 0.0, 0.0, 0.0}, 0, 0, 0);
+#pragma unroll
+            for (int v = 1; v < 4; ++v) pout = __builtin_amdgcn_mfma_f64_16x16x4f64(ax[v], Tk[v], pout, 0, 0, 0);
+        }
         if (!HELPABLE || hj < 0) {
 #pragma unroll
             for (int v = 0; v < 3; ++v) l.xs[slot * 192 + v * 64 + lane] = dx[v];
@@ -1566,7 +1631,7 @@
 
 
 constexpr int rsos_nthreads(int nw) { return (nw == 17 ? 16 : nw) * 64; }
-template <int KS, int NW, typename TO, int CYC>
+template <int KS, int NW, typename TO, int CYC, bool FOLDABLE = false>
 __device__ __forceinline__ void rsos_body(const double* __restrict__ tab, const int* __restrict__ jend_g, const RsSos& g, TO* __restrict__ y,
                                           const RsGlobalTables& gsrc, int64_t G0, int64_t Gstep) {
     constexpr bool HW = NW == 17;
@@ -1695,6 +1760,12 @@
                     continue;
                 }
             }
+            if constexpr (FOLDABLE && sizeof(TO) == 8 && (NW == 12 || NW == 8)) {
+                if (g.fold) {
+                    rsos_ywave<KS, NY, NL, TO, CYC, false, false, true>(&sh, lds_raw, G, yi);
+                    continue;
+                }
+            }
             rsos_ywave<KS, NY, NL, TO, CYC, false, HW>(&sh, lds_raw, G, yi);
         }
     }
@@ -1703,7 +1774,7 @@
 template <int KS, int NW, typename TO, int CYC>
 __global__ __launch_bounds__(rsos_nthreads(NW)) void k_rsos(const double* __restrict__ tab, const int* __restrict__ jend_g, RsSos g,
                                                   TO* __restrict__ y, RsGlobalTables gsrc) {
-    rsos_body<KS, NW, TO, CYC>(tab, jend_g, g, y, gsrc, (int64_t)blockIdx.x, (int64_t)gridDim.x);
+    rsos_body<KS, NW, TO, CYC, true>(tab, jend_g, g, y, gsrc, (int64_t)blockIdx.x, (int64_t)gridDim.x);
 }
 
 template <int KS, int NW, typename TO, int CYC>
diff --git a/signaloperators.jl_amd/csrc/plan.h b/signaloperators.jl_amd/csrc/plan.h
--- a/signaloperators.jl_amd/csrc/plan.h
+++ b/signaloperators.jl_amd/csrc/plan.h
@@ -22,6 +22,8 @@
 
 void rsos_wproj_matrix_sos(const double* sos, int nsec, double gain, const double* tab, const int* jend, int ngroups, int kw, int64_t M, int wp,
                            std::vector<double>& V, int& j0, int& K);
+void rsos_fold_tables_sos(const double* sos, int nsec, double gain, const double* tab, int ngroups, int kw, double* e, double* ftab, double* amp,
+                          int* fold);
 int resample_positions(double fs_in, double fs_out, double rate, int nphi, const double* h, int hlen,
                        int64_t n_out, int64_t* j, int32_t* p, double* alpha, int64_t* nfix, int64_t* nbaked);
 
diff --git a/signaloperators.jl_amd/csrc/sigops_internal.h b/signaloperators.jl_amd/csrc/sigops_internal.h
--- a/signaloperators.jl_amd/csrc/sigops_internal.h
+++ b/signaloperators.jl_amd/csrc/sigops_internal.h
@@ -317,8 +317,11 @@
     int32_t* bad;
     long long* trace;
     uint32_t* err;
+    int32_t fold;
+    int32_t fold_off;
 };
 constexpr int kRsosTraceIters = 96;
+constexpr int rsos_fold_time(int m) { return 2 * (m & 3) + ((m >> 2) & 1) + 8 * (m >> 3); }
 
 struct RsosItem {
     RsSos g;
diff --git a/signaloperators.jl_amd/csrc/stages.cpp b/signaloperators.jl_amd/csrc/stages.cpp
--- a/signaloperators.jl_amd/csrc/stages.cpp
+++ b/signaloperators.jl_amd/csrc/stages.cpp
@@ -1682,19 +1682,20 @@
     }
 }
 
-static void rsos_block_columns(const SosCoefs& cf, std::vector<double>& Tm, std::vector<double>& Cm, std::vector<double>& Dm, std::vector<double>& Am) {
+template <typename R>
+static void rsos_block_columns(const SosCoefs& cf, std::vector<R>& Tm, std::vector<R>& Cm, std::vector<R>& Dm, std::vector<R>& Am) {
     const int ns = cf.nsec, D = 2 * ns, B = 16;
     Tm.assign(B * B, 0.0);
     Cm.assign(B * 12, 0.0);
     Dm.assign(12 * B, 0.0);
     Am.assign(12 * 12, 0.0);
     for (int col = 0; col < B + D; ++col) {
-        std::vector<double> st(D, 0.0);
+        std::vector<R> st(D, 0.0);
         if (col >= B) st[col - B] = 1.0;
         for (int t = 0; t < B; ++t) {
-            double v = col == t ? 1.0 : 0.0;
+            R v = col == t ? 1.0 : 0.0;
             for (int f = 0; f < ns; ++f) {
-                const double xi = v;
+                const R xi = v;
                 v = st[2 * f] + cf.b0[f] * xi;
                 st[2 * f] = st[2 * f + 1] + cf.b1[f] * xi - cf.a1[f] * v;
                 st[2 * f + 1] = cf.b2[f] * xi - cf.a2[f] * v;
@@ -1729,6 +1730,102 @@
     }
 }
 
+constexpr double kRsosFoldAmp = 256.0;
+struct RsosFold {
+    std::vector<double> E;
+    std::vector<double> ftab;
+    std::vector<double> Cp;
+    double amp = 0.0;
+    bool ok = false;
+};
+static void rsos_fold_tables(const SosCoefs& cf, const double* tab, int ngroups, int kw, RsosFold& F) {
+    typedef long double R;
+    const int B = 16;
+    std::vector<R> Tm, Cm, Dm, Am;
+    rsos_block_columns<R>(cf, Tm, Cm, Dm, Am);
+    F = RsosFold{};
+    F.E.assign(12 * B, 0.0);
+    F.Cp.assign(B * 12, 0.0);
+    F.ftab.assign((size_t)ngroups * kw * 16, 0.0);
+    F.amp = INFINITY;
+    if (!(std::fabs((double)Tm[0]) > 0.0) || !std::isfinite((double)Tm[0])) return;
+    std::vector<R> Ti(B * B, 0.0L), E(12 * B, 0.0L);
+    for (int j = 0; j < B; ++j)
+        for (int i = j; i < B; ++i) {
+            R a = i == j ? 1.0L : 0.0L;
+            for (int k = j; k < i; ++k) a -= Tm[i * B + k] * Ti[k * B + j];
+            Ti[i * B + j] = a / Tm[i * B + i];
+        }
+    R dmax = 0.0L, emax = 0.0L;
+    for (int i = 0; i < 12; ++i) {
+        R dsum = 0.0L, esum = 0.0L;
+        for (int j = 0; j < B; ++j) {
+            R a = 0.0L;
+            for (int k = j; k < B; ++k) a += Dm[i * B + k] * Ti[k * B + j];
+            E[i * B + j] = a;
+            dsum += fabsl(Dm[i * B + j]);
+        }
+        for (int j = 0; j < B; ++j) {
+            R a = 0.0L;
+            for (int k = j; k < B; ++k) a += fabsl(E[i * B + k]) * fabsl(Tm[k * B + j]);
+            esum += a;
+        }
+        dmax = std::max(dmax, dsum);
+        emax = std::max(emax, esum);
+    }
+    F.amp = dmax > 0.0L ? (double)(emax / dmax) : INFINITY;
+    F.ok = std::isfinite(F.amp) && F.amp <= kRsosFoldAmp;
+    for (int i = 0; i < 12 * B; ++i) F.E[i] = (double)E[i];
+    for (int m = 0; m < B; ++m)
+        for (int d = 0; d < 12; ++d) F.Cp[m * 12 + d] = (double)Cm[rsos_fold_time(m) * 12 + d];
+    for (size_t r = 0; r < (size_t)ngroups * kw; ++r) {
+        const double* tp = tab + r * 16;
+        for (int m = 0; m < B; ++m) {
+            const int t = rsos_fold_time(m);
+            R a = 0.0L;
+            for (int k = 0; k <= t; ++k) a += Tm[t * B + k] * (R)tp[k];
+            F.ftab[r * 16 + m] = (double)a;
+        }
+    }
+}
+
+static void rsos_fold_operands(const RsosFold& F, std::vector<double>& mats) {
+    const size_t o = mats.size();
+    mats.resize(o + (size_t)7 * 64 + F.ftab.size(), 0.0);
+    for (int lane = 0; lane < 64; ++lane) {
+        const int i = lane & 15, kq = lane >> 4;
+        for (int v = 0; v < 4; ++v) {
+            const int k = 4 * v + kq;
+            mats[o + (size_t)v * 64 + lane] = i < 12 ? F.E[i * 16 + rsos_fold_time(k)] : 0.0;
+            if (v < 3) mats[o + (size_t)(4 + v) * 64 + lane] = F.Cp[i * 12 + k];
+        }
+    }
+    std::copy(F.ftab.begin(), F.ftab.end(), mats.begin() + (ptrdiff_t)(o + 7 * 64));
+}
+
+static SosCoefs sos_rows_coefs(const double* sos, int nsec, double gain) {
+    SosCoefs cf{};
+    cf.nsec = nsec;
+    cf.gain = gain;
+    for (int f = 0; f < nsec; ++f) {
+        cf.b0[f] = sos[6 * f + 0];
+        cf.b1[f] = sos[6 * f + 1];
+        cf.b2[f] = sos[6 * f + 2];
+        cf.a1[f] = sos[6 * f + 4];
+        cf.a2[f] = sos[6 * f + 5];
+    }
+    return cf;
+}
+void rsos_fold_tables_sos(const double* sos, int nsec, double gain, const double* tab, int ngroups, int kw, double* e, double* ftab, double* amp,
+                          int* fold) {
+    RsosFold F;
+    rsos_fold_tables(sos_rows_coefs(sos, nsec, gain), tab, ngroups, kw, F);
+    std::copy(F.E.begin(), F.E.end(), e);
+    std::copy(F.ftab.begin(), F.ftab.end(), ftab);
+    *amp = F.amp;
+    *fold = F.ok ? 1 : 0;
+}
+
 static void rsos_wproj_matrix(const SosCoefs& cf, const double* tab, const int* jend, int ngroups, int kw, int64_t M, int wp, std::vector<double>& V,
                        int& j0, int& K) {
     std::vector<double> Tm, Cm, Dm, Am;
@@ -1770,17 +1867,7 @@
 
 void rsos_wproj_matrix_sos(const double* sos, int nsec, double gain, const double* tab, const int* jend, int ngroups, int kw, int64_t M, int wp,
                            std::vector<double>& V, int& j0, int& K) {
-    SosCoefs cf{};
-    cf.nsec = nsec;
-    cf.gain = gain;
-    for (int f = 0; f < nsec; ++f) {
-        cf.b0[f] = sos[6 * f + 0];
-        cf.b1[f] = sos[6 * f + 1];
-        cf.b2[f] = sos[6 * f + 2];
-        cf.a1[f] = sos[6 * f + 4];
-        cf.a2[f] = sos[6 * f + 5];
-    }
-    rsos_wproj_matrix(cf, tab, jend, ngroups, kw, M, wp, V, j0, K);
+    rsos_wproj_matrix(sos_rows_coefs(sos, nsec, gain), tab, jend, ngroups, kw, M, wp, V, j0, K);
 }
 
 
@@ -2029,7 +2116,19 @@
                 wpj = c0.dtype == SO_F64 && c0.array_node >= 0 && (c0.nsteps == 0 || sine);
             }
             const double t_pro = wpj ? 0.013 * (double)(wp * Mp + kwp) : 0.0;
-            const double t_fused = (double)((ngrp + cus - 1) / cus) * ((double)((pr + (wpj ? 0 : wp)) * ngp) * 0.30 * unit_cost * (ks + 14) / 28.0 + t_pro) + 15.0;
+            double fold_pace = 1.0;
+            if (!std::getenv("SIGOPS_RSOS_NOFOLD") && !std::getenv("SIGOPS_RSOS_NWAVES") && nodes[S2.node].dtype == SO_F64 && !two_arrays && !was_ga && ct >= 8 &&
+                (plain_src ? S3.in_array_node >= 0 && nodes[nodes[S3.node].kids[0]].dtype != SO_F32
+                           : S3.carriers[0].dtype == SO_F64 && S3.carriers[0].array_node >= 0)) {
+                const std::vector<double>& tb = own_tab ? own_taps : S3.tab_host;
+                if (tb.size() == (size_t)ngp * kwp * 16) {
+                    RsosFold F;
+                    rsos_fold_tables(S2.groups[0], tb.data(), ngp, kwp, F);
+                    if (F.ok) fold_pace = 0.97;
+                }
+            }
+            const double t_fused =
+                (double)((ngrp + cus - 1) / cus) * ((double)((pr + (wpj ? 0 : wp)) * ngp) * 0.30 * unit_cost * fold_pace * (ks + 14) / 28.0 + t_pro) + 15.0;
             const double t_two = 8.0e-6 * (double)need * nch + 95.0;
             if (std::getenv("SIGOPS_DEBUG_PLAN"))
                 std::fprintf(stderr, "[sigops] k_rsos estimate: fused %.0f us (%lld groups, %lld + %lld periods), two kernels %.0f us\n", t_fused,
@@ -2201,6 +2300,23 @@
         }
     }
 
+    void fold_tables() {
+        const std::vector<double>& tb = own_tab ? S2.rsos_tab_host : S3.tab_host;
+        S2.rs.fold = 0;
+        S2.rs.fold_off = 0;
+        if (std::getenv("SIGOPS_RSOS_NOFOLD") || nodes[S2.node].dtype != SO_F64 || g.src32 || g.ring32 || g.x32 || g.f32m || (g.nwaves != 12 && g.nwaves != 8) ||
+            L % 16 != 0 || tb.size() != (size_t)ngp * kwp * 16 || S3.carriers[0].array_node < 0)
+            return;
+        RsosFold F;
+        rsos_fold_tables(S2.groups[0], tb.data(), ngp, kwp, F);
+        if (std::getenv("SIGOPS_DEBUG_PLAN"))
+            std::fprintf(stderr, "[sigops] k_rsos: folded block %s: amp %.3g (gate %.0f)\n", F.ok ? "taken" : "declined", F.amp, kRsosFoldAmp);
+        if (!F.ok) return;
+        S2.rs.fold_off = (int32_t)S2.rsos_mats_host.size();
+        rsos_fold_operands(F, S2.rsos_mats_host);
+        S2.rs.fold = 1;
+    }
+
     void commit_launch() {
         S2.rsos_mats_buf = P.raw_buf(S2.rsos_mats_host.size() * 8);
         if (S2.bad_buf < 0) S2.bad_buf = P.raw_buf((size_t)nch * 8);
@@ -2246,6 +2362,7 @@
         F.rewrite_carriers();
         F.commit();
         F.wproj_tables();
+        F.fold_tables();
         F.commit_launch();
     }
 }
diff --git a/signaloperators.jl_amd/engine.py b/signaloperators.jl_amd/engine.py
--- a/signaloperators.jl_amd/engine.py
+++ b/signaloperators.jl_amd/engine.py
@@ -111,11 +111,11 @@
         L = K.lib()
         return {"graph_replays": L.so_plan_counter(self.handle, 0), "graph_captures": L.so_plan_counter(self.handle, 1),
                 "direct_executes": L.so_plan_counter(self.handle, 2), "fused_mfmas_per_block": L.so_plan_counter(self.handle, 3),
-                "wproj": L.so_plan_counter(self.handle, 4)}
+                "wproj": L.so_plan_counter(self.handle, 4), "fold": L.so_plan_counter(self.handle, 10)}
 
     def rsos_geometry(self):
         L = K.lib()
-        return {k: L.so_plan_counter(self.handle, i) for i, k in enumerate(("pr", "wp", "M", "wproj_frames", "wproj_first"), 5)}
+        return {k: L.so_plan_counter(self.handle, i) for i, k in enumerate(("pr", "wp", "M", "wproj_frames", "wproj_first", "fold"), 5)}
 
     def steps(self):
         out = []
```
